# pgvector/pgvector

Measured on AMD Instinct MI355X. Metric: QPS @ recall@10 (IVFFlat, 1M x 1536d), higher is better.
Workload: dtype f32

## Files before the change

include/pgv_hip.h:

```cpp
#ifndef PGV_HIP_H
#define PGV_HIP_H

#include <stddef.h>
#include <stdint.h>

#ifdef __cplusplus
extern "C" {
#endif

#define PGV_ABI_VERSION 1

#define PGV_OK 0
#define PGV_ERR_ARG 1
#define PGV_ERR_DIMS 2
#define PGV_ERR_DEVICE 3
#define PGV_ERR_NOMEM 4
#define PGV_ERR_STATE 5
#define PGV_ERR_DATA 6

typedef enum pgv_dtype
{
	PGV_F32 = 0,
	PGV_F16 = 1
}			pgv_dtype;

typedef enum pgv_metric
{
	PGV_L2SQ = 0,
	PGV_NEG_IP = 1,
	PGV_L1 = 2
}			pgv_metric;

typedef enum pgv_ops
{
	PGV_OPS_L2 = 0,
	PGV_OPS_IP = 1,
	PGV_OPS_COSINE = 2
}			pgv_ops;

typedef struct pgv_ctx pgv_ctx;
typedef struct pgv_index pgv_index;
typedef struct pgv_hnsw pgv_hnsw;

typedef struct pgv_rng
{
	double		(*next_double) (void *state);
	uint32_t	(*next_u32) (void *state);
	void	   *state;
	uint64_t	seed;
}			pgv_rng;


const char *pgv_last_error(void);
int			pgv_abi_version(void);

int			pgv_device_count(void);
int			pgv_scan_chain_length(int dim, pgv_dtype dtype, int path);
int			pgv_device_memory(int device, uint64_t *free_bytes, uint64_t *total_bytes);
int			pgv_pinned_alloc(size_t bytes, void **out);
void		pgv_pinned_free(void *p);
int			pgv_pinned_register(void *p, size_t bytes);
void		pgv_pinned_unregister(void *p);

#define PGV_DEFAULT_STREAM ((void *) (intptr_t) -1)
int			pgv_ctx_create(int device, void *stream, pgv_ctx * *out);
void		pgv_ctx_destroy(pgv_ctx * ctx);
int			pgv_ctx_sync(pgv_ctx * ctx);
void	   *pgv_ctx_stream(pgv_ctx * ctx);
int			pgv_timer_start(pgv_ctx * ctx);
int			pgv_timer_stop(pgv_ctx * ctx, float *out_ms);

typedef struct pgv_stats
{
	double		scan_ms;
	int64_t		scan_launches;
	double		scan_pairs;
	double		scan_rows;
	double		aux_ms;
	int64_t		aux_launches;
	double		aux_pairs;
	double		assign_redo_rows;
	double		assign_rows;
	double		assign_recheck_rows;
	double		scan_unique_rows;
	double		scan_redo_queries;
	double		scan_widened_queries;
	double		scan_shadow_queries;
}			pgv_stats;
int			pgv_ctx_set_profiling(pgv_ctx * ctx, int on);
int			pgv_ctx_set_exact_scan(pgv_ctx * ctx, int on);
#define PGV_BOUND_STATISTICAL 0
#define PGV_BOUND_WORST_CASE 1
int			pgv_ctx_set_bound(pgv_ctx * ctx, int mode);
int			pgv_ctx_reset_stats(pgv_ctx * ctx);
int			pgv_ctx_get_stats(pgv_ctx * ctx, pgv_stats * out);


int			pgv_index_upload(pgv_ctx * ctx, pgv_metric metric, pgv_dtype dtype, int dim, int nlists,
							 const void *centers, const int64_t *list_offsets,
							 const void *vectors, const uint64_t *tids, pgv_index * *out);
void		pgv_index_free(pgv_index * index);
int			pgv_index_share(pgv_index * index, pgv_ctx * ctx, pgv_index * *out);
int			pgv_index_set_overlap(pgv_index * index, int lanes);
#define PGV_INDEX_HANDLE_BYTES 256
typedef struct pgv_index_handle
{
	unsigned char bytes[PGV_INDEX_HANDLE_BYTES];
}			pgv_index_handle;
int			pgv_index_export(pgv_index * index, pgv_index_handle * out);
int			pgv_index_import(pgv_ctx * ctx, const pgv_index_handle * handle, pgv_index * *out);
int			pgv_index_tids(pgv_index * index, const int64_t *slots, int64_t n, uint64_t *out);
int64_t		pgv_index_rows(const pgv_index * index);
int			pgv_index_lists(const pgv_index * index);

int			pgv_rank_lists(pgv_index * index, const void *queries, int nq, int maxprobes,
						   int32_t *out_lists, float *out_dist);

int			pgv_scan_lists(pgv_index * index, const void *query, const int32_t *lists, int nlists,
						   float *out_dist, int64_t *out_slot, int64_t capacity, int64_t *out_count);

int			pgv_search_batch(pgv_index * index, const void *queries, int nq, int probes, int k,
							 float *out_dist, int64_t *out_slot, uint64_t *out_tid);

int			pgv_index_shadow_cast(pgv_index * index, const void *queries, int nq, void *out_qcast, float *out_qscale,
								  float *out_qeps, float *out_cscale, float *out_ceps);

int			pgv_scan_batch(pgv_index * index, const void *queries, int nq, const int32_t *probe_lists,
						   int probes, int k, float *out_dist, int64_t *out_slot, uint64_t *out_tid);

typedef struct pgv_query pgv_query;
int			pgv_query_begin(pgv_index * index, pgv_query * *out);
void		pgv_query_end(pgv_query * q);
int			pgv_query_rank(pgv_query * q, const void *query, int max_probes);
int			pgv_query_scan(pgv_query * q, int first, int nprobes, int head, float *out_dist, int64_t *out_slot,
						   uint64_t *out_tid, int *out_count, int64_t *out_total);
int			pgv_query_more(pgv_query * q, int skip, int count, float *out_dist, int64_t *out_slot,
						   uint64_t *out_tid, int *out_count);
int			pgv_query_lists(pgv_query * q, int32_t *out_lists, int n);


int			pgv_assign(pgv_ctx * ctx, pgv_metric metric, pgv_dtype dtype, int dim,
					   const void *centers, int k, const void *rows, int64_t n,
					   int32_t *out_list, float *out_dist);

int			pgv_kmeans(pgv_ctx * ctx, pgv_ops ops, pgv_dtype dtype, int dim,
					   const void *samples, int n, int k, int max_iterations, const pgv_rng * rng,
					   void *out_centers, int32_t *out_closest, int *out_iters);

int			pgv_lloyd_partial(pgv_ctx * ctx, pgv_ops ops, pgv_dtype dtype, int dim,
							  const void *samples, int n, const void *centers, int k,
							  int32_t *io_closest, float *out_sums, int32_t *out_counts,
							  int64_t *out_changes);
int			pgv_lloyd_finish(pgv_ctx * ctx, pgv_ops ops, pgv_dtype dtype, int dim, int k,
							 const float *sums, const int32_t *counts, const pgv_rng * rng,
							 void *out_centers);

int			pgv_kmeanspp_init(pgv_ctx * ctx, pgv_ops ops, pgv_dtype dtype, int dim,
							  const void *samples, int n, int k, const pgv_rng * rng,
							  void *out_centers);


typedef struct pgv_comm pgv_comm;

#define PGV_COMM_ID_BYTES 128
int			pgv_comm_unique_id(void *out_id);
int			pgv_comm_create(pgv_ctx * ctx, int nranks, int rank, const void *unique_id, pgv_comm * *out);

typedef struct pgv_collectives
{
// ... 146 lines not shown
```

pgvector_amd/_lib.py:

```python
import ctypes as C
import os

try:
    import torch
except ImportError:
    torch = None

_HERE = os.path.dirname(os.path.abspath(__file__))
LIB_PATH = os.environ.get("PGV_HIP_LIB") or os.path.join(_HERE, "lib", "libpgv_hip.so")

PGV_OK, PGV_ERR_ARG, PGV_ERR_DIMS, PGV_ERR_DEVICE, PGV_ERR_NOMEM, PGV_ERR_STATE, PGV_ERR_DATA = range(7)
PGV_F32, PGV_F16 = 0, 1
PGV_L2SQ, PGV_NEG_IP, PGV_L1 = 0, 1, 2
PGV_OPS_L2, PGV_OPS_IP, PGV_OPS_COSINE = 0, 1, 2
PGV_BOUND_STATISTICAL, PGV_BOUND_WORST_CASE = 0, 1

SYMBOLS = [
    "pgv_last_error", "pgv_abi_version", "pgv_device_count", "pgv_scan_chain_length", "pgv_ctx_create", "pgv_ctx_destroy",
    "pgv_ctx_sync", "pgv_ctx_stream", "pgv_timer_start", "pgv_timer_stop", "pgv_ctx_set_profiling", "pgv_ctx_set_exact_scan", "pgv_index_share", "pgv_pinned_alloc", "pgv_pinned_free",
    "pgv_ctx_reset_stats", "pgv_ctx_get_stats", "pgv_index_upload", "pgv_index_free",
    "pgv_index_rows", "pgv_index_lists", "pgv_rank_lists", "pgv_scan_lists", "pgv_search_batch", "pgv_scan_batch",
    "pgv_assign", "pgv_kmeans", "pgv_lloyd_partial", "pgv_lloyd_finish", "pgv_kmeanspp_init",
    "pgv_distance_batch", "pgv_cosine_distance_batch", "pgv_bit_distance_batch", "pgv_hnsw_upload", "pgv_hnsw_free", "pgv_hnsw_score", "pgv_hnsw_set_graph", "pgv_hnsw_search",
    "pgv_hnsw_build_search", "pgv_hnsw_build_neighbors", "pgv_hnsw_link_begin", "pgv_hnsw_link_prepare",
    "pgv_hnsw_link_apply", "pgv_hnsw_link_end", "pgv_hnsw_build_search_keep", "pgv_hnsw_build_select_kept", "pgv_hnsw_score_pairs", "pgv_hnsw_score_groups", "pgv_hnsw_update_graph",
    "pgv_query_begin", "pgv_query_end", "pgv_query_rank", "pgv_query_scan", "pgv_query_more", "pgv_query_lists",
    "pgv_comm_unique_id", "pgv_comm_create", "pgv_comm_create_custom", "pgv_comm_destroy", "pgv_comm_size",
    "pgv_comm_rank", "pgv_kmeans_sharded", "pgv_search_batch_sharded",
    "pgv_device_memory", "pgv_pinned_register", "pgv_pinned_unregister", "pgv_index_export", "pgv_index_import",
    "pgv_index_tids", "pgv_hnsw_export", "pgv_hnsw_import", "pgv_hnsw_share", "pgv_hnsw_device", "pgv_exact_topk", "pgv_ctx_set_bound",
    "pgv_hnsw_upload_payload", "pgv_hnsw_get_payload", "pgv_builder_begin", "pgv_builder_add", "pgv_builder_set_centers", "pgv_builder_rows", "pgv_builder_finish", "pgv_builder_free", "pgv_index_drain",
    "pgv_index_set_overlap", "pgv_index_shadow_cast", "pgv_bit_topk", "pgv_binary_quantize", "pgv_rerank",
    "pgv_hnsw_upload_bits", "pgv_index_upload_bits", "pgv_index_nbits", "pgv_bit_assign", "pgv_bit_kmeans",
    "pgv_bit_lloyd_step", "pgv_sparse_distance_batch", "pgv_sparse_cosine_distance_batch", "pgv_sparse_topk",
]


class PgvError(RuntimeError):
    def __init__(self, code, message):
        super().__init__("libpgv_hip error %d: %s" % (code, message))
        self.code = code
        self.message = message


class PgvStats(C.Structure):
    _fields_ = [("scan_ms", C.c_double), ("scan_launches", C.c_int64),
                ("scan_pairs", C.c_double), ("scan_rows", C.c_double),
                ("aux_ms", C.c_double), ("aux_launches", C.c_int64), ("aux_pairs", C.c_double),
                ("assign_redo_rows", C.c_double), ("assign_rows", C.c_double), ("assign_recheck_rows", C.c_double), ("scan_unique_rows", C.c_double), ("scan_redo_queries", C.c_double), ("scan_widened_queries", C.c_double),
                ("scan_shadow_queries", C.c_double)]


ALL_REDUCE_F32 = C.CFUNCTYPE(C.c_int, C.c_void_p, C.c_void_p, C.c_size_t, C.c_void_p)
ALL_GATHER = C.CFUNCTYPE(C.c_int, C.c_void_p, C.c_void_p, C.c_void_p, C.c_size_t, C.c_void_p)


class PgvCollectives(C.Structure):
    _fields_ = [("all_reduce_sum_f32", ALL_REDUCE_F32), ("all_gather", ALL_GATHER), ("state", C.c_void_p)]


NEXT_DOUBLE = C.CFUNCTYPE(C.c_double, C.c_void_p)
NEXT_U32 = C.CFUNCTYPE(C.c_uint32, C.c_void_p)


class PgvRng(C.Structure):
    _fields_ = [("next_double", C.c_void_p), ("next_u32", C.c_void_p),
                ("state", C.c_void_p), ("seed", C.c_uint64)]


def _load():
    if not os.path.exists(LIB_PATH):
        raise ImportError(
            "libpgv_hip.so not built (%s): run `python -c 'import __graft_entry__ as g; g.build()'` "
            "or `make -C pgvector_amd/csrc` -- there is no CPU fallback" % LIB_PATH)
    lib = C.CDLL(LIB_PATH)
    P, I, I64 = C.c_void_p, C.c_int, C.c_int64
    lib.pgv_last_error.restype = C.c_char_p
    lib.pgv_last_error.argtypes = []
    lib.pgv_abi_version.restype = I
    lib.pgv_device_count.restype = I
    lib.pgv_scan_chain_length.argtypes = [I, I, I]
    lib.pgv_scan_chain_length.restype = I
    lib.pgv_ctx_create.argtypes = [I, P, C.POINTER(P)]
    lib.pgv_ctx_destroy.argtypes = [P]
    lib.pgv_ctx_destroy.restype = None
    lib.pgv_ctx_sync.argtypes = [P]
    lib.pgv_ctx_stream.argtypes = [P]
    lib.pgv_ctx_stream.restype = P
    lib.pgv_timer_start.argtypes = [P]
    lib.pgv_timer_stop.argtypes = [P, C.POINTER(C.c_float)]
    lib.pgv_ctx_set_profiling.argtypes = [P, I]
    lib.pgv_ctx_set_exact_scan.argtypes = [P, I]
    lib.pgv_ctx_reset_stats.argtypes = [P]
    lib.pgv_ctx_get_stats.argtypes = [P, C.POINTER(PgvStats)]
    lib.pgv_index_upload.argtypes = [P, I, I, I, I, P, P, P, P, C.POINTER(P)]
    lib.pgv_index_free.argtypes = [P]
    lib.pgv_index_share.argtypes = [P, P, C.POINTER(P)]
    lib.pgv_index_set_overlap.argtypes = [P, I]
    lib.pgv_index_shadow_cast.argtypes = [P, P, I, P, P, P, P, P]
    lib.pgv_index_free.restype = None
    lib.pgv_index_export.argtypes = [P, P]
    lib.pgv_index_import.argtypes = [P, P, C.POINTER(P)]
    lib.pgv_index_tids.argtypes = [P, P, I64, P]
    lib.pgv_hnsw_export.argtypes = [P, P]
    lib.pgv_hnsw_share.argtypes = [P, P, C.POINTER(P)]
    lib.pgv_hnsw_device.argtypes = [P]
    lib.pgv_hnsw_upload_payload.argtypes = [P, I, I, I, P, I64, P, I, C.POINTER(P)]
    lib.pgv_hnsw_get_payload.argtypes = [P, P, I, P]
    lib.pgv_hnsw_upload_bits.argtypes = [P, I, I, P, I64, P, I, C.POINTER(P)]
    lib.pgv_exact_topk.argtypes = [P, I, I, I, P, I, P, I64, I, P, P]
    lib.pgv_ctx_set_bound.argtypes = [P, I]
    lib.pgv_builder_begin.argtypes = [P, I, I, I, I, P, I64, C.POINTER(P)]
    lib.pgv_builder_add.argtypes = [P, P, P, I64]
    lib.pgv_builder_set_centers.argtypes = [P, P]
    lib.pgv_builder_rows.argtypes = [P]
    lib.pgv_builder_rows.restype = I64
    lib.pgv_builder_finish.argtypes = [P, C.POINTER(P), P, P]
    lib.pgv_builder_free.argtypes = [P]
    lib.pgv_builder_free.restype = None
    lib.pgv_index_drain.argtypes = [P, I64, P, P]
    lib.pgv_hnsw_import.argtypes = [P, P, C.POINTER(P)]
    lib.pgv_device_memory.argtypes = [I, C.POINTER(C.c_uint64), C.POINTER(C.c_uint64)]
    lib.pgv_pinned_register.argtypes = [P, C.c_size_t]
    lib.pgv_pinned_unregister.argtypes = [P]
    lib.pgv_pinned_unregister.restype = None
    lib.pgv_index_rows.argtypes = [P]
    lib.pgv_index_rows.restype = I64
    lib.pgv_index_lists.argtypes = [P]
    lib.pgv_rank_lists.argtypes = [P, P, I, I, P, P]
    lib.pgv_scan_lists.argtypes = [P, P, P, I, P, P, I64, C.POINTER(I64)]
    lib.pgv_search_batch.argtypes = [P, P, I, I, I, P, P, P]
    lib.pgv_scan_batch.argtypes = [P, P, I, P, I, I, P, P, P]
# ... 55 lines not shown
```

pgvector_amd/api.py:

```python
import ctypes as C
import weakref

import numpy as np

from . import _lib
from ._lib import (PGV_ERR_ARG, PGV_ERR_STATE, PGV_F16, PGV_F32, PGV_L1, PGV_L2SQ, PGV_NEG_IP, PGV_OPS_COSINE,
                   PGV_OPS_IP, PGV_OPS_L2, PgvError, PgvRng, PgvStats, check, lib)

_NP_OF = {PGV_F32: np.float32, PGV_F16: np.float16}


def _is_torch(x):
    return type(x).__module__.startswith("torch")


def ptr(x):
    if x is None:
        return None
    if _is_torch(x):
        assert x.is_contiguous(), "tensor must be contiguous"
        return C.c_void_p(x.data_ptr())
    assert isinstance(x, np.ndarray) and x.flags["C_CONTIGUOUS"], "need a C-contiguous array"
    return C.c_void_p(x.ctypes.data)

# ... 11 lines not shown

def as_dtype(x, dtype):
    if _is_torch(x):
        return x.contiguous()
    return np.ascontiguousarray(x, dtype=_NP_OF[dtype])


def make_rng(seed=0, next_double=None, next_u32=None, state=None):
    r = PgvRng()
    r.next_double = C.cast(next_double, C.c_void_p) if next_double is not None else None
    r.next_u32 = C.cast(next_u32, C.c_void_p) if next_u32 is not None else None
    r.state = state
    r.seed = seed
    return r


class Context:
    def __init__(self, device=0, stream=None):
        h = C.c_void_p()
        if stream is None:
            arg = None
        elif stream == 0:
            arg = C.c_void_p(-1)
        else:
            arg = C.c_void_p(stream)
        check(lib.pgv_ctx_create(device, arg, C.byref(h)))
        self.h = h
        self.device = device
        self._children = []

    def _adopt(self, child):
        self._children.append(weakref.ref(child))

    def close(self):
        if self.h:
            for ref in self._children:
                child = ref()
                if child is not None:
                    child.close()
            self._children = []
            lib.pgv_ctx_destroy(self.h)
            self.h = None

    def __del__(self):
        try:
            self.close()
        except Exception:
            pass

    def sync(self):
        check(lib.pgv_ctx_sync(self.h))

    def stream(self):
        return lib.pgv_ctx_stream(self.h)

    def timer_start(self):
        check(lib.pgv_timer_start(self.h))

    def timer_stop(self):
        ms = C.c_float()
        check(lib.pgv_timer_stop(self.h, C.byref(ms)))
        return ms.value

    def set_profiling(self, on):
        check(lib.pgv_ctx_set_profiling(self.h, 1 if on else 0))

    def set_exact_scan(self, on):
        check(lib.pgv_ctx_set_exact_scan(self.h, 1 if on else 0))

    def set_bound(self, worst_case):
        check(lib.pgv_ctx_set_bound(self.h, _lib.PGV_BOUND_WORST_CASE if worst_case else _lib.PGV_BOUND_STATISTICAL))

    def reset_stats(self):
        check(lib.pgv_ctx_reset_stats(self.h))

    def stats(self):
        s = PgvStats()
        check(lib.pgv_ctx_get_stats(self.h, C.byref(s)))
        return {"scan_ms": s.scan_ms, "scan_launches": s.scan_launches,
                "scan_pairs": s.scan_pairs, "scan_rows": s.scan_rows,
                "aux_ms": s.aux_ms, "aux_launches": s.aux_launches, "aux_pairs": s.aux_pairs,
                "assign_redo_rows": s.assign_redo_rows, "assign_rows": s.assign_rows,
                "assign_recheck_rows": s.assign_recheck_rows, "scan_unique_rows": s.scan_unique_rows, "scan_redo_queries": s.scan_redo_queries,
                "scan_widened_queries": s.scan_widened_queries, "scan_shadow_queries": s.scan_shadow_queries}


class IvfIndex:

    def __init__(self, ctx, metric, dtype, dim, centers, list_offsets, vectors, tids=None):
        self.ctx, self.metric, self.dtype, self.dim = ctx, metric, dtype, dim
        centers = as_dtype(centers, dtype)
        vectors = as_dtype(vectors, dtype)
        if not _is_torch(list_offsets):
            list_offsets = np.ascontiguousarray(list_offsets, dtype=np.int64)
        if tids is not None and not _is_torch(tids):
            tids = np.ascontiguousarray(tids, dtype=np.uint64)
        self.nlists = int(list_offsets.shape[0]) - 1
        h = C.c_void_p()
        check(lib.pgv_index_upload(ctx.h, metric, dtype, dim, self.nlists, ptr(centers),
                                   ptr(list_offsets), ptr(vectors), ptr(tids), C.byref(h)))
        self.h = h
        ctx._adopt(self)

    def set_overlap(self, lanes):
        check(lib.pgv_index_set_overlap(self.h, int(lanes)))

    def share(self, ctx):
        v = IvfIndex.__new__(IvfIndex)
        v.ctx, v.metric, v.dtype, v.dim, v.nlists = ctx, self.metric, self.dtype, self.dim, self.nlists
        h = C.c_void_p()
        check(lib.pgv_index_share(self.h, ctx.h, C.byref(h)))
        v.h = h
        ctx._adopt(v)
        return v

    def export(self):
        buf = C.create_string_buffer(256)
        check(lib.pgv_index_export(self.h, buf))
        return bytes(buf.raw)

    @classmethod
    def from_handle(cls, ctx, handle, metric=None, dtype=None, dim=None):
        v = cls.__new__(cls)
        h = C.c_void_p()
        buf = C.create_string_buffer(bytes(handle), 256)
        check(lib.pgv_index_import(ctx.h, buf, C.byref(h)))
        v.ctx, v.metric, v.dtype, v.dim, v.h = ctx, metric, dtype, dim, h
        v.nlists = lib.pgv_index_lists(h)
        ctx._adopt(v)
        return v

    def close(self):
        if self.h:
            lib.pgv_index_free(self.h)
            self.h = None

    def __del__(self):
        try:
            self.close()
        except Exception:
            pass

    @property
    def rows(self):
        return lib.pgv_index_rows(self.h)

    def tids(self, slots):
        slots = np.ascontiguousarray(slots, dtype=np.int64)
        out = np.empty(slots.shape, dtype=np.uint64)
        check(lib.pgv_index_tids(self.h, ptr(slots), int(slots.size), ptr(out)))
        return out

    def rank_lists(self, queries, maxprobes, want_dist=True):
        queries = as_dtype(queries, self.dtype)
        nq = int(queries.shape[0])
        lists = _empty_like_kind(queries, (nq, maxprobes), np.int32)
        dist = _empty_like_kind(queries, (nq, maxprobes), np.float32) if want_dist else None
        check(lib.pgv_rank_lists(self.h, ptr(queries), nq, maxprobes, ptr(lists), ptr(dist)))
        return lists, dist

    def scan_lists(self, query, lists):
        if query is not None:
            query = as_dtype(query, self.dtype)
        lists = np.ascontiguousarray(lists, dtype=np.int32)
        count = C.c_int64()
        rc = lib.pgv_scan_lists(self.h, ptr(query), ptr(lists), len(lists), None, None, 0, C.byref(count))
        if rc != _lib.PGV_OK and count.value == 0:
# ... 737 lines not shown
```

pgvector_amd/csrc/kernels_query.hip:

```cpp
#include "pgv_device.h"
#include "pgv_select.h"

#include <type_traits>

namespace pgv {

namespace {

constexpr int kQThreads = kSelThreads;
constexpr int kQWaves = kQThreads / kWave;
constexpr int kMaxBatchLists = 256;
constexpr int kHeadCap = 1024;

template <typename T, int METRIC, int NCH> struct WholeRows {
    Raw16 q[NCH];
    __device__ __forceinline__ void load_query(const char *qp, int lane) {
#pragma unroll
        for (int c = 0; c < NCH; c++) q[c] = load16(qp + ((size_t)c * kWave + lane) * sizeof(Raw16));
    }
    __device__ __forceinline__ float pair(const char *a, const char *b, int lane) const {
        Raw16 ra[NCH], rb[NCH];
#pragma unroll
        for (int c = 0; c < NCH; c++) ra[c] = load16(a + ((size_t)c * kWave + lane) * sizeof(Raw16));
#pragma unroll
// ... 222 lines not shown

template <typename T, int METRIC, int NCH>
__global__ __launch_bounds__(kQThreads) void mq_rank_kernel(const char *__restrict__ centers, int nlists, int nvec, int lg,
                                                            const char *__restrict__ queries, float *__restrict__ cdist,
                                                            int64_t cd_stride, int per) {
    const size_t row_bytes = (size_t)nvec * sizeof(Raw16);
    const char *qp = queries + (size_t)blockIdx.y * row_bytes;
    float *cd = cdist + (size_t)blockIdx.y * cd_stride;
    for (int64_t first = (int64_t)blockIdx.x * per; first < nlists; first += (int64_t)gridDim.x * per) {
        const int64_t end = first + per < nlists ? first + per : nlists;
        score_rows<T, METRIC, NCH>([&](int64_t j) { return centers + (size_t)j * row_bytes; }, first, end, qp, nvec, lg, cd);
    }
}

__global__ __launch_bounds__(kQThreads) void mq_lists_kernel(const float *__restrict__ cdist, int64_t cd_stride, int nlists,
                                                             int max_probes, int kp, int32_t *__restrict__ out_lists,
                                                             float *__restrict__ out_dist) {
    extern __shared__ __attribute__((aligned(16))) char smem[];
    unsigned long long *ent = reinterpret_cast<unsigned long long *>(smem);
    SelShared *s = reinterpret_cast<SelShared *>(smem + (size_t)kHeadCap * 8);
    const int q = blockIdx.x;
    block_topk_auto(cdist + (size_t)q * cd_stride, nlists, max_probes, kp, kHeadCap, ent, s);
    for (int i = threadIdx.x; i < max_probes; i += kQThreads) {
        out_lists[(size_t)q * max_probes + i] = (int32_t)(unsigned)(ent[i] & 0xffffffffu);
        if (out_dist) out_dist[(size_t)q * max_probes + i] = key_to_float((unsigned)(ent[i] >> 32));
    }
}

template <typename T, int METRIC, int NCH>
__global__ __launch_bounds__(kQThreads) void mq_scan_kernel(
    const char *__restrict__ vectors, const int64_t *__restrict__ list_off, const int32_t *__restrict__ probe_lists,
    int nprobes, int nvec, int lg, const char *__restrict__ queries, float *__restrict__ seg, int64_t seg_stride, int per) {
    __shared__ BatchMap map;
    const size_t row_bytes = (size_t)nvec * sizeof(Raw16);
    const int q = blockIdx.y;
    map.build(probe_lists + (size_t)q * nprobes, nprobes, list_off);
    const int64_t m = map.offs[nprobes];
    const char *qp = queries + (size_t)q * row_bytes;
    float *sg = seg + (size_t)q * seg_stride;
    for (int64_t first = (int64_t)blockIdx.x * per; first < m; first += (int64_t)gridDim.x * per) {
        const int64_t end = first + per < m ? first + per : m;
        score_rows<T, METRIC, NCH>([&](int64_t j) { return vectors + (size_t)map.slot_of(j, nprobes) * row_bytes; },
                                   first, end, qp, nvec, lg, sg);
    }
}

__global__ __launch_bounds__(kQThreads) void mq_head_kernel(
    const float *__restrict__ seg, int64_t seg_stride, const int64_t *__restrict__ list_off,
    const uint64_t *__restrict__ tids, const int32_t *__restrict__ probe_lists, int nprobes, int k, int kp,
    float *__restrict__ out_dist, int64_t *__restrict__ out_slot, uint64_t *__restrict__ out_tid,
    double *__restrict__ stats) {
    extern __shared__ __attribute__((aligned(16))) char smem[];
    __shared__ BatchMap map;
    const int q = blockIdx.x;
    map.build(probe_lists + (size_t)q * nprobes, nprobes, list_off);
    const int64_t m = map.offs[nprobes];
    unsigned long long *ent = reinterpret_cast<unsigned long long *>(smem);
    SelShared *s = reinterpret_cast<SelShared *>(smem + (size_t)kHeadCap * 8);
    block_topk_auto(seg + (size_t)q * seg_stride, m, k, kp, kHeadCap, ent, s);
    const int have = (int)(m < k ? m : k);
    for (int i = threadIdx.x; i < k; i += kQThreads) {
        const size_t o = (size_t)q * k + i;
        if (i < have) {
            const unsigned long long e = ent[i];
            const int64_t slot = map.slot_of((int64_t)(unsigned)(e & 0xffffffffu), nprobes);
            out_dist[o] = key_to_float((unsigned)(e >> 32));
            if (out_slot) out_slot[o] = slot;
            if (out_tid) out_tid[o] = tids ? tids[slot] : ~0ull;
        } else {
            out_dist[o] = INFINITY;
            if (out_slot) out_slot[o] = -1;
            if (out_tid) out_tid[o] = ~0ull;
        }
    }
    if (stats && threadIdx.x == 0) {
        atomicAdd(&stats[0], (double)m);
        atomicAdd(&stats[1], (double)m);
        atomicAdd(&stats[5], (double)m);
    }
}

constexpr int kRecheckCap = 256;

template <typename T, bool DOT = false>
__global__ __launch_bounds__(kQThreads) void batch_recheck_kernel(
    const char *__restrict__ vectors, const uint64_t *__restrict__ tids, int nvec, int lg,
    const char *__restrict__ queries, int kprime, int k, const float *__restrict__ approx_val,
    const int64_t *__restrict__ cand_pos, const int64_t *__restrict__ cand_slot,
    const int64_t *__restrict__ list_off, const int32_t *__restrict__ probe_lists,
    const int64_t *__restrict__ probe_off, int probes,
    const int64_t *__restrict__ seg_start, int64_t fixed_len,
    const unsigned *__restrict__ row_norm_max, ScanBound bound, const float *__restrict__ eps_add, int nq,
    float *__restrict__ out_dist, int64_t *__restrict__ out_slot, uint64_t *__restrict__ out_tid,
    int32_t *__restrict__ out_i32, int32_t *__restrict__ flags, float *__restrict__ pair_t, PlanEmit emit) {
    static_assert(!DOT || std::is_same<T, float>::value, "pair terms: fp32 rows");
    __shared__ float exact[kRecheckCap];
    __shared__ float dots[DOT ? kRecheckCap : 1];
    __shared__ __attribute__((aligned(16))) unsigned long long ent[kRecheckCap];
    const int q = blockIdx.x;
    const size_t row_bytes = (size_t)nvec * sizeof(Raw16);
    const int64_t m = seg_start ? seg_start[q + 1] - seg_start[q] : fixed_len;
    const int ncand = (int)(m < kprime ? m : (int64_t)kprime);
    const int kk = ncand < k ? ncand : k;
    const float *av = approx_val + (size_t)q * kprime;
    __shared__ float qn_part[kQWaves];
    {
        const char *qrow = queries + (size_t)q * row_bytes;
        float a = 0.f;
        for (int v = threadIdx.x; v < nvec; v += kQThreads) {
            const Raw16 x = load16(qrow + (size_t)v * sizeof(Raw16));
            a = accum_slice<T, 1>(a, x, x);
        }
        for (int m2 = 32; m2 > 0; m2 >>= 1) a += __shfl_xor(a, m2);
        if ((threadIdx.x & (kWave - 1)) == 0) qn_part[threadIdx.x >> 6] = a;
    }
    __syncthreads();
    float qn = 0.f;
    for (int w = 0; w < kQWaves; w++) qn += qn_part[w];
    const float rn = __uint_as_float(*row_norm_max);
    const float cross = 2.f * sqrtf(qn * rn);
    const float eps = 1.001f * (bound.g_sq * (qn + rn + cross) + bound.g_dot * cross + bound.g_norm * rn +
                                (eps_add ? eps_add[q] : 0.f));
    unsigned band = 0u;
    if (kk > 0) {
        const float edge = av[kk - 1] + 2.f * eps;
        band = float_to_key(edge + bound.g_ref * fabsf(edge + qn));
    }
    const int cnt = __syncthreads_count((int)threadIdx.x < ncand && float_to_key(av[threadIdx.x]) <= band);
    __shared__ int64_t slots[kRecheckCap];
    if ((int)threadIdx.x < cnt) {
        const int64_t p = cand_pos[(size_t)q * kprime + threadIdx.x];
        int64_t slot = p;
        if (cand_slot) {
            slot = cand_slot[(size_t)q * kprime + threadIdx.x];
        } else {
            const int64_t *off = probe_off + (size_t)q * probes;
            int lo = 0, hi = probes - 1;
            while (lo < hi) {
                const int mid = (lo + hi + 1) >> 1;
                if (off[mid] <= p)
                    lo = mid;
                else
                    hi = mid - 1;
            }
            slot = list_off[probe_lists[(size_t)q * probes + lo]] + (p - off[lo]);
        }
        slots[threadIdx.x] = slot;
    }
    __syncthreads();
    if constexpr (DOT)
        score_rows_dot([&](int64_t j) { return vectors + (size_t)slots[j] * row_bytes; }, 0, cnt,
                       queries + (size_t)q * row_bytes, nvec, lg, exact, dots);
    else
        score_rows<T, 0, 0>([&](int64_t j) { return vectors + (size_t)slots[j] * row_bytes; }, 0, cnt,
                            queries + (size_t)q * row_bytes, nvec, lg, exact);
    __syncthreads();
    if ((int)threadIdx.x < kRecheckCap)
        ent[threadIdx.x] = (int)threadIdx.x < cnt
                               ? ((unsigned long long)float_to_key(exact[threadIdx.x]) << 32) |
                                     (unsigned)cand_pos[(size_t)q * kprime + threadIdx.x]
                               : ~0ull;
    __syncthreads();
    const unsigned long long mine = ent[threadIdx.x];
    const int64_t my_slot = (int)threadIdx.x < cnt ? slots[threadIdx.x] : -1;
    int rank = 0;
    {
        const ulonglong2 *e2 = reinterpret_cast<const ulonglong2 *>(ent);
        const int n2 = (cnt + 1) / 2;
#pragma unroll 8
        for (int j = 0; j < n2; j++) {
            const ulonglong2 o = e2[j];
            rank += o.x < mine ? 1 : 0;
            rank += o.y < mine ? 1 : 0;
        }
    }
    if ((int)threadIdx.x < cnt && rank < k) {
        const size_t o = (size_t)q * k + rank;
        out_dist[o] = key_to_float((unsigned)(mine >> 32));
        if (out_slot) out_slot[o] = my_slot;
        if (out_i32) out_i32[o] = (int32_t)my_slot;
        if (out_tid) out_tid[o] = tids ? tids[my_slot] : ~0ull;
        if constexpr (DOT) pair_t[o] = -2.f * dots[threadIdx.x];
    }
    if ((int)threadIdx.x >= kk && (int)threadIdx.x < k) {
        const size_t o = (size_t)q * k + threadIdx.x;
        out_dist[o] = INFINITY;
        if (out_slot) out_slot[o] = -1;
        if (out_i32) out_i32[o] = -1;
        if (out_tid) out_tid[o] = ~0ull;
        if constexpr (DOT) pair_t[o] = 0.f;
    }
    if constexpr (DOT) {
        if (emit.cnt) {
            __syncthreads();
            if ((int)threadIdx.x < cnt && rank < k) {
                atomicAdd(&emit.cnt[my_slot], 1);
                slots[rank] = emit.list_off[my_slot + 1] - emit.list_off[my_slot];
            }
            if ((int)threadIdx.x >= kk && (int)threadIdx.x < k) slots[threadIdx.x] = 0;
            __syncthreads();
            if ((int)threadIdx.x < k) {
                int64_t run = 0;
                for (int i = 0; i < (int)threadIdx.x; i++) run += slots[i];
                emit.probe_off[(size_t)q * k + threadIdx.x] = run;
                if ((int)threadIdx.x == k - 1) emit.seg_len[q] = run + slots[threadIdx.x];
            }
        }
    }
    if (threadIdx.x == 0) {
        const int32_t flag = (m > ncand && cnt == ncand) ? 1 : 0;
        flags[q] = flag;
        if (flag) flags[nq + 1 + atomicAdd(&flags[nq], 1)] = q;
    }
}

constexpr int kWide = kRecheckCap;

template <typename T>
__global__ __launch_bounds__(kQThreads) void batch_fix_kernel(
    const char *__restrict__ vectors, const int64_t *__restrict__ list_off, const uint64_t *__restrict__ tids, int nvec,
    int lg, const char *__restrict__ queries, const int32_t *__restrict__ probe_lists,
    const int64_t *__restrict__ probe_off, int probes, const int64_t *__restrict__ seg_start, int64_t fixed_len,
    const int32_t *__restrict__ flags, int nq, float *__restrict__ seg_vals, int k, int kp, int cap,
    const unsigned *__restrict__ row_norm_max, ScanBound bound, const float *__restrict__ eps_add, int widen,
    float *__restrict__ out_dist, int64_t *__restrict__ out_slot, uint64_t *__restrict__ out_tid,
    int32_t *__restrict__ out_i32, double *__restrict__ stats, float *__restrict__ pair_t, PlanEmit emit) {
    extern __shared__ __attribute__((aligned(16))) char smem[];
    unsigned long long *ent = reinterpret_cast<unsigned long long *>(smem);
    SelShared *sel = reinterpret_cast<SelShared *>(smem + (size_t)cap * 8);
    __shared__ float exact[kWide];
    __shared__ int64_t slots[kWide];
    __shared__ float qn_part[kQWaves];
    const int nflag = flags[nq];
    const size_t row_bytes = (size_t)nvec * sizeof(Raw16);
    for (int f = blockIdx.x; f < nflag; f += gridDim.x) {
        const int q = flags[nq + 1 + f];
        const int64_t base = probe_lists ? seg_start[q] : (int64_t)q * fixed_len;
        const int64_t m = probe_lists ? seg_start[q + 1] - base : fixed_len;
        const int64_t *off = probe_off + (size_t)q * probes;
        const int32_t *pl = probe_lists + (size_t)q * probes;
        auto slot_of = [&](int64_t j) -> int64_t {
            if (!probe_lists) return j;
            int lo = 0, hi = probes - 1;
            while (lo < hi) {
                const int mid = (lo + hi + 1) >> 1;
                if (off[mid] <= j)
                    lo = mid;
                else
                    hi = mid - 1;
            }
            return list_off[pl[lo]] + (j - off[lo]);
        };
        float *v = seg_vals + base;
        const char *qrow = queries + (size_t)q * row_bytes;
        auto pair_terms = [&]() {
            if constexpr (std::is_same<T, float>::value) {
                if (pair_t) {
                    __threadfence();
                    __syncthreads();
                    fill_pair_terms(vectors, row_bytes, qrow, nvec * 4, out_i32 ? out_i32 + (size_t)q * k : nullptr,
                                    out_slot ? out_slot + (size_t)q * k : nullptr, k, pair_t + (size_t)q * k);
                    if (emit.cnt) {
                        if ((int)threadIdx.x < k) {
                            const int l = __hip_atomic_load(out_i32 + (size_t)q * k + threadIdx.x, __ATOMIC_RELAXED,
                                                            __HIP_MEMORY_SCOPE_AGENT);
                            if (l >= 0) atomicAdd(&emit.cnt[l], 1);
                            slots[threadIdx.x] = l >= 0 ? emit.list_off[l + 1] - emit.list_off[l] : 0;
                        }
                        __syncthreads();
                        if ((int)threadIdx.x < k) {
                            int64_t run = 0;
                            for (int i = 0; i < (int)threadIdx.x; i++) run += slots[i];
                            emit.probe_off[(size_t)q * k + threadIdx.x] = run;
                            if ((int)threadIdx.x == k - 1) emit.seg_len[q] = run + slots[threadIdx.x];
                        }
                    }
                }
            }
        };
        if constexpr (std::is_same<T, float>::value) {
            if (pair_t && emit.cnt) {
                if ((int)threadIdx.x < k) {
                    const int l = out_i32[(size_t)q * k + threadIdx.x];
                    if (l >= 0) atomicSub(&emit.cnt[l], 1);
                }
                __syncthreads();
            }
        }
        bool settled = false;
        if (widen && k <= kWide / 2) {
            const int nw = (int)(m < kWide ? m : (int64_t)kWide);
            block_topk([v](int64_t i) { return v[i]; }, m, nw, kWide, cap, ent, sel);
            {
                float a = 0.f;
                for (int x = threadIdx.x; x < nvec; x += kQThreads) {
                    const Raw16 e = load16(qrow + (size_t)x * sizeof(Raw16));
                    a = accum_slice<T, 1>(a, e, e);
                }
                for (int m2 = 32; m2 > 0; m2 >>= 1) a += __shfl_xor(a, m2);
                if ((threadIdx.x & (kWave - 1)) == 0) qn_part[threadIdx.x >> 6] = a;
            }
            __syncthreads();
            float qn = 0.f;
            for (int w = 0; w < kQWaves; w++) qn += qn_part[w];
            const float rn = __uint_as_float(*row_norm_max);
            const float cross = 2.f * sqrtf(qn * rn);
            const float eps = 1.001f * (bound.g_sq * (qn + rn + cross) + bound.g_dot * cross + bound.g_norm * rn +
                                        (eps_add ? eps_add[q] : 0.f));
            const int kk = nw < k ? nw : k;
            unsigned band = 0u;
            if (kk > 0) {
                const float edge = key_to_float((unsigned)(ent[kk - 1] >> 32)) + 2.f * eps;
                band = float_to_key(edge + bound.g_ref * fabsf(edge + qn));
            }
            const int cnt = __syncthreads_count((int)threadIdx.x < nw && (unsigned)(ent[threadIdx.x] >> 32) <= band);
            settled = !(m > nw && cnt == nw);
            if (settled) {
                const unsigned my_pos = (int)threadIdx.x < cnt ? (unsigned)(ent[threadIdx.x] & 0xffffffffu) : 0u;
                if ((int)threadIdx.x < cnt) slots[threadIdx.x] = slot_of((int64_t)my_pos);
                __syncthreads();
                score_rows<T, 0, 0>([&](int64_t j) { return vectors + (size_t)slots[j] * row_bytes; }, 0, cnt, qrow, nvec, lg,
                                    exact);
                __syncthreads();
                if ((int)threadIdx.x < kWide)
                    ent[threadIdx.x] = (int)threadIdx.x < cnt
                                           ? ((unsigned long long)float_to_key(exact[threadIdx.x]) << 32) | my_pos
                                           : ~0ull;
                __syncthreads();
                const unsigned long long mine = ent[threadIdx.x];
                int rank = 0;
                for (int j = 0; j < cnt; j++) rank += ent[j] < mine ? 1 : 0;
                const int have = (int)(m < k ? m : (int64_t)k);
                if ((int)threadIdx.x < cnt && rank < k) {
                    const size_t o = (size_t)q * k + rank;
                    const int64_t slot = slots[threadIdx.x];
                    out_dist[o] = key_to_float((unsigned)(mine >> 32));
                    if (out_slot) out_slot[o] = slot;
                    if (out_i32) out_i32[o] = (int32_t)slot;
                    if (out_tid) out_tid[o] = tids ? tids[slot] : ~0ull;
                }
                if ((int)threadIdx.x >= have && (int)threadIdx.x < k) {
                    const size_t o = (size_t)q * k + threadIdx.x;
                    out_dist[o] = INFINITY;
                    if (out_slot) out_slot[o] = -1;
                    if (out_i32) out_i32[o] = -1;
                    if (out_tid) out_tid[o] = ~0ull;
                }
                if (stats && threadIdx.x == 0) atomicAdd(&stats[7], 1.0);
                pair_terms();
            }
            __syncthreads();
        }
        if (settled) continue;
        if (stats && threadIdx.x == 0) atomicAdd(&stats[6], 1.0);
        score_rows<T, 0, 0>([&](int64_t j) { return vectors + (size_t)slot_of(j) * row_bytes; }, 0, m, qrow, nvec, lg, v);
        __threadfence();
        __syncthreads();
        block_topk([v](int64_t i) { return __hip_atomic_load(v + i, __ATOMIC_RELAXED, __HIP_MEMORY_SCOPE_AGENT); }, m, k, kp,
                   cap, ent, sel);
        for (int i = threadIdx.x; i < k; i += kQThreads) {
            const unsigned long long e = ent[i];
            const bool have = e != ~0ull && (int64_t)i < (m < k ? m : (int64_t)k);
            const int64_t slot = have ? slot_of((int64_t)(unsigned)(e & 0xffffffffu)) : -1;
            out_dist[(size_t)q * k + i] = have ? key_to_float((unsigned)(e >> 32)) : INFINITY;
            if (out_slot) out_slot[(size_t)q * k + i] = slot;
            if (out_i32) out_i32[(size_t)q * k + i] = (int32_t)slot;
            if (out_tid) out_tid[(size_t)q * k + i] = (have && tids) ? tids[slot] : ~0ull;
        }
        pair_terms();
        __syncthreads();
    }
}

constexpr size_t kQueryLds = (size_t)kHeadCap * 8 + sizeof(SelShared);

void run_geometry(pgv_ctx *ctx, const RowGeom &g, int64_t nrows, int *per, int *grid) {
    const bool whole = g.lpr_log2 == 6 && g.nvec % kWave == 0;
    const int step = kQWaves * (whole ? 2 : (kWave >> g.lpr_log2));
    int64_t runs = (nrows + step - 1) / step;
    const int64_t cap = (int64_t)ctx->num_cus * 8;
    *per = step;
    *grid = (int)(runs < 1 ? 1 : (runs > cap ? cap : runs));
}

int pow2_at_least(int k) {
    int kp = 2;
    while (kp < k) kp <<= 1;
    return kp;
}

template <typename T, int METRIC, typename F> int dispatch_nch(const RowGeom &g, F f) {
    if (g.lpr_log2 == 6 && g.nvec % kWave == 0) {
        switch (g.nvec / kWave) {
            case 1: return f(std::integral_constant<int, 1>());
            case 2: return f(std::integral_constant<int, 2>());
            case 3: return f(std::integral_constant<int, 3>());
            case 4: return f(std::integral_constant<int, 4>());
            case 6: return f(std::integral_constant<int, 6>());
        }
    }
    return f(std::integral_constant<int, 0>());
}

}

int query_max_batch_lists() { return kMaxBatchLists; }
int query_head_cap() { return kHeadCap; }
size_t query_head_bytes(int head) { return sizeof(QueryHead) + (size_t)head * (4 + 8 + 8) + 64; }

int launch_query_stage(pgv_ctx *ctx, const void *src_pinned, void *dst_dev, int nvec) {
    hipLaunchKernelGGL(query_stage_kernel, dim3(1), dim3(1024), 0, ctx->stream, static_cast<const Raw16 *>(src_pinned),
                       static_cast<Raw16 *>(dst_dev), nvec);
    PGV_HIP(hipGetLastError());
    return PGV_OK;
}

int launch_query_iota(pgv_ctx *ctx, int32_t *out, int n) {
    hipLaunchKernelGGL(query_iota_kernel, dim3((n + 255) / 256), dim3(256), 0, ctx->stream, out, n);
    PGV_HIP(hipGetLastError());
    return PGV_OK;
}

int launch_one_query_rows(pgv_ctx *ctx, const RowsView &v, const void *q_dev, float *out) {
    if (v.n <= 0) return PGV_OK;
    if (v.bits()) PGV_FAIL(PGV_ERR_ARG, "one query over rows: fp32 / fp16 rows only");
    const RowGeom &g = v.geom;
    const void *rows = v.rows;
    const int n = (int)v.n;
    int per, grid;
    run_geometry(ctx, g, n, &per, &grid);
    return dispatch_metric(v.metric, v.dtype(), [&](auto *tp, auto mc) {
        using T = std::remove_pointer_t<decltype(tp)>;
        constexpr int M = decltype(mc)::value;
        return dispatch_nch<T, M>(g, [&](auto nc) {
            constexpr int NCH = decltype(nc)::value;
            hipLaunchKernelGGL((query_rank_kernel<T, M, NCH>), dim3(grid), dim3(kQThreads), 0, ctx->stream,
                               static_cast<const char *>(rows), n, g.nvec, g.lpr_log2, static_cast<const char *>(q_dev),
                               out, per);
            PGV_HIP(hipGetLastError());
            return PGV_OK;
        });
    });
}

int launch_query_rank(pgv_ctx *ctx, const pgv_index *ix, const void *q_dev, float *cdist, int max_probes,
                      int32_t *out_lists) {
    const RowGeom &g = ix->geom;
    int per, grid;
    run_geometry(ctx, g, ix->nlists, &per, &grid);
    const int kp = pow2_at_least(max_probes);
    PGV_TRY(dispatch_metric(ix->metric, ix->dtype, [&](auto *tp, auto mc) {
        using T = std::remove_pointer_t<decltype(tp)>;
        constexpr int M = decltype(mc)::value;
        return dispatch_nch<T, M>(g, [&](auto nc) {
            constexpr int NCH = decltype(nc)::value;
            hipLaunchKernelGGL((query_rank_kernel<T, M, NCH>), dim3(grid), dim3(kQThreads), 0, ctx->stream,
// ... 13 lines not shown
                      int64_t rows_bound, float *seg) {
    const RowGeom &g = ix->geom;
    int per, grid;
    run_geometry(ctx, g, rows_bound, &per, &grid);
    return dispatch_metric(ix->metric, ix->dtype, [&](auto *tp, auto mc) {
        using T = std::remove_pointer_t<decltype(tp)>;
        constexpr int M = decltype(mc)::value;
        return dispatch_nch<T, M>(g, [&](auto nc) {
            constexpr int NCH = decltype(nc)::value;
            hipLaunchKernelGGL((query_scan_kernel<T, M, NCH>), dim3(grid), dim3(kQThreads), 0, ctx->stream,
                               static_cast<const char *>(ix->vectors), ix->list_offsets, probe_lists, nprobes, g.nvec,
                               g.lpr_log2, static_cast<const char *>(q_dev), seg, per);
            PGV_HIP(hipGetLastError());
            return PGV_OK;
        });
    });
}

int launch_query_head(pgv_ctx *ctx, const pgv_index *ix, const float *seg, const int32_t *probe_lists, int nprobes,
                      int skip, int count, void *head_rec, unsigned seq) {
    const int kp = pow2_at_least(skip + count);
    QueryHead *hdr = static_cast<QueryHead *>(head_rec);
    char *base = static_cast<char *>(head_rec) + 64;
    int64_t *h_slot = reinterpret_cast<int64_t *>(base);
    uint64_t *h_tid = reinterpret_cast<uint64_t *>(base + (size_t)count * 8);
    float *h_dist = reinterpret_cast<float *>(base + (size_t)count * 16);
    hipLaunchKernelGGL(query_head_kernel, dim3(1), dim3(kQThreads), kQueryLds, ctx->stream, seg, ix->list_offsets,
                       ix->tids, probe_lists, nprobes, skip, count, kp, hdr, h_dist, h_slot, h_tid, seq);
    PGV_HIP(hipGetLastError());
    return PGV_OK;
}

int launch_multi_rank(pgv_ctx *ctx, const pgv_index *ix, const void *q_dev, int nq, float *cdist, int64_t cd_stride,
                      int max_probes, int32_t *out_lists, float *out_dist) {
    const RowGeom &g = ix->geom;
    int per, grid;
    run_geometry(ctx, g, ix->nlists, &per, &grid);
    const int kp = pow2_at_least(max_probes);
    PGV_TRY(dispatch_metric(ix->metric, ix->dtype, [&](auto *tp, auto mc) {
        using T = std::remove_pointer_t<decltype(tp)>;
        constexpr int M = decltype(mc)::value;
        return dispatch_nch<T, M>(g, [&](auto nc) {
            constexpr int NCH = decltype(nc)::value;
            hipLaunchKernelGGL((mq_rank_kernel<T, M, NCH>), dim3(grid, nq), dim3(kQThreads), 0, ctx->stream,
                               static_cast<const char *>(ix->centers), ix->nlists, g.nvec, g.lpr_log2,
                               static_cast<const char *>(q_dev), cdist, cd_stride, per);
            PGV_HIP(hipGetLastError());
            return PGV_OK;
        });
    }));
    hipLaunchKernelGGL(mq_lists_kernel, dim3(nq), dim3(kQThreads), kQueryLds, ctx->stream, cdist, cd_stride, ix->nlists,
                       max_probes, kp, out_lists, out_dist);
    PGV_HIP(hipGetLastError());
    return PGV_OK;
}

int launch_multi_scan(pgv_ctx *ctx, const pgv_index *ix, const void *q_dev, int nq, const int32_t *probe_lists, int nprobes,
                      int64_t rows_bound, float *seg, int64_t seg_stride, int k, float *out_dist, int64_t *out_slot,
                      uint64_t *out_tid) {
    const RowGeom &g = ix->geom;
    int per, grid;
    run_geometry(ctx, g, rows_bound, &per, &grid);
    const int cap = (ctx->num_cus * 8 + nq - 1) / nq;
    if (grid > cap) grid = cap < 1 ? 1 : cap;
    PGV_TRY(dispatch_metric(ix->metric, ix->dtype, [&](auto *tp, auto mc) {
        using T = std::remove_pointer_t<decltype(tp)>;
        constexpr int M = decltype(mc)::value;
        return dispatch_nch<T, M>(g, [&](auto nc) {
            constexpr int NCH = decltype(nc)::value;
            hipLaunchKernelGGL((mq_scan_kernel<T, M, NCH>), dim3(grid, nq), dim3(kQThreads), 0, ctx->stream,
                               static_cast<const char *>(ix->vectors), ix->list_offsets, probe_lists, nprobes, g.nvec,
                               g.lpr_log2, static_cast<const char *>(q_dev), seg, seg_stride, per);
            PGV_HIP(hipGetLastError());
            return PGV_OK;
        });
    }));
    double *stats = (ctx->profiling && ctx->stats_dev.p) ? ctx->stats_dev.as<double>() : nullptr;
    hipLaunchKernelGGL(mq_head_kernel, dim3(nq), dim3(kQThreads), kQueryLds, ctx->stream, seg, seg_stride, ix->list_offsets,
                       ix->tids, probe_lists, nprobes, k, pow2_at_least(k), out_dist, out_slot, out_tid, stats);
    PGV_HIP(hipGetLastError());
    return PGV_OK;
}

namespace {
struct ApproxScratch {
    float *cand_val = nullptr;
    int64_t *cand_pos = nullptr;
    int32_t *flags = nullptr;
    int carve(DBuf &buf, int nq, int kprime) {
        const size_t nk = (size_t)nq * kprime;
        const size_t a1 = (sizeof(float) * nk + 15) & ~(size_t)15, a2 = a1 + sizeof(int64_t) * nk;
        PGV_TRY(buf.ensure(a2 + sizeof(int32_t) * (2 * (size_t)nq + 1)));
        cand_val = buf.as<float>();
        cand_pos = reinterpret_cast<int64_t *>(buf.as<char>() + a1);
        flags = reinterpret_cast<int32_t *>(buf.as<char>() + a2);
        return PGV_OK;
    }
};
}

int launch_exact_tail(pgv_ctx *ctx, const ExactTail &t, DBuf &scratch) {
    if (t.nq <= 0) return PGV_OK;
    const ExactRows &xr = t.rows;
    const bool dense = t.dense();
    if (dense ? (t.fixed_len <= 0 || t.probe_off || t.seg_start || t.probes != 0)
              : (t.fixed_len != 0 || !t.probe_off || !t.seg_start || t.probes < 1))
        PGV_FAIL(PGV_ERR_ARG, "exact tail: a list plan or one dense run");
    if (t.kprime > kRecheckCap || t.k > t.kprime)
        PGV_FAIL(PGV_ERR_ARG, "exact tail: k' = %d outside k..%d", t.kprime, kRecheckCap);
    if (t.pair_t && xr.dtype != PGV_F32) PGV_FAIL(PGV_ERR_ARG, "exact tail: pair terms are for fp32 rows");
    static_assert(kWide >= kRecheckCap, "k <= k' <= kWide: batch_fix_kernel's emit");
    if (t.emit.cnt && !(dense && t.pair_t && t.out_i32 && t.emit.probe_off && t.emit.seg_len && t.emit.list_off))
        PGV_FAIL(PGV_ERR_ARG, "exact tail: the plan is counted where the pair terms are written");
    ApproxScratch sc;
    PGV_TRY(sc.carve(scratch, t.nq, t.kprime));
    const int64_t *cand_slot = dense ? sc.cand_pos : nullptr;
    const int64_t *seg_start = dense ? nullptr : t.seg_start;
    const int64_t fixed_len = dense ? t.fixed_len : 0;
    PGV_TRY(launch_topk_segments(ctx, t.approx, seg_start, t.nq, fixed_len, t.kprime, sc.cand_val, sc.cand_pos,
                                 sc.flags + t.nq, t.emit.cnt, t.emit.cnt ? 2 * (int)fixed_len : 0,
                                 dense ? 0 : t.seg_bound));
#define PGV_RECHECK(T, DOT)                                                                                          \
    hipLaunchKernelGGL((batch_recheck_kernel<T, DOT>), dim3(t.nq), dim3(kQThreads), 0, ctx->stream,                   \
                       static_cast<const char *>(xr.vectors), xr.tids, xr.geom.nvec, xr.geom.lpr_log2,                \
                       static_cast<const char *>(t.queries), t.kprime, t.k, sc.cand_val, sc.cand_pos, cand_slot,      \
                       xr.list_offsets, t.probe_lists, t.probe_off, t.probes, seg_start, fixed_len, xr.norm_max,      \
                       t.bound, t.eps_add, t.nq, t.out_dist, t.out_slot, t.out_tid, t.out_i32, sc.flags, t.pair_t,    \
                       t.emit)
    if (t.pair_t)
        PGV_RECHECK(float, true);
    else if (xr.dtype == PGV_F32)
        PGV_RECHECK(float, false);
    else
        PGV_RECHECK(__half, false);
#undef PGV_RECHECK
    PGV_HIP(hipGetLastError());
    double *stats = (ctx->profiling && ctx->stats_dev.p) ? ctx->stats_dev.as<double>() : nullptr;
    int kp = 2;
    while (kp < t.k) kp <<= 1;
    const int cap = kp > kFastCap ? kp : kFastCap;
    const size_t lds = (size_t)cap * 8 + sizeof(SelShared);
    const int grid = t.nq < ctx->num_cus ? t.nq : ctx->num_cus;
#define PGV_FIX(T)                                                                                                    \
    hipLaunchKernelGGL(batch_fix_kernel<T>, dim3(grid), dim3(kQThreads), lds, ctx->stream,                            \
                       static_cast<const char *>(xr.vectors), xr.list_offsets, xr.tids, xr.geom.nvec,                 \
                       xr.geom.lpr_log2, static_cast<const char *>(t.queries), t.probe_lists, t.probe_off, t.probes,  \
                       seg_start, fixed_len, sc.flags, t.nq, t.approx, t.k, kp, cap, xr.norm_max, t.bound, t.eps_add, \
                       ctx->no_widen ? 0 : 1, t.out_dist, t.out_slot, t.out_tid, t.out_i32, stats, t.pair_t, t.emit)
    if (xr.dtype == PGV_F32)
        PGV_FIX(float);
    else
        PGV_FIX(__half);
#undef PGV_FIX
    PGV_HIP(hipGetLastError());
    return PGV_OK;
}

}
```

pgvector_amd/csrc/kernels_select.hip:

```cpp
#include "pgv_device.h"
#include "pgv_select.h"

namespace pgv {

namespace {


__global__ void plan_count_kernel(const int32_t *__restrict__ probe_lists,
                                  const int64_t *__restrict__ list_off, int nq, int probes,
                                  int *__restrict__ cnt, int64_t *__restrict__ probe_off,
                                  int64_t *__restrict__ seg_len) {
    const int q = blockIdx.x * blockDim.x + threadIdx.x;
    if (q >= nq) return;
    int64_t run = 0;
    for (int p = 0; p < probes; p++) {
        const int l = probe_lists[(size_t)q * probes + p];
        probe_off[(size_t)q * probes + p] = run;
        run += list_off[l + 1] - list_off[l];
        atomicAdd(&cnt[l], 1);
    }
    seg_len[q] = run;
}

template <typename F>
__device__ void block_exclusive_scan(int n, F value, int64_t *out, int64_t *scratch ) {
    const int lane = threadIdx.x & 63, wave = threadIdx.x >> 6, nwaves = blockDim.x >> 6;
    int64_t carry = 0;
    for (int base = 0; base < n; base += blockDim.x) {
        const int i = base + threadIdx.x;
        const int64_t v = i < n ? value(i) : 0;
        int64_t incl = v;
#pragma unroll
        for (int d = 1; d < 64; d <<= 1) {
            const int64_t t = __shfl_up(incl, d);
            if (lane >= d) incl += t;
        }
        if (lane == 63) scratch[wave] = incl;
        __syncthreads();
        int64_t before = 0, total = 0;
        for (int w = 0; w < nwaves; w++) {
            const int64_t t = scratch[w];
            if (w < wave) before += t;
            total += t;
        }
        if (i < n) out[i] = carry + before + incl - v;
        carry += total;
        __syncthreads();
    }
    if (threadIdx.x == 0) out[n] = carry;
    __syncthreads();
}

__global__ __launch_bounds__(1024) void plan_scan_kernel(
    const int *__restrict__ cnt, const int64_t *__restrict__ list_off,
    const int64_t *__restrict__ seg_len, int nq, int nlists, int qt, int rows_per_task,
    int64_t *__restrict__ seg_start, int64_t *__restrict__ pair_start,
    int64_t *__restrict__ task_start, int64_t *__restrict__ totals ,
    double *__restrict__ acc) {
    __shared__ int64_t scratch[1024 / 64 + 1];
    __shared__ double red[2][1024 / 64];
    block_exclusive_scan(nq, [&](int i) { return seg_len[i]; }, seg_start, scratch);
    block_exclusive_scan(nlists, [&](int i) { return (int64_t)cnt[i]; }, pair_start, scratch);
    double rows = 0.0, uniq = 0.0;
    block_exclusive_scan(
        nlists,
        [&](int i) {
            const int64_t len = list_off[i + 1] - list_off[i];
            const int64_t ng = (cnt[i] + qt - 1) / qt;
            const int64_t nc = (len + rows_per_task - 1) / rows_per_task;
            rows += (double)ng * (double)len;
            uniq += ng > 0 ? (double)len : 0.0;
            return ng * nc;
        },
        task_start, scratch);
    if (threadIdx.x == 0) {
        totals[0] = seg_start[nq];
        totals[1] = task_start[nlists];
        *reinterpret_cast<int *>(totals + 2) = (int)task_start[nlists];
    }
    if (acc) {
        for (int o = 32; o > 0; o >>= 1) {
            rows += __shfl_xor(rows, o);
            uniq += __shfl_xor(uniq, o);
        }
        if ((threadIdx.x & 63) == 0) {
            red[0][threadIdx.x >> 6] = rows;
            red[1][threadIdx.x >> 6] = uniq;
        }
        __syncthreads();
        if (threadIdx.x == 0) {
            double r = 0.0, u = 0.0;
            for (int w = 0; w < (int)(blockDim.x >> 6); w++) {
                r += red[0][w];
                u += red[1][w];
            }
            acc[0] += (double)seg_start[nq];
            acc[1] += r;
            acc[5] += u;
        }
    }
}

__device__ __forceinline__ void plan_pairs_body(int64_t i, const int32_t *__restrict__ probe_lists,
                                                const int64_t *__restrict__ list_off,
                                                const int64_t *__restrict__ probe_off,
                                                const int64_t *__restrict__ seg_start,
                                                const int64_t *__restrict__ pair_start, int *__restrict__ fill,
                                                int nq, int probes, const float *__restrict__ pair_t,
                                                ScanPair *__restrict__ pairs) {
    if (i >= (int64_t)nq * probes) return;
    const int q = (int)(i / probes);
    const int l = probe_lists[i];
    const int64_t pos = pair_start[l] + atomicAdd(&fill[l], 1);
    ScanPair pr;
    pr.out_rel = seg_start[q] + probe_off[i] - list_off[l];
    pr.query = q;
    pr.pad = pair_t ? (int32_t)__float_as_uint(pair_t[i]) : 0;
    pairs[pos] = pr;
}

__global__ void plan_pairs_kernel(const int32_t *__restrict__ probe_lists,
                                  const int64_t *__restrict__ list_off,
                                  const int64_t *__restrict__ probe_off,
                                  const int64_t *__restrict__ seg_start,
                                  const int64_t *__restrict__ pair_start, int *__restrict__ fill,
                                  int nq, int probes, const float *__restrict__ pair_t,
                                  ScanPair *__restrict__ pairs) {
    plan_pairs_body((int64_t)blockIdx.x * blockDim.x + threadIdx.x, probe_lists, list_off, probe_off, seg_start, pair_start,
                    fill, nq, probes, pair_t, pairs);
}

__device__ __forceinline__ void plan_tasks_body(int64_t first, int64_t stride, const int *__restrict__ cnt,
                                                const int64_t *__restrict__ list_off,
                                                const int64_t *__restrict__ pair_start,
                                                const int64_t *__restrict__ task_start, int nlists, int qt,
                                                int rows_per_task, ScanTask *__restrict__ tasks) {
    const int64_t ntasks = task_start[nlists];
    for (int64_t t = first; t < ntasks; t += stride) {
        int lo = 0, hi = nlists - 1;
        while (lo < hi) {
            const int mid = (lo + hi + 1) >> 1;
            if (task_start[mid] <= t)
                lo = mid;
            else
                hi = mid - 1;
        }
        const int l = lo;
        const int64_t len = list_off[l + 1] - list_off[l];
        const int ng = (cnt[l] + qt - 1) / qt;
        const int64_t rel = t - task_start[l];
        const int c = (int)(rel / ng), g = (int)(rel % ng);
        ScanTask task;
        task.row0 = list_off[l] + (int64_t)c * rows_per_task;
        const int64_t left = len - (int64_t)c * rows_per_task;
        task.nrows = (int)(left < rows_per_task ? left : rows_per_task);
        task.pair0 = (int)(pair_start[l] + (int64_t)g * qt);
        const int pl = cnt[l] - g * qt;
        task.npairs = pl < qt ? pl : qt;
        task.pad = ng > 1 ? 1 : 0;
        tasks[t] = task;
    }
}

__global__ void plan_tasks_kernel(const int *__restrict__ cnt, const int64_t *__restrict__ list_off,
                                  const int64_t *__restrict__ pair_start,
                                  const int64_t *__restrict__ task_start, int nlists, int qt,
                                  int rows_per_task, ScanTask *__restrict__ tasks) {
    plan_tasks_body((int64_t)blockIdx.x * blockDim.x + threadIdx.x, (int64_t)gridDim.x * blockDim.x, cnt, list_off,
                    pair_start, task_start, nlists, qt, rows_per_task, tasks);
}

__global__ void plan_pairs_tasks_kernel(const int32_t *__restrict__ probe_lists, const int64_t *__restrict__ list_off,
                                        const int64_t *__restrict__ probe_off, const int64_t *__restrict__ seg_start,
                                        const int64_t *__restrict__ pair_start, const int64_t *__restrict__ task_start,
                                        const int *__restrict__ cnt, int *__restrict__ fill, int nq, int probes, int nlists,
                                        int qt, int rows_per_task, const float *__restrict__ pair_t, int pair_blocks,
                                        ScanPair *__restrict__ pairs, ScanTask *__restrict__ tasks) {
    if ((int)blockIdx.x < pair_blocks)
        plan_pairs_body((int64_t)blockIdx.x * blockDim.x + threadIdx.x, probe_lists, list_off, probe_off, seg_start,
                        pair_start, fill, nq, probes, pair_t, pairs);
    else
        plan_tasks_body((int64_t)(blockIdx.x - pair_blocks) * blockDim.x + threadIdx.x,
                        (int64_t)(gridDim.x - pair_blocks) * blockDim.x, cnt, list_off, pair_start, task_start, nlists, qt,
                        rows_per_task, tasks);
}

__device__ __forceinline__ bool dist_before(float a, float b) { return float_to_key(a) < float_to_key(b); }

enum TopkClass { kTopkSmall = 0, kTopkMedium = 1, kTopkLong = 2 };
constexpr int kLongVec = 16;
constexpr int kLongTail = 16;
constexpr int kLongMax = (kLongVec + kLongTail) * 4 * kSelThreads;

template <int CLS>
__device__ __forceinline__ bool topk_class_forms(const float *va, int ma, int skip, int k, int kp, int cap,
// ... 5 lines not shown
        if (ma <= 16 * kSelThreads) return block_topk_small<4>(va, ma, skip, k, kp, cap, ent, s);
    } else {
        if (ma <= 16 * kSelThreads) return block_topk_small<4>(va, ma, skip, k, kp, cap, ent, s);
        if (ma <= kSmallVec * 4 * kSelThreads) return block_topk_small<kSmallVec>(va, ma, skip, k, kp, cap, ent, s);
        if (ma <= kLongVec * 4 * kSelThreads) return block_topk_small<kLongVec>(va, ma, skip, k, kp, cap, ent, s);
        if (ma <= kLongMax) return block_topk_small<kLongVec, kLongTail>(va, ma, skip, k, kp, cap, ent, s);
    }
    return false;
}

template <int CLS>
__global__ __launch_bounds__(kSelThreads) void topk_kernel(
    const float *__restrict__ vals, const int64_t *__restrict__ seg_start, int64_t fixed_len,
    int k, int kp, int cap, float *__restrict__ out_val, int64_t *__restrict__ out_pos,
    int32_t *__restrict__ zero_word, int32_t *__restrict__ zero_range, int zero_n) {
    extern __shared__ __attribute__((aligned(16))) char smem[];
    unsigned long long *ent = reinterpret_cast<unsigned long long *>(smem);
    SelShared *s = reinterpret_cast<SelShared *>(smem + (size_t)cap * 8);

    const int seg = blockIdx.x;
    if (zero_word && seg == 0 && threadIdx.x == 0) *zero_word = 0;
    if (zero_range)
        for (int i = seg * kSelThreads + (int)threadIdx.x; i < zero_n; i += (int)gridDim.x * kSelThreads) zero_range[i] = 0;
    const int64_t base = seg_start ? seg_start[seg] : (int64_t)seg * fixed_len;
    const int64_t m = seg_start ? seg_start[seg + 1] - base : fixed_len;
    const float *v = vals + base;
    bool done = false;
    const int skip = (int)((reinterpret_cast<uintptr_t>(v) >> 2) & 3);
    const int64_t ma = m + skip;
    if (m > k && ma <= kLongMax && k <= kSelThreads / 2)
        done = topk_class_forms<CLS>(v - skip, (int)ma, skip, k, kp, cap, ent, s);
    if (!done) block_topk([v](int64_t i) { return v[i]; }, m, k, kp, cap, ent, s);

    for (int i = threadIdx.x; i < k; i += kSelThreads) {
        const unsigned long long e = ent[i];
        const bool have = e != ~0ull && (int64_t)i < (m < k ? m : (int64_t)k);
        out_val[(size_t)seg * k + i] = have ? key_to_float((unsigned)(e >> 32)) : INFINITY;
        out_pos[(size_t)seg * k + i] = have ? (int64_t)(unsigned)(e & 0xffffffffu) : -1;
    }
}

__global__ void positions_to_slots_kernel(const int32_t *__restrict__ probe_lists,
                                          const int64_t *__restrict__ probe_off,
                                          const int64_t *__restrict__ list_off,
                                          const uint64_t *__restrict__ tids, int nq, int probes,
                                          int k, const int64_t *__restrict__ pos,
                                          int64_t *__restrict__ out_slot,
                                          uint64_t *__restrict__ out_tid) {
    const int64_t i = (int64_t)blockIdx.x * blockDim.x + threadIdx.x;
    if (i >= (int64_t)nq * k) return;
    const int q = (int)(i / k);
    const int64_t p = pos[i];
    int64_t slot = -1;
    if (p >= 0) {
        const int64_t *off = probe_off + (size_t)q * probes;
        int lo = 0, hi = probes - 1;
        while (lo < hi) {
            const int mid = (lo + hi + 1) >> 1;
            if (off[mid] <= p)
                lo = mid;
            else
                hi = mid - 1;
        }
        const int l = probe_lists[(size_t)q * probes + lo];
        slot = list_off[l] + (p - off[lo]);
    }
    if (out_slot) out_slot[i] = slot;
    if (out_tid) out_tid[i] = (slot >= 0 && tids) ? tids[slot] : ~0ull;
}

__global__ void iota_slots_kernel(const int32_t *__restrict__ lists,
                                  const int64_t *__restrict__ probe_off,
                                  const int64_t *__restrict__ list_off,
                                  int64_t *__restrict__ out_slot) {
    const int p = blockIdx.x;
    const int l = lists[p];
    const int64_t beg = list_off[l], len = list_off[l + 1] - beg;
    for (int64_t i = threadIdx.x; i < len; i += blockDim.x) out_slot[probe_off[p] + i] = beg + i;
}

__global__ __launch_bounds__(256) void plan_stats_kernel(const int *__restrict__ cnt,
                                                         const int64_t *__restrict__ list_off,
                                                         const int64_t *__restrict__ totals, int nlists,
                                                         int qt, double *__restrict__ acc) {
    __shared__ double red[256], red_u[256];
    double rows = 0.0, uniq = 0.0;
    for (int l = threadIdx.x; l < nlists; l += 256) {
        const double len = (double)(list_off[l + 1] - list_off[l]);
        rows += (double)((cnt[l] + qt - 1) / qt) * len;
        uniq += cnt[l] > 0 ? len : 0.0;
    }
    red[threadIdx.x] = rows;
    red_u[threadIdx.x] = uniq;
    __syncthreads();
    for (int s = 128; s > 0; s >>= 1) {
        if (threadIdx.x < s) {
            red[threadIdx.x] += red[threadIdx.x + s];
            red_u[threadIdx.x] += red_u[threadIdx.x + s];
        }
        __syncthreads();
    }
    if (threadIdx.x == 0) {
        acc[0] += (double)totals[0];
        acc[1] += red[0];
        acc[5] += red_u[0];
    }
}

__global__ void merge_heads_kernel(const float *__restrict__ dist_all, const uint64_t *__restrict__ tid_all, int nranks,
                                   int nq, int k, float *__restrict__ out_dist, uint64_t *__restrict__ out_tid) {
    const int q = blockIdx.x * blockDim.x + threadIdx.x;
    if (q >= nq) return;
    int at[16];
    for (int r = 0; r < nranks; r++) at[r] = 0;
    for (int i = 0; i < k; i++) {
        int best = -1;
        float bd = INFINITY;
        for (int r = 0; r < nranks; r++) {
            if (at[r] >= k) continue;
            const float d = dist_all[((size_t)r * nq + q) * k + at[r]];
            if (best < 0 || dist_before(d, bd)) {
                best = r;
                bd = d;
            }
        }
        out_dist[(size_t)q * k + i] = bd;
        out_tid[(size_t)q * k + i] = tid_all[((size_t)best * nq + q) * k + at[best]];
        at[best]++;
    }
}

__global__ void cast_pos_kernel(const int64_t *__restrict__ pos, int64_t n,
                                int32_t *__restrict__ out) {
    const int64_t i = (int64_t)blockIdx.x * blockDim.x + threadIdx.x;
    if (i < n) out[i] = (int32_t)pos[i];
}

}

int launch_merge_heads(pgv_ctx *ctx, const float *dist_all, const uint64_t *tid_all, int nranks, int nq, int k,
                       float *out_dist, uint64_t *out_tid) {
    if (nq <= 0) return PGV_OK;
    if (nranks > 16) PGV_FAIL(PGV_ERR_ARG, "merge: more than 16 ranks");
    hipLaunchKernelGGL(merge_heads_kernel, dim3((nq + 127) / 128), dim3(128), 0, ctx->stream, dist_all, tid_all, nranks,
                       nq, k, out_dist, out_tid);
    PGV_HIP(hipGetLastError());
    return PGV_OK;
}

int launch_cast_pos_to_i32(pgv_ctx *ctx, const int64_t *pos, int64_t n, int32_t *out) {
    if (n <= 0) return PGV_OK;
    hipLaunchKernelGGL(cast_pos_kernel, dim3((unsigned)((n + 255) / 256)), dim3(256), 0,
                       ctx->stream, pos, n, out);
    PGV_HIP(hipGetLastError());
    return PGV_OK;
}

int plan_batch_reserve(pgv_ctx *ctx, int nlists, int nq, int probes, PlanBuffers *pb) {
    const size_t npairs = (size_t)nq * probes;
    PGV_TRY(ctx->plan_a.ensure(sizeof(int) * 2 * (size_t)nlists));
    const size_t nb = npairs + (size_t)nq + (size_t)nq + 1 + 2 * ((size_t)nlists + 1) + 3;
    PGV_TRY(ctx->plan_b.ensure(sizeof(int64_t) * nb));
    pb->cnt = ctx->plan_a.as<int>();
    pb->fill = pb->cnt + nlists;
    pb->probe_off = ctx->plan_b.as<int64_t>();
    pb->seg_len = pb->probe_off + npairs;
    pb->seg_start = pb->seg_len + nq;
    pb->pair_start = pb->seg_start + nq + 1;
    pb->task_start = pb->pair_start + nlists + 1;
    pb->totals = pb->task_start + nlists + 1;
    return PGV_OK;
}

int launch_plan_batch(pgv_ctx *ctx, const pgv_index *ix, const int32_t *probe_lists, int nq,
                      int probes, int qt, int rows_per_task, bool read_totals, PlanResult *res, const float *pair_t,
                      bool counted) {
    const int nlists = ix->nlists;
    const size_t npairs = (size_t)nq * probes;

    int64_t max_chunks = 0, sum_chunks = 0;
    for (int l = 0; l < nlists; l++) {
        const int64_t nc = (ix->h_offsets[l + 1] - ix->h_offsets[l] + rows_per_task - 1) / rows_per_task;
        sum_chunks += nc;
        if (nc > max_chunks) max_chunks = nc;
    }
    res->ntasks_bound = max_chunks * (int64_t)(npairs / qt) + sum_chunks;
    res->out_bound = (int64_t)nq * ix->len_prefix[probes];
    if (res->ntasks_bound > 0x7fffffff) PGV_FAIL(PGV_ERR_ARG, "plan: too many tasks");

    PlanBuffers pb;
    PGV_TRY(plan_batch_reserve(ctx, nlists, nq, probes, &pb));
    PGV_TRY(ctx->pairs.ensure(sizeof(ScanPair) * npairs));
    PGV_TRY(ctx->tasks.ensure(sizeof(ScanTask) * (size_t)(res->ntasks_bound > 0 ? res->ntasks_bound : 1) + 16));
    int *cnt = pb.cnt, *fill = pb.fill;
    int64_t *probe_off = pb.probe_off, *seg_len = pb.seg_len, *seg_start = pb.seg_start, *pair_start = pb.pair_start;
    int64_t *task_start = pb.task_start, *totals = pb.totals;
    ScanTask *tasks = ctx->tasks.as<ScanTask>();
    const int64_t want = (res->ntasks_bound + 255) / 256;
    const int64_t cap = (int64_t)ctx->num_cus * 8;
    const unsigned task_blocks = (unsigned)(want < 1 ? 1 : (want > cap ? cap : want));
    const unsigned pair_blocks = (unsigned)((npairs + 255) / 256);
    res->ntasks = res->ntasks_bound;
    res->total_out = res->out_bound;

    if (counted) {
        double *acc = nullptr;
        if (read_totals) {
            PGV_TRY(ctx->stats_dev.ensure(8 * sizeof(double)));
            acc = ctx->stats_dev.as<double>();
        }
        hipLaunchKernelGGL(plan_scan_kernel, dim3(1), dim3(1024), 0, ctx->stream, cnt, ix->list_offsets, seg_len, nq, nlists,
                           qt, rows_per_task, seg_start, pair_start, task_start, totals, acc);
        hipLaunchKernelGGL(plan_pairs_tasks_kernel, dim3(pair_blocks + task_blocks), dim3(256), 0, ctx->stream, probe_lists,
                           ix->list_offsets, probe_off, seg_start, pair_start, task_start, cnt, fill, nq, probes, nlists, qt,
                           rows_per_task, pair_t, (int)pair_blocks, ctx->pairs.as<ScanPair>(), tasks);
        PGV_HIP(hipGetLastError());
    } else {
        PGV_HIP(hipMemsetAsync(cnt, 0, sizeof(int) * 2 * (size_t)nlists, ctx->stream));
        hipLaunchKernelGGL(plan_count_kernel, dim3((nq + 255) / 256), dim3(256), 0, ctx->stream,
                           probe_lists, ix->list_offsets, nq, probes, cnt, probe_off, seg_len);
        hipLaunchKernelGGL(plan_scan_kernel, dim3(1), dim3(1024), 0, ctx->stream, cnt,
                           ix->list_offsets, seg_len, nq, nlists, qt, rows_per_task, seg_start,
                           pair_start, task_start, totals, static_cast<double *>(nullptr));
        hipLaunchKernelGGL(plan_pairs_kernel, dim3(pair_blocks), dim3(256), 0,
                           ctx->stream, probe_lists, ix->list_offsets, probe_off, seg_start,
                           pair_start, fill, nq, probes, pair_t, ctx->pairs.as<ScanPair>());
        hipLaunchKernelGGL(plan_tasks_kernel, dim3(task_blocks), dim3(256), 0,
                           ctx->stream, cnt, ix->list_offsets, pair_start, task_start, nlists, qt, rows_per_task, tasks);
        PGV_HIP(hipGetLastError());
        if (read_totals) {
            PGV_TRY(ctx->stats_dev.ensure(8 * sizeof(double)));
            hipLaunchKernelGGL(plan_stats_kernel, dim3(1), dim3(256), 0, ctx->stream, cnt,
                               ix->list_offsets, totals, nlists, qt, ctx->stats_dev.as<double>());
            PGV_HIP(hipGetLastError());
        }
    }
    res->tasks = tasks;
    res->pairs = ctx->pairs.as<ScanPair>();
    res->ntasks_dev = reinterpret_cast<int *>(totals + 2);
    res->seg_start = seg_start;
    res->probe_off = probe_off;
    res->pair_start = pair_start;
    return PGV_OK;
}

int launch_topk_segments(pgv_ctx *ctx, const float *vals, const int64_t *seg_start, int nseg,
                         int64_t fixed_len, int k, float *out_val, int64_t *out_pos, int32_t *zero_word,
                         int32_t *zero_range, int zero_n, int64_t len_bound) {
    if (nseg <= 0 || k <= 0) return PGV_OK;
    if (k > 4096) PGV_FAIL(PGV_ERR_ARG, "top-k: k = %d exceeds the supported 4096", k);
    int kp = 1;
    while (kp < k) kp <<= 1;
    if (kp < 2) kp = 2;
    const int cap = kp > kFastCap ? kp : kFastCap;
    const size_t lds = (size_t)cap * 8 + sizeof(SelShared);
    int64_t ma_bound = 0;
    if (!seg_start)
        ma_bound = fixed_len + (fixed_len % 4 == 0 ? (int64_t)((reinterpret_cast<uintptr_t>(vals) >> 2) & 3) : 3);
    else if (len_bound > 0)
        ma_bound = len_bound + 3;
    auto kernel = topk_kernel<kTopkLong>;
    if (ma_bound > 0 && ma_bound <= 4 * kSelThreads)
        kernel = topk_kernel<kTopkSmall>;
    else if (ma_bound > 0 && ma_bound <= 16 * kSelThreads)
        kernel = topk_kernel<kTopkMedium>;
    hipLaunchKernelGGL(kernel, dim3(nseg), dim3(kSelThreads), lds, ctx->stream, vals, seg_start, fixed_len, k, kp, cap,
                       out_val, out_pos, zero_word, zero_range, zero_n);
    PGV_HIP(hipGetLastError());
    return PGV_OK;
}

int launch_positions_to_slots(pgv_ctx *ctx, const pgv_index *ix, const int32_t *probe_lists,
                              const int64_t *probe_off, int nq, int probes, int k,
                              const int64_t *pos, int64_t *out_slot, uint64_t *out_tid) {
    const int64_t total = (int64_t)nq * k;
    if (total <= 0) return PGV_OK;
    hipLaunchKernelGGL(positions_to_slots_kernel, dim3((unsigned)((total + 255) / 256)), dim3(256),
                       0, ctx->stream, probe_lists, probe_off, ix->list_offsets, ix->tids, nq,
                       probes, k, pos, out_slot, out_tid);
    PGV_HIP(hipGetLastError());
    return PGV_OK;
}

int launch_iota_slots(pgv_ctx *ctx, const pgv_index *ix, const int32_t *lists_dev, int nlists,
                      const int64_t *probe_off, int64_t *out_slot) {
    if (nlists <= 0) return PGV_OK;
    hipLaunchKernelGGL(iota_slots_kernel, dim3(nlists), dim3(256), 0, ctx->stream, lists_dev,
                       probe_off, ix->list_offsets, out_slot);
    PGV_HIP(hipGetLastError());
    return PGV_OK;
}

}
```

pgvector_amd/csrc/kernels_shadow.hip:

```cpp
#include "pgv_device.h"

#include <cfloat>

namespace pgv {

namespace {

__device__ __forceinline__ int list_of_row(const int64_t *__restrict__ list_off, int nlists, int64_t r) {
    int lo = 0, hi = nlists - 1;
    while (lo < hi) {
        const int mid = (lo + hi + 1) >> 1;
        if (list_off[mid] <= r)
            lo = mid;
        else
            hi = mid - 1;
    }
    return lo;
}

__device__ __forceinline__ int scale_for(float m) {
    if (!(m > 0.f) || !isfinite(m)) return 0;
    int e;
    (void)frexpf(m, &e);
    return e - 14;
}

__global__ __launch_bounds__(256) void shadow_absmax_kernel(const float *__restrict__ rows, const float *__restrict__ centers,
                                                            const int64_t *__restrict__ list_off, int nlists, int64_t n,
                                                            int ld, unsigned *__restrict__ max_bits) {
    const int64_t r = (int64_t)blockIdx.x * 4 + (threadIdx.x >> 6);
    if (r >= n) return;
    const int lane = threadIdx.x & (kWave - 1);
    const float *x = rows + (size_t)r * ld;
    const float *c = centers ? centers + (size_t)list_of_row(list_off, nlists, r) * ld : nullptr;
    float m = 0.f;
    for (int i = lane; i < ld; i += kWave) {
        const float d = fabsf(c ? x[i] - c[i] : x[i]);
        m = (d > m || d != d) ? d : m;
    }
    for (int o = 32; o > 0; o >>= 1) {
        const float v = __shfl_xor(m, o);
        m = (v > m || v != v) ? v : m;
    }
    if (lane == 0 && __float_as_uint(m) > __hip_atomic_load(max_bits, __ATOMIC_RELAXED, __HIP_MEMORY_SCOPE_AGENT))
        atomicMax(max_bits, __float_as_uint(m));
}

__global__ __launch_bounds__(256) void shadow_build_kernel(const float *__restrict__ rows, const float *__restrict__ centers,
                                                           const int64_t *__restrict__ list_off, int nlists, int64_t n,
                                                           int ld, int ld16, const unsigned *__restrict__ max_bits,
                                                           __half *__restrict__ shadow,
                                                           unsigned long long *__restrict__ ep_bits) {
    const int64_t r = (int64_t)blockIdx.x * 4 + (threadIdx.x >> 6);
    if (r >= n) return;
    const int lane = threadIdx.x & (kWave - 1);
    const int s = scale_for(__uint_as_float(*max_bits));
    const float *x = rows + (size_t)r * ld;
    const float *c = centers ? centers + (size_t)list_of_row(list_off, nlists, r) * ld : nullptr;
    __half *h = shadow + (size_t)r * ld16;
    const double up = ldexp(1.0, s);
    double e2 = 0.0, p2 = 0.0;
    for (int i = lane; i < ld16; i += kWave) {
        __half v = __float2half(0.f);
        if (i < ld) {
            const float ci = c ? c[i] : 0.f;
            v = __float2half(ldexpf(x[i] - ci, -s));
            const double back = (double)__half2float(v) * up;
            const double d = ((double)x[i] - (double)ci) - back;
            e2 = fma(d, d, e2);
            p2 = fma(back, back, p2);
        }
        h[i] = v;
    }
    for (int o = 32; o > 0; o >>= 1) {
        e2 += __shfl_xor(e2, o);
        p2 += __shfl_xor(p2, o);
    }
    if (lane == 0) {
        const unsigned long long eb = (unsigned long long)__double_as_longlong(e2 != e2 ? INFINITY : e2),
                                 pb = (unsigned long long)__double_as_longlong(p2 != p2 ? INFINITY : p2);
        if (eb > __hip_atomic_load(&ep_bits[0], __ATOMIC_RELAXED, __HIP_MEMORY_SCOPE_AGENT)) atomicMax(&ep_bits[0], eb);
        if (pb > __hip_atomic_load(&ep_bits[1], __ATOMIC_RELAXED, __HIP_MEMORY_SCOPE_AGENT)) atomicMax(&ep_bits[1], pb);
    }
}

constexpr int kCastChunks = 4;

struct CastChunk {
    float4 a, b;
};

__device__ __forceinline__ float absmax_keep_nan(float m, float v) {
    const float a = fabsf(v);
    return (a > m || a != a) ? a : m;
}

__device__ __forceinline__ CastChunk cast_chunk_load(const float *__restrict__ x, int c, int ld) {
    CastChunk r;
    const float4 zero = make_float4(0.f, 0.f, 0.f, 0.f);
    r.a = 8 * c < ld ? *reinterpret_cast<const float4 *>(x + 8 * c) : zero;
    r.b = 8 * c + 4 < ld ? *reinterpret_cast<const float4 *>(x + 8 * c + 4) : zero;
    return r;
}

__device__ __forceinline__ float cast_chunk_max(const CastChunk &r, float m) {
    m = absmax_keep_nan(m, r.a.x);
    m = absmax_keep_nan(m, r.a.y);
    m = absmax_keep_nan(m, r.a.z);
    m = absmax_keep_nan(m, r.a.w);
    m = absmax_keep_nan(m, r.b.x);
    m = absmax_keep_nan(m, r.b.y);
    m = absmax_keep_nan(m, r.b.z);
    m = absmax_keep_nan(m, r.b.w);
    return m;
}

__device__ __forceinline__ void cast_chunk_store(const CastChunk &r, int c, int ld, int sq, double up, __half *__restrict__ h,
                                                 double (&qq)[4], double (&dd)[4], double (&hh)[4]) {
    const float xs[8] = {r.a.x, r.a.y, r.a.z, r.a.w, r.b.x, r.b.y, r.b.z, r.b.w};
    union {
        __half v[8];
        uint4 w;
    } out;
#pragma unroll
    for (int e = 0; e < 8; e++) {
        __half v = __float2half(0.f);
        if (8 * c + e < ld) {
            v = __float2half(ldexpf(xs[e], -sq));
            const double back = (double)__half2float(v) * up, xi = (double)xs[e];
            qq[e & 3] = fma(xi, xi, qq[e & 3]);
            dd[e & 3] = fma(xi - back, xi - back, dd[e & 3]);
            hh[e & 3] = fma(back, back, hh[e & 3]);
        }
        out.v[e] = v;
    }
    *reinterpret_cast<uint4 *>(h + 8 * c) = out.w;
}

__global__ __launch_bounds__(256) void shadow_query_kernel(const float *__restrict__ queries, int nq, int ld, int ld16,
                                                           ShadowTerms st, RankShadowTerms rt,
                                                           const float *__restrict__ center_norm_max,
                                                           const float *__restrict__ row_norm_max,
                                                           __half *__restrict__ qcast, float *__restrict__ qscale,
                                                           float *__restrict__ qeps, float *__restrict__ cscale,
                                                           float *__restrict__ ceps) {
    const int q = (int)(blockIdx.x * 4 + (threadIdx.x >> 6));
    if (q >= nq) return;
    const int lane = threadIdx.x & (kWave - 1);
    const float *x = queries + (size_t)q * ld;
    __half *h = qcast + (size_t)q * ld16;
    const int nchunks = ld16 / 8;
    const bool in_regs = nchunks <= kWave * kCastChunks;
    CastChunk reg[kCastChunks];
    float m = 0.f;
    if (in_regs) {
#pragma unroll
        for (int j = 0; j < kCastChunks; j++) {
            const int c = lane + j * kWave;
            reg[j] = cast_chunk_load(x, c < nchunks ? c : nchunks, ld);
        }
#pragma unroll
        for (int j = 0; j < kCastChunks; j++) m = cast_chunk_max(reg[j], m);
    } else {
        for (int c = lane; c < nchunks; c += kWave) m = cast_chunk_max(cast_chunk_load(x, c, ld), m);
    }
    for (int o = 32; o > 0; o >>= 1) {
        const float v = __shfl_xor(m, o);
        m = (v > m || v != v) ? v : m;
    }
    const int sq = scale_for(m);
    const double up = ldexp(1.0, sq);
    double qq4[4] = {0.0, 0.0, 0.0, 0.0}, dd4[4] = {0.0, 0.0, 0.0, 0.0}, hh4[4] = {0.0, 0.0, 0.0, 0.0};
    if (in_regs) {
#pragma unroll
        for (int j = 0; j < kCastChunks; j++) {
            const int c = lane + j * kWave;
            if (c < nchunks) cast_chunk_store(reg[j], c, ld, sq, up, h, qq4, dd4, hh4);
        }
    } else {
        for (int c = lane; c < nchunks; c += kWave) cast_chunk_store(cast_chunk_load(x, c, ld), c, ld, sq, up, h, qq4, dd4, hh4);
    }
    double qq = (qq4[0] + qq4[1]) + (qq4[2] + qq4[3]);
    double dd = (dd4[0] + dd4[1]) + (dd4[2] + dd4[3]);
    double hh = (hh4[0] + hh4[1]) + (hh4[2] + hh4[3]);
    for (int o = 32; o > 0; o >>= 1) {
        qq += __shfl_xor(qq, o);
        dd += __shfl_xor(dd, o);
        hh += __shfl_xor(hh, o);
    }
    const double u = 5.9604644775390625e-8;
    if (lane == 0 && ceps) {
        const int e = 1 + rt.s + sq;
        const double qn = sqrt(qq), dq = sqrt(dd), qh = sqrt(hh);
        const double cn = (double)*center_norm_max * (1.0 + rt.g_cn);
        double eps = 2.0 * (qn * rt.E + dq * rt.P)
                     + rt.g_dot * 2.0 * qh * rt.P
                     + 4.0 * u * (cn + 2.0 * qh * rt.P * (1.0 + rt.g_dot));
        eps = eps * (1.0 + 1.0 / 1048576.0) + 4.0 * (double)FLT_MIN;
        if (e < -125 || e > 125 || !(eps < 1e30)) eps = INFINITY;
        cscale[q] = ldexpf(1.f, e < -125 ? 0 : (e > 125 ? 0 : e));
        ceps[q] = (float)eps;
    }
    if (lane == 0 && qeps) {
        const int e = 1 + st.s + sq;
        const double qn = sqrt(qq), dq = sqrt(dd), qh = sqrt(hh);
        const double cmax = sqrt((double)*center_norm_max * (1.0 + st.g_cn)), rn = (double)*row_norm_max * (1.0 + st.g_cn);
        const double tmax = 2.0 * qn * cmax;
        double eps = 2.0 * (qn * st.E + dq * st.P)
                     + st.g_dot * 2.0 * qh * st.P
                     + st.g_pair * tmax
                     + 4.0 * u * (rn + tmax * (1.0 + st.g_pair) + 2.0 * qh * st.P * (1.0 + st.g_dot));
        eps = eps * (1.0 + 1.0 / 1048576.0) + 4.0 * (double)FLT_MIN;
        if (e < -125 || e > 125 || !(eps < 1e30)) eps = INFINITY;
        qscale[q] = ldexpf(1.f, e < -125 ? 0 : (e > 125 ? 0 : e));
        qeps[q] = (float)eps;
    }
}

__global__ __launch_bounds__(256) void shadow_pair_kernel(const float *__restrict__ queries, const float *__restrict__ centers,
                                                          const int64_t *__restrict__ pair_start, int nlists, int64_t npairs,
                                                          int ld, ScanPair *__restrict__ pairs) {
    const int64_t pos = (int64_t)blockIdx.x * 4 + (threadIdx.x >> 6);
    if (pos >= npairs) return;
    const int lane = threadIdx.x & (kWave - 1);
    int lo = 0, hi = nlists - 1;
    while (lo < hi) {
        const int mid = (lo + hi + 1) >> 1;
        if (pair_start[mid] <= pos)
            lo = mid;
        else
            hi = mid - 1;
    }
    const int q = pairs[pos].query;
    const float *x = queries + (size_t)q * ld;
    const float *c = centers + (size_t)lo * ld;
    float a = 0.f;
    for (int i = lane; i < ld; i += kWave) a = fmaf(x[i], c[i], a);
    for (int o = 32; o > 0; o >>= 1) a += __shfl_xor(a, o);
    if (lane == 0) pairs[pos].pad = (int32_t)__float_as_uint(-2.f * a);
}

}

int launch_shadow_build(pgv_ctx *ctx, const RowGeom &g32, const RowGeom &g16, const void *rows, const void *centers,
                        const int64_t *list_off, int nlists, int64_t n, void *shadow, void *words) {
    if (n <= 0) return PGV_OK;
    PGV_HIP(hipMemsetAsync(words, 0, 24, ctx->stream));
    unsigned *max_bits = static_cast<unsigned *>(words);
    unsigned long long *ep = reinterpret_cast<unsigned long long *>(static_cast<char *>(words) + 8);
    const dim3 grid((unsigned)((n + 3) / 4));
    hipLaunchKernelGGL(shadow_absmax_kernel, grid, dim3(256), 0, ctx->stream, static_cast<const float *>(rows),
                       static_cast<const float *>(centers), list_off, nlists, n, g32.ld, max_bits);
    hipLaunchKernelGGL(shadow_build_kernel, grid, dim3(256), 0, ctx->stream, static_cast<const float *>(rows),
                       static_cast<const float *>(centers), list_off, nlists, n, g32.ld, g16.ld, max_bits, static_cast<__half *>(shadow), ep);
    PGV_HIP(hipGetLastError());
    return PGV_OK;
}

int shadow_scale_of(float max_abs) {
    if (!(max_abs > 0.f) || !std::isfinite(max_abs)) return 0;
    int e;
    (void)std::frexp(max_abs, &e);
    return e - 14;
}

int launch_shadow_query(pgv_ctx *ctx, const RowGeom &g32, const RowGeom &g16, const void *queries, int nq,
                        const ShadowTerms &st, const RankShadowTerms &rt, const float *center_norm_max,
                        const float *row_norm_max, void *qcast, float *qscale, float *qeps, float *cscale, float *ceps) {
    if (nq <= 0) return PGV_OK;
    hipLaunchKernelGGL(shadow_query_kernel, dim3((unsigned)((nq + 3) / 4)), dim3(256), 0, ctx->stream,
                       static_cast<const float *>(queries), nq, g32.ld, g16.ld, st, rt, center_norm_max, row_norm_max,
                       static_cast<__half *>(qcast), qscale, qeps, cscale, ceps);
    PGV_HIP(hipGetLastError());
    return PGV_OK;
}

int launch_shadow_pairs(pgv_ctx *ctx, const RowGeom &g32, const void *queries, const void *centers,
                        const int64_t *pair_start, int nlists, int64_t npairs, ScanPair *pairs) {
    if (npairs <= 0) return PGV_OK;
    hipLaunchKernelGGL(shadow_pair_kernel, dim3((unsigned)((npairs + 3) / 4)), dim3(256), 0, ctx->stream,
                       static_cast<const float *>(queries), static_cast<const float *>(centers), pair_start, nlists, npairs,
                       g32.ld, pairs);
    PGV_HIP(hipGetLastError());
    return PGV_OK;
}

}
```

pgvector_amd/csrc/pgv_abi.hip:

```cpp
#include "pgv_abi_common.h"




namespace pgv {

static thread_local char g_err[512] = "";

void set_error(const char *fmt, ...) {
    va_list ap;
    va_start(ap, fmt);
    vsnprintf(g_err, sizeof(g_err), fmt, ap);
    va_end(ap);
}

int DBuf::ensure(size_t bytes) {
    bytes += 64;
    if (bytes <= cap && p) return PGV_OK;
    if (p) {
        (void)hipFree(p);
        p = nullptr;
        cap = 0;
    }
    size_t want = bytes < 256 ? 256 : bytes;
// ... 123 lines not shown
    hipDeviceProp_t prop;
    PGV_HIP(hipGetDeviceProperties(&prop, device));
    if (strncmp(prop.gcnArchName, "gfx950", 6) != 0)
        PGV_FAIL(PGV_ERR_DEVICE, "device %d is %s; libpgv_hip is built for gfx950 only", device,
                 prop.gcnArchName);
    pgv_ctx *ctx = new (std::nothrow) pgv_ctx();
    if (!ctx) PGV_FAIL(PGV_ERR_NOMEM, "out of host memory");
    ctx->device = device;
    {
        const char *e = getenv("PGV_NO_WIDEN");
        ctx->no_widen = e && atoi(e) != 0;
    }
    ctx->num_cus = prop.multiProcessorCount > 0 ? prop.multiProcessorCount : 256;
    if (stream == PGV_DEFAULT_STREAM) {
        ctx->stream = nullptr;
    } else if (stream) {
        ctx->stream = static_cast<hipStream_t>(stream);
    } else {
        hipError_t e = hipStreamCreateWithFlags(&ctx->stream, hipStreamNonBlocking);
        if (e != hipSuccess) {
            delete ctx;
            PGV_FAIL(PGV_ERR_DEVICE, "hipStreamCreate failed: %s", hipGetErrorString(e));
        }
        ctx->own_stream = true;
    }
    if (hipEventCreate(&ctx->ev0) != hipSuccess || hipEventCreate(&ctx->ev1) != hipSuccess) {
        pgv_ctx_destroy(ctx);
        PGV_FAIL(PGV_ERR_DEVICE, "hipEventCreate failed");
    }
    *out = ctx;
    return PGV_OK;
}

void pgv_ctx_destroy(pgv_ctx *ctx) {
    if (!ctx) return;
    (void)hipSetDevice(ctx->device);
    (void)hipStreamSynchronize(ctx->stream);
    DBuf *d[] = {&ctx->q_stage, &ctx->rows_stage, &ctx->centers_stage, &ctx->out_stage,
                 &ctx->out_stage2, &ctx->idx_stage, &ctx->tasks, &ctx->pairs, &ctx->counters,
                 &ctx->plan_a, &ctx->plan_b, &ctx->plan_c, &ctx->plan_d, &ctx->dist_mat,
                 &ctx->sel_a, &ctx->sel_b, &ctx->km_a, &ctx->km_b, &ctx->km_c, &ctx->km_d,
                 &ctx->km_e, &ctx->km_f, &ctx->km_g, &ctx->stats_dev, &ctx->mf_a, &ctx->mf_b, &ctx->mf_c,
                 &ctx->zeros, &ctx->ms_a, &ctx->ms_b, &ctx->dense_plan, &ctx->xt_norms, &ctx->mf_d, &ctx->sh_q};
    for (DBuf *b : d) b->release();
    ctx->h_a.release();
    ctx->h_b.release();
    ctx->h_c.release();
    for (hipEvent_t e : ctx->ev_pool) (void)hipEventDestroy(e);
    if (ctx->h_a_busy) (void)hipEventDestroy(ctx->h_a_busy);
    if (ctx->ev0) (void)hipEventDestroy(ctx->ev0);
    if (ctx->ev1) (void)hipEventDestroy(ctx->ev1);
    if (ctx->own_stream && ctx->stream) (void)hipStreamDestroy(ctx->stream);
    delete ctx;
}

int pgv_ctx_sync(pgv_ctx *ctx) {
    if (!ctx) PGV_FAIL(PGV_ERR_ARG, "ctx is NULL");
    PGV_HIP(hipStreamSynchronize(ctx->stream));
    for (pgv_ctx *c : ctx->children) PGV_HIP(hipStreamSynchronize(c->stream));
    return PGV_OK;
}

void *pgv_ctx_stream(pgv_ctx *ctx) { return ctx ? (void *)ctx->stream : nullptr; }

int pgv_timer_start(pgv_ctx *ctx) {
    if (!ctx) PGV_FAIL(PGV_ERR_ARG, "ctx is NULL");
    PGV_HIP(hipEventRecord(ctx->ev0, ctx->stream));
    return PGV_OK;
}

int pgv_timer_stop(pgv_ctx *ctx, float *out_ms) {
    if (!ctx || !out_ms) PGV_FAIL(PGV_ERR_ARG, "ctx/out_ms is NULL");
    PGV_HIP(hipEventRecord(ctx->ev1, ctx->stream));
    PGV_HIP(hipEventSynchronize(ctx->ev1));
    PGV_HIP(hipEventElapsedTime(out_ms, ctx->ev0, ctx->ev1));
    return PGV_OK;
}

int pgv_ctx_set_profiling(pgv_ctx *ctx, int on) {
    if (!ctx) PGV_FAIL(PGV_ERR_ARG, "ctx is NULL");
    PGV_TRY(resolve_events(ctx));
    ctx->profiling = on != 0;
    if (ctx->profiling && !ctx->stats_dev.p) {
        PGV_TRY(ctx->stats_dev.ensure(8 * sizeof(double)));
        PGV_HIP(hipMemsetAsync(ctx->stats_dev.p, 0, 8 * sizeof(double), ctx->stream));
    }
    for (pgv_ctx *c : ctx->children) PGV_TRY(pgv_ctx_set_profiling(c, on));
    return PGV_OK;
}

int pgv_ctx_set_exact_scan(pgv_ctx *ctx, int on) {
    if (!ctx) PGV_FAIL(PGV_ERR_ARG, "pgv_ctx_set_exact_scan: ctx is NULL");
    ctx->no_mfma_scan = on != 0;
    for (pgv_ctx *c : ctx->children) c->no_mfma_scan = ctx->no_mfma_scan;
    return PGV_OK;
}

int pgv_ctx_set_bound(pgv_ctx *ctx, int mode) {
    if (!ctx) PGV_FAIL(PGV_ERR_ARG, "pgv_ctx_set_bound: ctx is NULL");
    if (mode != PGV_BOUND_STATISTICAL && mode != PGV_BOUND_WORST_CASE)
        PGV_FAIL(PGV_ERR_ARG, "pgv_ctx_set_bound: unknown mode %d", mode);
    ctx->bound_mode = mode;
    ctx->assign_bound_mode = mode;
    for (pgv_ctx *c : ctx->children) c->bound_mode = c->assign_bound_mode = mode;
    return PGV_OK;
}

int pgv_ctx_reset_stats(pgv_ctx *ctx) {
    if (!ctx) PGV_FAIL(PGV_ERR_ARG, "ctx is NULL");
    PGV_TRY(resolve_events(ctx));
    ctx->scan_ms = 0;
    ctx->scan_launches = 0;
    ctx->scan_pairs = 0;
    ctx->scan_rows = 0;
    if (ctx->stats_dev.p) PGV_HIP(hipMemsetAsync(ctx->stats_dev.p, 0, 8 * sizeof(double), ctx->stream));
    ctx->aux_ms = 0;
    ctx->aux_launches = 0;
    ctx->aux_pairs = 0;
    ctx->scan_shadow_queries = 0;
    for (pgv_ctx *c : ctx->children) PGV_TRY(pgv_ctx_reset_stats(c));
    return PGV_OK;
}

int pgv_ctx_get_stats(pgv_ctx *ctx, pgv_stats *out) {
    if (!ctx || !out) PGV_FAIL(PGV_ERR_ARG, "ctx/out is NULL");
    PGV_TRY(resolve_events(ctx));
    double dev_acc[8] = {0.0, 0.0, 0.0, 0.0, 0.0, 0.0, 0.0, 0.0};
    if (ctx->stats_dev.p) {
        PGV_HIP(hipMemcpyAsync(dev_acc, ctx->stats_dev.p, sizeof(dev_acc), hipMemcpyDeviceToHost, ctx->stream));
        PGV_HIP(hipStreamSynchronize(ctx->stream));
    }
    out->scan_ms = ctx->scan_ms;
    out->scan_launches = ctx->scan_launches;
    out->scan_pairs = ctx->scan_pairs + dev_acc[0];
    out->scan_rows = ctx->scan_rows + dev_acc[1];
    out->aux_ms = ctx->aux_ms;
    out->aux_launches = ctx->aux_launches;
    out->aux_pairs = ctx->aux_pairs;
    out->assign_redo_rows = dev_acc[2];
    out->assign_rows = dev_acc[3];
    out->assign_recheck_rows = dev_acc[4];
    out->scan_unique_rows = dev_acc[5];
    out->scan_redo_queries = dev_acc[6];
    out->scan_widened_queries = dev_acc[7];
    out->scan_shadow_queries = ctx->scan_shadow_queries;
    for (pgv_ctx *c : ctx->children) {
        pgv_stats cs;
        PGV_TRY(pgv_ctx_get_stats(c, &cs));
        out->scan_ms += cs.scan_ms;
        out->scan_launches += cs.scan_launches;
        out->scan_pairs += cs.scan_pairs;
        out->scan_rows += cs.scan_rows;
        out->aux_ms += cs.aux_ms;
        out->aux_launches += cs.aux_launches;
        out->aux_pairs += cs.aux_pairs;
        out->assign_redo_rows += cs.assign_redo_rows;
        out->assign_rows += cs.assign_rows;
        out->assign_recheck_rows += cs.assign_recheck_rows;
        out->scan_unique_rows += cs.scan_unique_rows;
        out->scan_redo_queries += cs.scan_redo_queries;
        out->scan_widened_queries += cs.scan_widened_queries;
        out->scan_shadow_queries += cs.scan_shadow_queries;
    }
    return PGV_OK;
}

}
```

pgvector_amd/csrc/pgv_abi_common.h:

```cpp
#pragma once

#include "pgv_internal.h"
#include "pgv_gate.h"
#include <dlfcn.h>
#include <linux/futex.h>
#include <sys/syscall.h>
#include <unistd.h>
#include <algorithm>
#include <cmath>
#include <cstdarg>
#include <new>

using namespace pgv;

namespace {

int check_common(pgv_dtype dtype, int dim) {
    if (dtype != PGV_F32 && dtype != PGV_F16) PGV_FAIL(PGV_ERR_ARG, "unknown dtype %d", (int)dtype);
    if (dim < 1 || dim > 16000) PGV_FAIL(PGV_ERR_DIMS, "dimensions %d outside 1..16000", dim);
    return PGV_OK;
}

int check_metric(pgv_metric m) {
    if (m != PGV_L2SQ && m != PGV_NEG_IP && m != PGV_L1) PGV_FAIL(PGV_ERR_ARG, "unknown metric %d", (int)m);
// ... 253 lines not shown
        PGV_TRY(launch_scan(ctx, v, queries_dev, w, qt, out_dev));
    PGV_TRY(timer.end());
    return PGV_OK;
}

struct Xoro {
    uint64_t s0, s1;
    static uint64_t rotl(uint64_t x, int k) { return (x << k) | (x >> (64 - k)); }
    static uint64_t splitmix(uint64_t &st) {
        uint64_t v = (st += 0x9E3779B97f4A7C15ull);
        v = (v ^ (v >> 30)) * 0xBF58476D1CE4E5B9ull;
        v = (v ^ (v >> 27)) * 0x94D049BB133111EBull;
        return v ^ (v >> 31);
    }
    explicit Xoro(uint64_t seed) {
        s0 = splitmix(seed);
        s1 = splitmix(seed);
        if (!s0 && !s1) s0 = 1;
    }
    uint64_t next() {
        uint64_t a = s0, x = s1 ^ a, out = rotl(a * 5, 7) * 9;
        s0 = rotl(a, 24) ^ x ^ (x << 16);
        s1 = rotl(x, 37);
        return out;
    }
};

struct Rng {
    const pgv_rng *user;
    Xoro own;
    explicit Rng(const pgv_rng *r) : user(r), own(r ? r->seed : 0) {}
    double next_double() {
        if (user && user->next_double) return user->next_double(user->state);
        return std::ldexp((double)(own.next() >> 12), -52);
    }
    uint32_t next_u32() {
        if (user && user->next_u32) return user->next_u32(user->state);
        return (uint32_t)(own.next() >> 32);
    }
};

struct KmppState {
    float *weight, *raw;
    double *block_sums, *draws_dev;
    int nblocks;
    int32_t *picked;
};

}

namespace {

static const size_t kExportGranule = (size_t)2 << 20;
static inline hipError_t malloc_exportable(void **p, size_t bytes) {
    const size_t rounded = (bytes + kExportGranule - 1) / kExportGranule * kExportGranule;
    return hipMalloc(p, rounded ? rounded : kExportGranule);
}

static int approx_candidates(int k) {
    if (k <= 8) return 32;
    if (4 * k > 256) return k + 64;
    int kp = 64;
    while (kp < 4 * k) kp <<= 1;
    return kp;
}

static bool spherical(pgv_ops ops) { return ops == PGV_OPS_IP || ops == PGV_OPS_COSINE; }

static RowsView kmeans_rows(pgv_ops ops, pgv_dtype dtype, const RowGeom &g, const void *s_dev, int n) {
    return {s_dev, n, g, row_kind(dtype), spherical(ops) ? PGV_NEG_IP : PGV_L2SQ};
}

static int check_ops(pgv_ops ops) {
    if (ops != PGV_OPS_L2 && ops != PGV_OPS_IP && ops != PGV_OPS_COSINE)
        PGV_FAIL(PGV_ERR_ARG, "unknown opclass family %d", (int)ops);
    return PGV_OK;
}

}

extern "C" {
int rank_lists_dev(pgv_index *ix, const void *q_dev, int nq, int maxprobes, int32_t *out_lists_dev, float *out_dist_dev);
int scan_batch_dev(pgv_index *ix, const void *q_dev, int nq, const int32_t *probe_lists, int probes, int k, float *out_dist,
                   int64_t *out_slot, uint64_t *out_tid);
int check_batch_args(pgv_index *ix, const void *queries, int nq, int probes, int k, float *out_dist, uint64_t *out_tid,
                     const char *who);
int kmpp_begin(pgv_ctx *ctx, int n_local, int k, int64_t n_total, Rng &rng, KmppState *state, int64_t *first);
int kmpp_round_weights(pgv_ctx *ctx, const RowsView &sv, const void *center_i, const KmppState &state);
int lloyd_partial_dev(pgv_ctx *ctx, pgv_ops ops, pgv_dtype dtype, const RowGeom &g, const void *samples_dev, int n,
                      const void *centers_dev, int k, int32_t *closest_io, float *sums, int32_t *counts,
                      unsigned long long *changes);
int lloyd_finish_dev(pgv_ctx *ctx, pgv_ops ops, pgv_dtype dtype, const RowGeom &g, int dim, int k, const float *sums_dev,
                     const int32_t *counts_dev, const int32_t *counts_host, Rng &rng, void *centers_dev);
int check_centers_dev(pgv_ctx *ctx, pgv_ops ops, pgv_dtype dtype, const RowGeom &g, int dim, int k, const void *centers_dev);
}
```

pgvector_amd/csrc/pgv_abi_ivf.hip:

```cpp
#include "pgv_abi_common.h"

extern "C" {


namespace {
struct IndexLayout {
    size_t centers, vectors, offsets, tids, row_norms, center_norms, bytes;
    bool has_tids, has_norms;
};
IndexLayout index_layout(int nlists, int64_t n, size_t row_bytes, bool has_tids, bool l2) {
    auto up = [](size_t v) { return (v + 255) & ~(size_t)255; };
    IndexLayout L{};
    size_t at = 0;
    L.centers = at; at = up(at + (size_t)nlists * row_bytes);
    L.vectors = at; at = up(at + (size_t)(n > 0 ? n : 1) * row_bytes);
    L.offsets = at; at = up(at + sizeof(int64_t) * ((size_t)nlists + 1));
    L.has_tids = has_tids;
    L.tids = at; if (has_tids) at = up(at + sizeof(uint64_t) * (size_t)n);
    L.has_norms = l2;
    L.row_norms = at; if (l2 && n > 0) at = up(at + sizeof(float) * ((size_t)n + 1));
    L.center_norms = at; if (l2) at = up(at + sizeof(float) * ((size_t)nlists + 1));
    L.bytes = at;
    return L;
}
void index_carve(pgv_index *ix, const IndexLayout &L) {
    char *b = static_cast<char *>(ix->arena);
    ix->centers = b + L.centers;
    ix->vectors = b + L.vectors;
    ix->list_offsets = reinterpret_cast<int64_t *>(b + L.offsets);
    ix->tids = L.has_tids ? reinterpret_cast<uint64_t *>(b + L.tids) : nullptr;
    ix->row_norms = L.has_norms && ix->nrows > 0 ? reinterpret_cast<float *>(b + L.row_norms) : nullptr;
    ix->center_norms = L.has_norms ? reinterpret_cast<float *>(b + L.center_norms) : nullptr;
}
void index_host_tables(pgv_index *ix) {
    const int nlists = ix->nlists;
    std::vector<int64_t> lens((size_t)nlists);
    int64_t maxlen = 0;
    for (int l = 0; l < nlists; l++) {
        lens[l] = ix->h_offsets[l + 1] - ix->h_offsets[l];
        if (lens[l] > maxlen) maxlen = lens[l];
    }
    ix->max_list_len = maxlen;
    std::sort(lens.begin(), lens.end(), [](int64_t a, int64_t b) { return a > b; });
    ix->len_prefix.assign((size_t)nlists + 1, 0);
    for (int l = 0; l < nlists; l++) ix->len_prefix[l + 1] = ix->len_prefix[l] + lens[l];
}
}

extern "C++" {
namespace {

int shadow_env() {
    const char *e = getenv("PGV_SCAN_SHADOW");
    return e ? atoi(e) : -1;
}

int rank_shadow_env() {
    const char *e = getenv("PGV_RANK_SHADOW");
    return e ? atoi(e) : 1;
}

int shadow_create(pgv_ctx *ctx, pgv_index *ix) {
    const int env = shadow_env();
    if (env == 0 || ix->metric != PGV_L2SQ || ix->dtype != PGV_F32 || ix->nrows <= 0 || !ix->row_norms || !ix->center_norms)
        return PGV_OK;
    if (env < 0 && !rows_stream_past_caches(ivf_rows(ix))) return PGV_OK;
    const RowGeom g16 = row_geom(ix->dim, PGV_F16);
    const size_t bytes = ((size_t)ix->nrows * g16.ld * sizeof(uint16_t) + 255) & ~(size_t)255;
    const size_t cbytes = ((size_t)ix->nlists * g16.ld * sizeof(uint16_t) + 255) & ~(size_t)255;
    void *sh = nullptr;
    if (hipMalloc(&sh, bytes + 256 + cbytes) != hipSuccess) {
        (void)hipGetLastError();
        return PGV_OK;
    }
    void *words = static_cast<char *>(sh) + bytes;
    void *csh = static_cast<char *>(sh) + bytes + 256;
    int rc = launch_shadow_build(ctx, ix->geom, g16, ix->vectors, ix->centers, ix->list_offsets, ix->nlists, ix->nrows, sh,
                                 words);
    if (rc == PGV_OK)
        rc = launch_shadow_build(ctx, ix->geom, g16, ix->centers, nullptr, nullptr, 0, ix->nlists, csh,
                                 static_cast<char *>(words) + 32);
    unsigned char h[56];
    if (rc == PGV_OK && (hipStreamSynchronize(ctx->stream) != hipSuccess ||
                         hipMemcpy(h, words, sizeof(h), hipMemcpyDeviceToHost) != hipSuccess)) {
        set_error("shadow build failed: %s", hipGetErrorString(hipGetLastError()));
        rc = PGV_ERR_DEVICE;
    }
    if (rc != PGV_OK) {
        (void)hipFree(sh);
        return rc;
    }
    float max_abs;
    double e2, p2;
    memcpy(&max_abs, h, 4);
    memcpy(&e2, h + 8, 8);
    memcpy(&p2, h + 16, 8);
    const double P = std::sqrt(p2), E = std::sqrt(e2);
    if (!std::isfinite(E) || !std::isfinite(P) || !std::isfinite(max_abs)) {
        (void)hipFree(sh);
        return PGV_OK;
    }
    ix->shadow = sh;
    ix->shadow_geom = g16;
    ix->shadow_s = shadow_scale_of(max_abs);
    ix->shadow_E = (E + 1e-12 * (P + E)) * (1.0 + 1e-9);
    ix->shadow_P = P * (1.0 + 1e-9);
    float cmax_abs;
    double ce2, cp2;
    memcpy(&cmax_abs, h + 32, 4);
    memcpy(&ce2, h + 40, 8);
    memcpy(&cp2, h + 48, 8);
    const double Pc = std::sqrt(cp2), Ec = std::sqrt(ce2);
    if (std::isfinite(Ec) && std::isfinite(Pc) && std::isfinite(cmax_abs)) {
        ix->cshadow = csh;
        ix->cshadow_s = shadow_scale_of(cmax_abs);
        ix->cshadow_E = (Ec + 1e-12 * (Pc + Ec)) * (1.0 + 1e-9);
        ix->cshadow_P = Pc * (1.0 + 1e-9);
    }
    return PGV_OK;
}

struct ShadowBatch {
    void *qcast = nullptr;
    float *qscale = nullptr, *qeps = nullptr;
    float *cscale = nullptr, *ceps = nullptr;
    float *pair_t = nullptr;
    bool scan_follows = false;
    bool cast_for_scan = false;
    bool pairs_done = false;
};

int shadow_batch_cast(pgv_index *ix, const void *q_dev, int nq, int probes, bool for_rank, bool for_scan, ShadowBatch *sb) {
    pgv_ctx *ctx = ix->ctx;
    const RowGeom &g16 = ix->shadow_geom;
    const size_t qb = ((size_t)nq * g16.ld * sizeof(uint16_t) + 255) & ~(size_t)255;
    PGV_TRY(ctx->sh_q.ensure(qb + sizeof(float) * (size_t)nq * (4 + (size_t)probes)));
    sb->qcast = ctx->sh_q.p;
    sb->qscale = reinterpret_cast<float *>(ctx->sh_q.as<char>() + qb);
    sb->qeps = sb->qscale + nq;
    sb->cscale = sb->qeps + nq;
    sb->ceps = sb->cscale + nq;
    sb->pair_t = sb->ceps + nq;
    constexpr double u = 5.9604644775390625e-8;
    ShadowTerms st{};
    st.s = ix->shadow_s;
    st.E = ix->shadow_E;
    st.P = ix->shadow_P;
    st.g_dot = gamma_n(shadow_chain_length(g16) + 4.0, u);
    st.g_pair = gamma_n((double)pair_chain_length(ix->geom), u);
    st.g_cn = shadow_band(ix->geom.ld, 0.f, u).g_norm;
    RankShadowTerms rt{};
    rt.s = ix->cshadow_s;
    rt.E = ix->cshadow_E;
    rt.P = ix->cshadow_P;
    rt.g_dot = st.g_dot;
    rt.g_cn = st.g_cn;
    PGV_TRY(launch_shadow_query(ctx, ix->geom, g16, q_dev, nq, st, rt, ix->center_norms + ix->nlists,
                                ix->row_norms + ix->nrows, sb->qcast, for_scan ? sb->qscale : nullptr,
                                for_scan ? sb->qeps : nullptr, for_rank ? sb->cscale : nullptr,
                                for_rank ? sb->ceps : nullptr));
    sb->cast_for_scan = for_scan;
    return PGV_OK;
}

struct IndexElem {
    pgv_metric metric;
    pgv_dtype dtype;
    int dim, nbits;
    static IndexElem bits(int nbits) { return {PGV_L1, PGV_F32, nbits, nbits}; }
    size_t tight_bytes() const { return nbits > 0 ? (size_t)(nbits + 7) / 8 : (size_t)dim * elem_size(dtype); }
};

template <typename Fill>
int index_create(pgv_ctx *ctx, const IndexElem &el, int nlists, const std::vector<int64_t> &off, bool has_tids, Fill fill,
                 pgv_index **out) {
    const pgv_metric metric = el.metric;
    const int nbits = el.nbits;
    const int64_t n = off[nlists];
    pgv_index *ix = new (std::nothrow) pgv_index();
    if (!ix) PGV_FAIL(PGV_ERR_NOMEM, "out of host memory");
    ix->ctx = ctx;
    ix->refs = new (std::nothrow) int(1);
    if (!ix->refs) {
        delete ix;
        PGV_FAIL(PGV_ERR_NOMEM, "out of host memory");
    }
    ix->metric = metric;
    ix->dtype = el.dtype;
    ix->dim = el.dim;
    ix->nlists = nlists;
    ix->nrows = n;
    ix->nbits = nbits;
    ix->geom = nbits > 0 ? bit_row_geom(nbits) : row_geom(el.dim, el.dtype);
    ix->h_offsets = off;
    index_host_tables(ix);

    auto fail = [&](int rc) {
        pgv_index_free(ix);
        return rc;
    };
    IndexLayout lay = index_layout(nlists, n, ivf_rows(ix).row_bytes(), has_tids && n > 0, metric == PGV_L2SQ && nbits == 0);
    if (malloc_exportable(&ix->arena, lay.bytes) != hipSuccess) {
        (void)hipGetLastError();
        set_error("hipMalloc(%zu) for the index mirror failed", lay.bytes);
        return fail(PGV_ERR_NOMEM);
    }
    ix->arena_bytes = lay.bytes;
    index_carve(ix, lay);
    int rc;
    if ((rc = fill(ix)) != PGV_OK) return fail(rc);
// ... 538 lines not shown
    }
    if (ix->arena) {
        if (ix->imported)
            (void)hipIpcCloseMemHandle(ix->arena);
        else
            (void)hipFree(ix->arena);
    }
    if (ix->shadow) (void)hipFree(ix->shadow);
    delete ix->refs;
    delete ix;
}

int pgv_index_tids(pgv_index *ix, const int64_t *slots, int64_t n, uint64_t *out) {
    if (!ix || !out || (n > 0 && !slots)) PGV_FAIL(PGV_ERR_ARG, "pgv_index_tids: index/slots/out is NULL");
    if (!ix->tids) PGV_FAIL(PGV_ERR_STATE, "pgv_index_tids: the index was uploaded without tids");
    if (is_device_ptr(slots) || is_device_ptr(out)) PGV_FAIL(PGV_ERR_ARG, "pgv_index_tids: host arrays only");
    PGV_HIP(hipSetDevice(ix->ctx->device));
    int64_t i = 0;
    while (i < n) {
        if (slots[i] < 0 || slots[i] >= ix->nrows) PGV_FAIL(PGV_ERR_ARG, "pgv_index_tids: slot %lld out of range", (long long)slots[i]);
        int64_t j = i + 1;
        while (j < n && slots[j] == slots[j - 1] + 1) j++;
        if (slots[j - 1] >= ix->nrows) PGV_FAIL(PGV_ERR_ARG, "pgv_index_tids: slot %lld out of range", (long long)slots[j - 1]);
        PGV_HIP(hipMemcpyAsync(out + i, ix->tids + slots[i], sizeof(uint64_t) * (size_t)(j - i), hipMemcpyDeviceToHost,
                               ix->ctx->stream));
        i = j;
    }
    PGV_HIP(hipStreamSynchronize(ix->ctx->stream));
    return PGV_OK;
}

int64_t pgv_index_rows(const pgv_index *ix) { return ix ? ix->nrows : -1; }
int pgv_index_lists(const pgv_index *ix) { return ix ? ix->nlists : -1; }

static int rank_lists_impl(pgv_index *ix, const void *q_dev, int nq, int maxprobes,
                           int32_t *out_lists_dev, float *out_dist_dev, ShadowBatch *sb) {
    pgv_ctx *ctx = ix->ctx;
    PGV_TRY(ctx->dist_mat.ensure(sizeof(float) * (size_t)nq * ix->nlists));
    float *mat = ctx->dist_mat.as<float>();
    PGV_TRY(ctx->sel_a.ensure(sizeof(int64_t) * (size_t)nq * maxprobes));
    float *dist = out_dist_dev;
    if (!dist) {
        PGV_TRY(ctx->sel_b.ensure(sizeof(float) * (size_t)nq * maxprobes));
        dist = ctx->sel_b.as<float>();
    }
    int64_t *pos = ctx->sel_a.as<int64_t>();
    if (ix->nbits > 0) {
        ScanTimer timer{ctx};
        PGV_TRY(timer.begin((double)ix->nlists * nq, (double)ix->nlists * ((nq + 31) / 32), true));
        PGV_TRY(launch_hamming_tiles(ctx, ivf_centers(ix), q_dev, bit_query_bytes(ix->nbits), nq, mat));
        PGV_TRY(timer.end());
        PGV_TRY(launch_topk_segments(ctx, mat, nullptr, nq, ix->nlists, maxprobes, dist, pos));
        return launch_cast_pos_to_i32(ctx, pos, (int64_t)nq * maxprobes, out_lists_dev);
    }
    if (nq <= 24 && maxprobes <= query_head_cap()) {
        const int64_t cd_stride = ((int64_t)ix->nlists + 7) / 4 * 4;
        PGV_TRY(ctx->dist_mat.ensure(sizeof(float) * (size_t)nq * cd_stride));
        return launch_multi_rank(ctx, ix, q_dev, nq, ctx->dist_mat.as<float>(), cd_stride, maxprobes, out_lists_dev,
                                 out_dist_dev);
    }
    int cand = maxprobes + 16 < ix->nlists ? maxprobes + 16 : ix->nlists;
    const int rank_env = rank_shadow_env();
    const bool rank_sh = ix->metric == PGV_L2SQ && ix->cshadow && ix->dtype == PGV_F32 && rank_env != 0 && shadow_env() != 0;
    if (rank_sh && maxprobes + 54 <= 256) cand = maxprobes + 54 < ix->nlists ? maxprobes + 54 : ix->nlists;
    const bool mfma = nq >= 128 && ix->nlists >= 64 && !ctx->no_mfma_scan &&
                      (ix->metric == PGV_NEG_IP || (ix->metric == PGV_L2SQ && ix->center_norms && cand <= 256));
    if (mfma && ix->metric == PGV_L2SQ) {
        ShadowBatch own;
        if (!sb) sb = &own;
        const bool scan_follows = sb->scan_follows;
        if (rank_sh) {
            PGV_TRY(shadow_batch_cast(ix, q_dev, nq, maxprobes, true, scan_follows, sb));
            PGV_TRY(dense_scan(ctx, ivf_shadow_centers(ix), sb->qcast, nq, ix->nlists, mat, true, ix->center_norms, nullptr,
                               sb->cscale));
        } else {
            PGV_TRY(dense_scan(ctx, ivf_centers(ix), q_dev, nq, ix->nlists, mat, true, ix->center_norms, nullptr));
        }
        ExactTail tail;
        tail.pair_t = (rank_sh && rank_env == 1 && scan_follows) ? sb->pair_t : nullptr;
        PlanBuffers pbuf;
        if (tail.pair_t) {
            PGV_TRY(plan_batch_reserve(ctx, ix->nlists, nq, maxprobes, &pbuf));
            tail.emit = {pbuf.cnt, pbuf.probe_off, pbuf.seg_len, ix->list_offsets};
        }
        tail.rows = {ix->centers, nullptr, nullptr, ix->geom, ix->dtype,
                     reinterpret_cast<const unsigned *>(ix->center_norms + ix->nlists)};
        tail.queries = q_dev;
        tail.nq = nq;
        tail.kprime = cand;
        tail.k = maxprobes;
        tail.approx = mat;
        tail.fixed_len = ix->nlists;
        tail.bound = scan_bound_chain(ctx, ix->geom.ld, scan_chain_length(ix->geom, ix->dtype, false));
        if (rank_sh) tail.bound = shadow_band(ix->geom.ld, tail.bound.g_ref);
        tail.eps_add = rank_sh ? sb->ceps : nullptr;
        tail.out_dist = dist;
        tail.out_i32 = out_lists_dev;
        PGV_TRY(launch_exact_tail(ctx, tail, ctx->ms_b));
        sb->pairs_done = tail.pair_t != nullptr;
        return PGV_OK;
    } else {
        PGV_TRY(dense_scan(ctx, ivf_centers(ix), q_dev, nq, ix->nlists, mat, mfma, nullptr, nullptr));
        PGV_TRY(launch_topk_segments(ctx, mat, nullptr, nq, ix->nlists, maxprobes, dist, pos));
    }
    PGV_TRY(launch_cast_pos_to_i32(ctx, pos, (int64_t)nq * maxprobes, out_lists_dev));
    return PGV_OK;
}

int rank_lists_dev(pgv_index *ix, const void *q_dev, int nq, int maxprobes, int32_t *out_lists_dev, float *out_dist_dev) {
    return rank_lists_impl(ix, q_dev, nq, maxprobes, out_lists_dev, out_dist_dev, nullptr);
}

int pgv_rank_lists(pgv_index *ix, const void *queries, int nq, int maxprobes, int32_t *out_lists,
                   float *out_dist) {
    if (!ix || !out_lists) PGV_FAIL(PGV_ERR_ARG, "pgv_rank_lists: index/out_lists is NULL");
    if (nq < 0) PGV_FAIL(PGV_ERR_ARG, "nq < 0");
    if (maxprobes < 1 || maxprobes > ix->nlists)
        PGV_FAIL(PGV_ERR_ARG, "maxprobes %d outside 1..lists (%d)", maxprobes, ix->nlists);
    if (nq == 0) return PGV_OK;
    if (!queries) PGV_FAIL(PGV_ERR_ARG, "queries is NULL");
    pgv_ctx *ctx = ix->ctx;
    PGV_HIP(hipSetDevice(ctx->device));
    const void *q_dev;
    PGV_TRY(stage_queries(ix, queries, nq, &q_dev));
    OutArg ol, od;
    PGV_TRY(ol.init(out_lists, sizeof(int32_t) * (size_t)nq * maxprobes, ctx->out_stage));
    PGV_TRY(od.init(out_dist, sizeof(float) * (size_t)nq * maxprobes, ctx->out_stage2));
    PGV_TRY(rank_lists_dev(ix, q_dev, nq, maxprobes, ol.as<int32_t>(), od.as<float>()));
    bool need = false;
    PGV_TRY(ol.finish(ctx, &need));
    PGV_TRY(od.finish(ctx, &need));
    return sync_if(ctx, need);
}

static int scan_turn_begin(pgv_ctx *ctx) {
    if (ctx->scan_gate) PGV_HIP(hipStreamWaitEvent(ctx->stream, ctx->scan_gate, 0));
    return PGV_OK;
}
static int scan_turn_end(pgv_ctx *ctx) {
    if (ctx->scan_gate) PGV_HIP(hipEventRecord(ctx->scan_gate, ctx->stream));
    return PGV_OK;
}

struct ScanPath {
    bool bits = false;
    bool per_query = false;
    bool use_mfma = false;
    bool use_tile = false;
    bool wide = false;
    int qt = 0, rows_per_task = 0;
    bool approx = false;
    bool shadow = false;
};
static ScanPath scan_path(const pgv_index *ix, int nq, int probes, int k) {
    ScanPath p;
    const double share = (double)nq * probes / (double)ix->nlists;
    if (ix->nbits > 0) {
        p.bits = true;
        p.qt = hamming_list_group_size(share);
        p.rows_per_task = hamming_list_rows_per_task();
        return p;
    }
    p.per_query = (share <= 0.4 || nq <= 4) && nq <= 1024 && probes <= query_max_batch_lists() && k <= query_head_cap();
    if (p.per_query) return p;
    p.use_mfma = share > 3.0 && k <= 192 && !ix->ctx->no_mfma_scan &&
                 (ix->metric == PGV_NEG_IP || (ix->metric == PGV_L2SQ && ix->row_norms));
    p.use_tile = !p.use_mfma && tile_scan_supported(ix->geom) && share > 8.0;
    static const int wide_env = [] {
        const char *e = getenv("PGV_SCAN_WIDE");
        return e ? atoi(e) : -1;
    }();
    p.wide = p.use_mfma && (wide_env < 0 ? share > 12.0 : wide_env != 0);
    p.qt = p.use_mfma ? (p.wide ? mfma_scan_queries_per_task_wide() : mfma_scan_queries_per_task())
                      : (p.use_tile ? tile_scan_queries_per_task()
                                    : scan_group_size(ix->geom, ix->dtype, (int)std::ceil(share)));
    constexpr int rpt_tiles = 20;
    p.rows_per_task = p.use_mfma ? mfma_scan_rows_per_task()
                                 : (p.use_tile ? rpt_tiles * tile_scan_tile_rows(ix->geom)
                                               : (p.qt >= 16 ? 256 : (p.qt >= 4 ? 128 : 64)));
    p.approx = p.use_mfma && ix->metric == PGV_L2SQ;
    p.shadow = p.approx && ix->shadow && shadow_env() != 0;
    return p;
}

static int list_scan_step(pgv_index *ix, const ScanPath &path, const ScanWork &work, const void *queries, const float *qscale,
                          double counted, float *out) {
    pgv_ctx *ctx = ix->ctx;
    const RowsView v = path.shadow ? ivf_shadow_rows(ix) : ivf_rows(ix);
    PGV_TRY(scan_turn_begin(ctx));
    ScanTimer timer{ctx};
    PGV_TRY(timer.begin(counted, counted));
    if (path.bits)
        PGV_TRY(launch_hamming_lists(ctx, v, queries, bit_query_bytes(ix->nbits), work, path.qt, out));
    else if (path.use_mfma)
        PGV_TRY(launch_mfma_scan(ctx, v, queries, work, ix->row_norms, nullptr, out, rows_stream_past_caches(v), path.qt,
                                 path.shadow ? qscale : nullptr));
    else if (path.use_tile)
        PGV_TRY(launch_tile_scan(ctx, v, queries, work, out));
    else
        PGV_TRY(launch_scan(ctx, v, queries, work, path.qt, out));
    PGV_TRY(timer.end());
    return scan_turn_end(ctx);
}

static int scan_batch_impl(pgv_index *ix, const void *q_dev, int nq, const int32_t *probe_lists, int probes,
                           int k, float *out_dist, int64_t *out_slot, uint64_t *out_tid, ShadowBatch *sb) {
    pgv_ctx *ctx = ix->ctx;
    const ScanPath path = scan_path(ix, nq, probes, k);
    if (path.per_query) {
        const int64_t bound = ix->len_prefix[probes];
        const int64_t seg_stride = (bound + 7) / 4 * 4;
        PGV_TRY(ctx->plan_d.ensure(sizeof(float) * (size_t)nq * seg_stride));
        OutArg od, os, ot;
        PGV_TRY(od.init(out_dist, sizeof(float) * (size_t)nq * k, ctx->out_stage));
        PGV_TRY(os.init(out_slot, sizeof(int64_t) * (size_t)nq * k, ctx->out_stage2));
        PGV_TRY(ot.init(out_tid, sizeof(uint64_t) * (size_t)nq * k, ctx->sel_b));
        PGV_TRY(scan_turn_begin(ctx));
        ScanTimer timer{ctx};
        PGV_TRY(timer.begin(0.0, 0.0));
        PGV_TRY(launch_multi_scan(ctx, ix, q_dev, nq, probe_lists, probes, bound, ctx->plan_d.as<float>(), seg_stride, k,
                                  od.as<float>(), os.as<int64_t>(), ot.as<uint64_t>()));
        PGV_TRY(timer.end());
        PGV_TRY(scan_turn_end(ctx));
        bool need = false;
        PGV_TRY(od.finish(ctx, &need));
        PGV_TRY(os.finish(ctx, &need));
        PGV_TRY(ot.finish(ctx, &need));
        return sync_if(ctx, need);
    }
    ShadowBatch own;
    if (!sb) sb = &own;
    if (path.shadow && !sb->cast_for_scan) PGV_TRY(shadow_batch_cast(ix, q_dev, nq, probes, false, true, sb));
    const float *pair_t = (path.shadow && sb->pairs_done) ? sb->pair_t : nullptr;
    PlanResult plan;
    PGV_TRY(launch_plan_batch(ctx, ix, probe_lists, nq, probes, path.qt, path.rows_per_task, ctx->profiling, &plan, pair_t,
                              pair_t != nullptr));
    if (path.shadow) {
        if (!pair_t)
            PGV_TRY(launch_shadow_pairs(ctx, ix->geom, q_dev, ix->centers, plan.pair_start, ix->nlists, (int64_t)nq * probes,
                                        plan.pairs));
        ctx->scan_shadow_queries += nq;
    }

    PGV_TRY(ctx->plan_d.ensure(sizeof(float) * (size_t)(plan.out_bound > 0 ? plan.out_bound : 1)));
    float *seg_vals = ctx->plan_d.as<float>();
    if (plan.ntasks_bound > 0)
        PGV_TRY(list_scan_step(ix, path, plan.work(), path.shadow ? sb->qcast : q_dev, sb->qscale, 0.0, seg_vals));

    OutArg od, os, ot;
    PGV_TRY(od.init(out_dist, sizeof(float) * (size_t)nq * k, ctx->out_stage));
    PGV_TRY(os.init(out_slot, sizeof(int64_t) * (size_t)nq * k, ctx->out_stage2));
    PGV_TRY(ot.init(out_tid, sizeof(uint64_t) * (size_t)nq * k, ctx->sel_b));
    PGV_TRY(ctx->sel_a.ensure(sizeof(int64_t) * (size_t)nq * k));
    int64_t *pos = ctx->sel_a.as<int64_t>();
    if (path.approx) {
        ExactTail tail;
        tail.rows = {ix->vectors, ix->tids, ix->list_offsets, ix->geom, ix->dtype,
                     reinterpret_cast<const unsigned *>(ix->row_norms + ix->nrows)};
        tail.queries = q_dev;
        tail.nq = nq;
        tail.kprime = approx_candidates(k);
        tail.k = k;
        tail.approx = seg_vals;
        tail.probe_lists = probe_lists;
        tail.probe_off = plan.probe_off;
        tail.probes = probes;
        tail.seg_start = plan.seg_start;
        tail.seg_bound = ix->len_prefix[probes];
        tail.bound = scan_bound_chain(ctx, ix->geom.ld, scan_chain_length(ix->geom, ix->dtype, path.wide));
        if (path.shadow) tail.bound = shadow_band(ix->geom.ld, tail.bound.g_ref);
        tail.eps_add = path.shadow ? sb->qeps : nullptr;
        tail.out_dist = od.as<float>();
        tail.out_slot = os.as<int64_t>();
        tail.out_tid = ot.as<uint64_t>();
        PGV_TRY(launch_exact_tail(ctx, tail, ctx->ms_a));
    } else {
        PGV_TRY(launch_topk_segments(ctx, seg_vals, plan.seg_start, nq, 0, k, od.as<float>(), pos, nullptr, nullptr, 0,
                                     ix->len_prefix[probes]));
        PGV_TRY(launch_positions_to_slots(ctx, ix, probe_lists, plan.probe_off, nq, probes, k, pos,
                                          os.as<int64_t>(), ot.as<uint64_t>()));
    }
    bool need = false;
    PGV_TRY(od.finish(ctx, &need));
    PGV_TRY(os.finish(ctx, &need));
    PGV_TRY(ot.finish(ctx, &need));
    return sync_if(ctx, need);
}

int scan_batch_dev(pgv_index *ix, const void *q_dev, int nq, const int32_t *probe_lists, int probes, int k, float *out_dist,
                   int64_t *out_slot, uint64_t *out_tid) {
    return scan_batch_impl(ix, q_dev, nq, probe_lists, probes, k, out_dist, out_slot, out_tid, nullptr);
}

int pgv_scan_lists(pgv_index *ix, const void *query, const int32_t *lists, int nlists,
                   float *out_dist, int64_t *out_slot, int64_t capacity, int64_t *out_count) {
    if (!ix || !out_count) PGV_FAIL(PGV_ERR_ARG, "pgv_scan_lists: index/out_count is NULL");
    if (nlists < 0 || (nlists > 0 && !lists)) PGV_FAIL(PGV_ERR_ARG, "bad list array");
    pgv_ctx *ctx = ix->ctx;
    PGV_HIP(hipSetDevice(ctx->device));

    std::vector<int32_t> hl((size_t)nlists);
    if (nlists) {
        if (is_device_ptr(lists))
            PGV_HIP(hipMemcpy(hl.data(), lists, sizeof(int32_t) * (size_t)nlists, hipMemcpyDeviceToHost));
        else
            memcpy(hl.data(), lists, sizeof(int32_t) * (size_t)nlists);
    }
    int64_t m = 0;
    for (int p = 0; p < nlists; p++) {
        if (hl[p] < 0 || hl[p] >= ix->nlists) PGV_FAIL(PGV_ERR_ARG, "list id %d out of range", hl[p]);
        m += ix->h_offsets[hl[p] + 1] - ix->h_offsets[hl[p]];
    }
    *out_count = m;
    if (m > capacity) PGV_FAIL(PGV_ERR_ARG, "output capacity %lld < %lld tuples", (long long)capacity, (long long)m);
    if (m == 0) return PGV_OK;
    if (!out_dist || !out_slot) PGV_FAIL(PGV_ERR_ARG, "out_dist/out_slot is NULL");

    OutArg od, os;
    PGV_TRY(od.init(out_dist, sizeof(float) * (size_t)m, ctx->out_stage));
    PGV_TRY(os.init(out_slot, sizeof(int64_t) * (size_t)m, ctx->out_stage2));

    ScanPath path;
    path.bits = ix->nbits > 0;
    path.qt = path.bits ? hamming_list_group_size(1.0) : 1;
    path.rows_per_task = path.bits ? hamming_list_rows_per_task() : rows_per_task_for(ctx, m, 1);
    const int ch = path.rows_per_task;
    int64_t ntasks = 0;
    for (int p = 0; p < nlists; p++) {
        int64_t len = ix->h_offsets[hl[p] + 1] - ix->h_offsets[hl[p]];
        ntasks += (len + ch - 1) / ch;
    }
    const size_t tb = sizeof(ScanTask) * (size_t)ntasks, pb = sizeof(ScanPair) * (size_t)nlists,
                 ob = sizeof(int64_t) * (size_t)nlists, lb = sizeof(int32_t) * (size_t)nlists;
    PGV_TRY(staging_acquire(ctx));
    PGV_TRY(ctx->h_a.ensure(tb + pb + ob + lb + 16));
    char *hb = ctx->h_a.as<char>();
    ScanTask *ht = reinterpret_cast<ScanTask *>(hb);
    ScanPair *hp = reinterpret_cast<ScanPair *>(hb + tb);
    int64_t *hoff = reinterpret_cast<int64_t *>(hb + tb + pb);
    int32_t *hlist = reinterpret_cast<int32_t *>(hb + tb + pb + ob);
    int *hn = reinterpret_cast<int *>(hb + tb + pb + ob + lb);
    int64_t t = 0, run = 0;
    for (int p = 0; p < nlists; p++) {
        const int64_t beg = ix->h_offsets[hl[p]], len = ix->h_offsets[hl[p] + 1] - beg;
        hp[p].out_rel = run - beg;
        hp[p].query = 0;
        hp[p].pad = 0;
        hoff[p] = run;
        hlist[p] = hl[p];
        for (int64_t c = 0; c * ch < len; c++) {
            ht[t].row0 = beg + c * ch;
            int64_t left = len - c * ch;
            ht[t].nrows = (int)(left < ch ? left : ch);
            ht[t].pair0 = p;
            ht[t].npairs = 1;
            ht[t].pad = 0;
            t++;
        }
        run += len;
    }
    *hn = (int)ntasks;
    const size_t total = tb + pb + ob + lb + 16;
    PGV_TRY(ctx->tasks.ensure(total));
    PGV_HIP(hipMemcpyAsync(ctx->tasks.p, hb, total, hipMemcpyHostToDevice, ctx->stream));
    char *db = ctx->tasks.as<char>();

    PGV_TRY(launch_iota_slots(ctx, ix, reinterpret_cast<int32_t *>(db + tb + pb + ob), nlists,
                              reinterpret_cast<int64_t *>(db + tb + pb), os.as<int64_t>()));
    if (query == nullptr) {
        PGV_HIP(hipMemsetAsync(od.dev, 0, sizeof(float) * (size_t)m, ctx->stream));
    } else {
        const void *q_dev;
        PGV_TRY(stage_queries(ix, query, 1, &q_dev));
        const ScanWork work{reinterpret_cast<ScanTask *>(db), reinterpret_cast<int *>(db + tb + pb + ob + lb), (int)ntasks,
                            reinterpret_cast<ScanPair *>(db + tb)};
        PGV_TRY(list_scan_step(ix, path, work, q_dev, nullptr, (double)m, od.as<float>()));
    }
    bool need = true;
    PGV_TRY(od.finish(ctx, &need));
    PGV_TRY(os.finish(ctx, &need));
    return sync_if(ctx, need);
}

int check_batch_args(pgv_index *ix, const void *queries, int nq, int probes, int k, float *out_dist,
                            uint64_t *out_tid, const char *who) {
    if (!ix) PGV_FAIL(PGV_ERR_ARG, "%s: index is NULL", who);
    if (nq < 0 || k < 1) PGV_FAIL(PGV_ERR_ARG, "bad nq/k");
    if (probes < 1 || probes > ix->nlists)
        PGV_FAIL(PGV_ERR_ARG, "probes %d outside 1..lists (%d)", probes, ix->nlists);
    if (out_tid && !ix->tids) PGV_FAIL(PGV_ERR_STATE, "index was uploaded without tids");
    if (nq > 0 && (!queries || !out_dist)) PGV_FAIL(PGV_ERR_ARG, "queries/out_dist is NULL");
    return PGV_OK;
}

int pgv_search_batch(pgv_index *ix, const void *queries, int nq, int probes, int k, float *out_dist,
                     int64_t *out_slot, uint64_t *out_tid) {
    PGV_TRY(check_batch_args(ix, queries, nq, probes, k, out_dist, out_tid, "pgv_search_batch"));
    if (nq == 0) return PGV_OK;
    if (!ix->lanes.empty()) {
        pgv_index *lane = ix->lanes[ix->lane_next++ % ix->lanes.size()];
        PGV_HIP(hipSetDevice(ix->ctx->device));
        PGV_HIP(hipEventRecord(ix->lane_event, ix->ctx->stream));
        PGV_HIP(hipStreamWaitEvent(lane->ctx->stream, ix->lane_event, 0));
        return pgv_search_batch(lane, queries, nq, probes, k, out_dist, out_slot, out_tid);
    }
    pgv_ctx *ctx = ix->ctx;
    PGV_HIP(hipSetDevice(ctx->device));
    const void *q_dev;
    PGV_TRY(stage_queries(ix, queries, nq, &q_dev));
    PGV_TRY(ctx->idx_stage.ensure(sizeof(int32_t) * (size_t)nq * probes));
    int32_t *probe_lists = ctx->idx_stage.as<int32_t>();
    ShadowBatch sb;
    sb.scan_follows = scan_path(ix, nq, probes, k).shadow;
    PGV_TRY(rank_lists_impl(ix, q_dev, nq, probes, probe_lists, nullptr, &sb));
    return scan_batch_impl(ix, q_dev, nq, probe_lists, probes, k, out_dist, out_slot, out_tid, &sb);
}

int pgv_scan_batch(pgv_index *ix, const void *queries, int nq, const int32_t *probe_lists, int probes, int k,
                   float *out_dist, int64_t *out_slot, uint64_t *out_tid) {
    PGV_TRY(check_batch_args(ix, queries, nq, probes, k, out_dist, out_tid, "pgv_scan_batch"));
    if (nq == 0) return PGV_OK;
    if (!probe_lists) PGV_FAIL(PGV_ERR_ARG, "probe_lists is NULL");
    pgv_ctx *ctx = ix->ctx;
    PGV_HIP(hipSetDevice(ctx->device));
    if (!is_device_ptr(probe_lists)) {
        for (size_t i = 0; i < (size_t)nq * probes; i++)
            if (probe_lists[i] < 0 || probe_lists[i] >= ix->nlists)
                PGV_FAIL(PGV_ERR_ARG, "probe list id %d out of range 0..%d", probe_lists[i], ix->nlists - 1);
    }
    const void *q_dev, *pl_dev;
    PGV_TRY(stage_queries(ix, queries, nq, &q_dev));
    PGV_TRY(stage_flat(ctx, probe_lists, sizeof(int32_t) * (size_t)nq * probes, ctx->idx_stage, &pl_dev));
    return scan_batch_dev(ix, q_dev, nq, static_cast<const int32_t *>(pl_dev), probes, k, out_dist, out_slot,
                          out_tid);
}

int pgv_index_shadow_cast(pgv_index *ix, const void *queries, int nq, void *out_qcast, float *out_qscale, float *out_qeps,
                          float *out_cscale, float *out_ceps) {
    if (!ix || !queries || nq < 1) PGV_FAIL(PGV_ERR_ARG, "pgv_index_shadow_cast: index/queries is NULL or nq < 1");
    PGV_NO_BIT_INDEX(ix, "pgv_index_shadow_cast");
    if (!ix->shadow || !ix->cshadow) PGV_FAIL(PGV_ERR_STATE, "pgv_index_shadow_cast: the index has no fp16 shadow");
    pgv_ctx *ctx = ix->ctx;
    PGV_HIP(hipSetDevice(ctx->device));
    const void *q_dev;
    PGV_TRY(stage_rows(ctx, queries, nq, ix->dim, ix->dtype, ix->geom, ctx->q_stage, &q_dev));
    ShadowBatch sb;
    PGV_TRY(shadow_batch_cast(ix, q_dev, nq, 1, true, true, &sb));
    const struct {
        void *dst;
        const void *src;
        size_t bytes;
    } parts[] = {{out_qcast, sb.qcast, (size_t)nq * ix->shadow_geom.ld * sizeof(uint16_t)},
                 {out_qscale, sb.qscale, sizeof(float) * (size_t)nq},
                 {out_qeps, sb.qeps, sizeof(float) * (size_t)nq},
                 {out_cscale, sb.cscale, sizeof(float) * (size_t)nq},
                 {out_ceps, sb.ceps, sizeof(float) * (size_t)nq}};
    for (const auto &p : parts)
        if (p.dst) PGV_HIP(hipMemcpyAsync(p.dst, p.src, p.bytes, hipMemcpyDefault, ctx->stream));
    PGV_HIP(hipStreamSynchronize(ctx->stream));
    return PGV_OK;
}

namespace {

struct QueryHeadHost {
    long long total;
    int count;
    unsigned seq;
};

static int g_scan_gate_width = -1;
static PgvGate g_scan_gate;
static void scan_gate_enter() {
    if (g_scan_gate_width < 0) {
        const char *e = getenv("PGV_MAX_INFLIGHT_SCANS");
        __atomic_store_n(&g_scan_gate_width, e ? atoi(e) : 16, __ATOMIC_RELAXED);
    }
    g_scan_gate.enter(g_scan_gate_width);
}
static void scan_gate_leave() { g_scan_gate.leave(g_scan_gate_width); }
struct ScanGate {
    ScanGate() { scan_gate_enter(); }
    ~ScanGate() { scan_gate_leave(); }
};

int wait_head(pgv_ctx *ctx, pgv_query *q, unsigned seq) {
    volatile QueryHeadHost *h = static_cast<volatile QueryHeadHost *>(q->head_pinned);
    for (int spin = 0; spin < 200000; spin++) {
        if (__atomic_load_n(&h->seq, __ATOMIC_ACQUIRE) == seq) return PGV_OK;
        __builtin_ia32_pause();
    }
    PGV_HIP(hipStreamSynchronize(ctx->stream));
    if (__atomic_load_n(&h->seq, __ATOMIC_ACQUIRE) != seq) PGV_FAIL(PGV_ERR_DEVICE, "query kernel did not report");
    return PGV_OK;
}

void copy_head(pgv_query *q, int stride, int n, float *out_dist, int64_t *out_slot, uint64_t *out_tid) {
    const char *base = static_cast<const char *>(q->head_pinned) + 64;
    if (out_slot) memcpy(out_slot, base, sizeof(int64_t) * (size_t)n);
    if (out_tid) memcpy(out_tid, base + (size_t)stride * 8, sizeof(uint64_t) * (size_t)n);
    if (out_dist) memcpy(out_dist, base + (size_t)stride * 16, sizeof(float) * (size_t)n);
}

}

static bool query_direct_enabled() {
    static const bool on = [] {
        const char *e = getenv("PGV_QUERY_DIRECT");
        return !(e && e[0] == '0');
    }();
    return on;
}

int pgv_query_begin(pgv_index *ix, pgv_query **out) {
    if (!ix || !out) PGV_FAIL(PGV_ERR_ARG, "pgv_query_begin: index/out is NULL");
    *out = nullptr;
    PGV_NO_BIT_INDEX(ix, "pgv_query_begin");
// ... 148 lines not shown
```

pgvector_amd/csrc/pgv_internal.h:

```cpp
#pragma once

#include <hip/hip_runtime.h>

#include <cstdint>
#include <cstdio>
#include <cstdlib>
#include <cstring>
#include <cmath>
#include <vector>

#include "../../include/pgv_hip.h"

namespace pgv {

void set_error(const char *fmt, ...) __attribute__((format(printf, 1, 2)));

#define PGV_FAIL(code, ...)            \
    do {                               \
        ::pgv::set_error(__VA_ARGS__); \
        return (code);                 \
    } while (0)

#define PGV_HIP(call)                                                                  \
    do {                                                                               \
// ... 6 lines not shown
    } while (0)

#define PGV_TRY(call)          \
    do {                       \
        int rc__ = (call);     \
        if (rc__ != PGV_OK)    \
            return rc__;       \
    } while (0)

struct DBuf {
    void *p = nullptr;
    size_t cap = 0;
    int ensure(size_t bytes);
    void release();
    template <typename T> T *as() const { return static_cast<T *>(p); }
};

struct HBuf {
    void *p = nullptr;
    size_t cap = 0;
    int ensure(size_t bytes);
    void release();
    template <typename T> T *as() const { return static_cast<T *>(p); }
};

bool is_device_ptr(const void *p);

constexpr int kVecBytes = 16;

constexpr int kHnswMaxBits = 64000;
constexpr int kIvfMaxBits = 64000;

inline int elem_size(pgv_dtype t) { return t == PGV_F32 ? 4 : 2; }
inline int padded_dim(int dim, pgv_dtype t) {
    int per = kVecBytes / elem_size(t);
    return (dim + per - 1) / per * per;
}

struct RowGeom {
    int ld;
    int nvec;
    int lpr_log2;
    int nchunks;
};
RowGeom row_geom(int dim, pgv_dtype t);
RowGeom bit_row_geom(int nbits);

enum class RowKind { F32, F16, Bits };
struct RowsView {
    const void *rows;
    int64_t n;
    RowGeom geom;
    RowKind kind;
    pgv_metric metric;
    bool bits() const { return kind == RowKind::Bits; }
    pgv_dtype dtype() const { return kind == RowKind::F16 ? PGV_F16 : PGV_F32; }
    size_t row_bytes() const { return bits() ? (size_t)geom.ld : (size_t)geom.ld * elem_size(dtype()); }
};
inline RowKind row_kind(pgv_dtype t) { return t == PGV_F16 ? RowKind::F16 : RowKind::F32; }

struct HnswGraph {
    void *mem = nullptr;
    size_t bytes = 0;
    const int32_t *levels = nullptr;
    const int64_t *nbr_start = nullptr;
    int32_t *nbr = nullptr;
    int64_t nbr_total = 0;
    int m = 0;
    int32_t entry = -1;
};

struct ScanTask {
    int64_t row0;
    int32_t nrows;
    int32_t pair0;
    int32_t npairs;
    int32_t pad;
};
struct ScanPair {
    int64_t out_rel;
    int32_t query;
    int32_t pad;
};
struct ScanWork {
    const ScanTask *tasks;
    const int *ntasks_dev;
    int ntasks_bound;
    const ScanPair *pairs;
};

}

struct pgv_ctx {
    int device = 0;
    hipStream_t stream = nullptr;
    bool own_stream = false;
    int num_cus = 256;
    hipEvent_t ev0 = nullptr, ev1 = nullptr;
    pgv::DBuf q_stage, rows_stage, centers_stage, out_stage, out_stage2, idx_stage;
    pgv::DBuf tasks, pairs, counters, plan_a, plan_b, plan_c, plan_d, dist_mat, sel_a, sel_b;
    pgv::DBuf km_a, km_b, km_c, km_d, km_e, km_f, km_g;
    pgv::DBuf ms_b;
    pgv::DBuf dense_plan;
    int64_t dense_plan_rows = -1, dense_plan_stride = -1;
    int dense_plan_nq = -1, dense_plan_kind = -1;
    bool counters_clean = false;
    pgv::DBuf ms_a;
    pgv::DBuf sh_q;
    pgv::DBuf mf_d;
    pgv::DBuf mf_a, mf_b, mf_c, zeros;
    pgv::DBuf stats_dev;
    pgv::HBuf h_a, h_b, h_c;
    hipEvent_t h_a_busy = nullptr;
    bool h_a_pending = false;
    bool profiling = false;
    bool no_mfma_scan = false;
    bool no_widen = false;
    int bound_mode = 1;
    int assign_bound_mode = 1;
    pgv::DBuf xt_norms;
    std::vector<hipEvent_t> ev_pool;
    size_t ev_used = 0;
    double scan_ms = 0.0;
    int64_t scan_launches = 0;
    double scan_pairs = 0.0;
    double scan_rows = 0.0;
    std::vector<char> ev_is_aux;
    double aux_ms = 0.0;
    int64_t aux_launches = 0;
    double aux_pairs = 0.0;
    double scan_shadow_queries = 0.0;
    std::vector<pgv_ctx *> children;
    hipEvent_t scan_gate = nullptr;
};

struct pgv_index {
    pgv_ctx *ctx = nullptr;
    pgv_metric metric = PGV_L2SQ;
    pgv_dtype dtype = PGV_F32;
    int dim = 0;
    int nbits = 0;
    int nlists = 0;
    int64_t nrows = 0;
    pgv::RowGeom geom{};
    void *centers = nullptr;
    void *vectors = nullptr;
    int64_t *list_offsets = nullptr;
    uint64_t *tids = nullptr;
    float *row_norms = nullptr;
    float *center_norms = nullptr;
    int *refs = nullptr;
    void *arena = nullptr;
    size_t arena_bytes = 0;
    bool imported = false;
    void *shadow = nullptr;
    pgv::RowGeom shadow_geom{};
    int shadow_s = 0;
    double shadow_E = 0.0;
    double shadow_P = 0.0;
    void *cshadow = nullptr;
    int cshadow_s = 0;
    double cshadow_E = 0.0;
    double cshadow_P = 0.0;
    std::vector<int64_t> h_offsets;
    std::vector<int64_t> len_prefix;
    int64_t max_list_len = 0;
    std::vector<pgv_index *> lanes;
    unsigned lane_next = 0;
    hipEvent_t lane_event = nullptr;
    hipEvent_t lane_scan_done = nullptr;
};

struct pgv_query {
    pgv_index *ix = nullptr;
    pgv::DBuf state;
    pgv::DBuf seg;
    pgv::DBuf q_dev;
    void *q_pinned = nullptr;
    const void *q_row = nullptr;
    void *q_direct = nullptr;
    void *head_pinned = nullptr;
    size_t head_bytes = 0;
    int32_t *lists = nullptr;
    float *cdist = nullptr;
    int max_probes = 0;
    bool is_null = false;
    bool rank_pending = false;
    int cur_first = 0, cur_n = 0;
    unsigned seq = 0;
};

struct HnswElements {
    pgv_metric metric = PGV_L2SQ;
    pgv_dtype dtype = PGV_F32;
    int dim = 0;
    int nbits = 0;
    int64_t n = 0;
    pgv::RowGeom geom{};
    void *elements = nullptr;
    char *payload = nullptr;
    int payload_bytes = 0;
};

struct pgv_hnsw : HnswElements {
    pgv_ctx *ctx = nullptr;
    pgv::HnswGraph graph;
    pgv::DBuf bitmaps;
    bool imported = false;
    pgv_hnsw *view_of = nullptr;
    hipEvent_t graph_ev = nullptr;
    bool graph_ev_set = false;
    struct HnswLinkState *link = nullptr;
};

namespace pgv {
inline RowsView hnsw_rows(const pgv_hnsw *h) {
    return {h->elements, h->n, h->geom, h->nbits > 0 ? RowKind::Bits : row_kind(h->dtype), h->metric};
}
inline RowsView ivf_rows(const pgv_index *ix) {
    return {ix->vectors, ix->nrows, ix->geom, ix->nbits > 0 ? RowKind::Bits : row_kind(ix->dtype), ix->metric};
}
inline RowsView ivf_centers(const pgv_index *ix) {
    RowsView v = ivf_rows(ix);
    v.rows = ix->centers;
    v.n = ix->nlists;
    return v;
}
inline RowsView ivf_shadow_rows(const pgv_index *ix) { return {ix->shadow, ix->nrows, ix->shadow_geom, RowKind::F16, ix->metric}; }
inline RowsView ivf_shadow_centers(const pgv_index *ix) {
    return {ix->cshadow, ix->nlists, ix->shadow_geom, RowKind::F16, ix->metric};
}
}

struct HnswLinkState {
    float *nb_dist = nullptr;
    uint8_t *nb_flag = nullptr;
    int *list_count = nullptr;
    int *list_rec = nullptr;
    size_t nlists = 0;
    int64_t *stats_dev = nullptr, *stats_host = nullptr;
    pgv::DBuf rec, links, ids, pa, pb, tri, mm, loc, sel;
    int nrec = 0, nq = 0, lcap = 0;
    int64_t npairs = 0;
    bool prepared = false;
    int32_t *rec_owner = nullptr, *rec_lc = nullptr, *rec_nstart = nullptr, *rec_from = nullptr, *rec_wait = nullptr,
            *rec_list = nullptr;
    int64_t *rec_off = nullptr, *rec_pos = nullptr, *ids_start = nullptr, *pair_start = nullptr, *mm_start = nullptr,
            *totals = nullptr;
    int *rec_fill = nullptr, *blocked = nullptr, *nrec_dev = nullptr;
    int32_t *d_link_elem = nullptr;
    float *d_link_dist = nullptr;
    int32_t *d_sel_ids = nullptr, *d_sel_cnt = nullptr, *d_elems = nullptr;
    float *d_sel_dist = nullptr;
    uint8_t *d_sel_closer = nullptr, *d_linked = nullptr;
    struct Kept {
        pgv::DBuf ids, dist, cnt, elems;
        int nq = 0, ef = 0, lcap = 0;
    } kept[2];
};

namespace pgv {

struct ScanBound {
    float g_sq, g_dot, g_norm, g_ref;
};
struct ShadowTerms {
    int s;
    double E, P;
    double g_dot, g_pair, g_cn;
};
struct RankShadowTerms {
    int s;
    double E, P;
    double g_dot, g_cn;
};
inline float gamma_n(double n, double v) { return (float)(n * v / (1.0 - n * v)); }
inline int pair_chain_length(const RowGeom &g32) {
    const int by_pair_kernel = (g32.ld + 63) / 64 + 6;
    const int per_lane = (g32.nvec + (1 << g32.lpr_log2) - 1) >> g32.lpr_log2;
    const int by_recheck = 4 * ((per_lane + 1) / 2) + 1 + g32.lpr_log2;
    return by_pair_kernel > by_recheck ? by_pair_kernel : by_recheck;
}
inline ScanBound scan_bound(const pgv_ctx *ctx, int dim) {
    if (ctx->bound_mode == 0) return {8.f * std::sqrt((float)dim + 4.f) * 5.9604645e-8f, 0.f, 0.f, 0.f};
    constexpr double v = 5.9604645e-8;
    return {0.f, gamma_n(dim / 4.0 + 4.0, v), gamma_n(dim / 64.0 + 10.0, v), 2.f * gamma_n(dim + 2.0, v)};
}
inline ScanBound scan_bound_chain(const pgv_ctx *ctx, int dim, int chain) {
    ScanBound b = scan_bound(ctx, dim);
    if (ctx->bound_mode != 0) b.g_dot = gamma_n(chain + 4.0, 5.9604645e-8);
    return b;
}
inline ScanBound shadow_band(int ld, float g_ref, double u = 5.9604645e-8) {
    return {0.f, 0.f, gamma_n(ld / 64.0 + 10.0, u), g_ref};
}
struct ExpansionBound {
    float gamma;
    float gamma_exact;
};
inline ExpansionBound argmin_bound(const pgv_ctx *ctx, int dim) {
    constexpr float u = 5.9604645e-8f;
    if (ctx->assign_bound_mode == 0) return {8.f * std::sqrt((float)dim + 4.f) * u, 0.f};
    const float n1 = (float)(dim + 1) * u, n2 = (float)(dim + 2) * u;
    return {n1 / (1.f - n1), n2 / (1.f - n2)};
}

int launch_scan(pgv_ctx *ctx, const RowsView &v, const void *queries, const ScanWork &w, int qt, float *out);
int scan_group_size(const RowGeom &g, pgv_dtype dtype, int wanted);
int launch_score_gather(pgv_ctx *ctx, const RowsView &v, const void *queries, const int32_t *slot, const int32_t *query_of,
                        int64_t npairs, float *out);
int launch_score_groups(pgv_ctx *ctx, const RowsView &v, const int32_t *ids, const int64_t *ids_at, int64_t ids_stride,
                        const int32_t *n_arr, const int32_t *from_arr, const int64_t *pair_at, int ngroups, float *out);
int launch_expand_groups(pgv_ctx *ctx, const int32_t *ids, const int64_t *ids_at, int64_t ids_stride, const int32_t *n_arr,
                         const int32_t *from_arr, const int64_t *pair_at, int ngroups, int32_t *a, int32_t *b);

int launch_cosine(pgv_ctx *ctx, pgv_dtype dtype, const RowGeom &g, const void *rows, const void *query, int64_t n,
                  double *out);
int launch_bit_distance(pgv_ctx *ctx, int mode, const RowGeom &g, const void *rows, const void *query, int64_t n,
                        double *out);

int bit_topk_slice_bytes();
inline int bit_query_bytes(int nbits) {
    const int slice = bit_topk_slice_bytes();
    return ((nbits + 7) / 8 + slice - 1) / slice * slice;
}
int launch_hamming_tiles(pgv_ctx *ctx, const RowsView &v, const void *queries, int qbytes, int nq, float *out);
int hamming_list_group_size(double queries_per_list);
int hamming_list_rows_per_task();
int launch_hamming_lists(pgv_ctx *ctx, const RowsView &v, const void *queries, int qbytes, const ScanWork &w, int qt,
                         float *out);
int launch_bit_closest(pgv_ctx *ctx, const float *mat, int k, const float *best_val, const int64_t *best_pos, int n,
                       bool sticky, int32_t *closest_io, float *out_dist, int32_t *counts, unsigned long long *changes);
int launch_bit_sums(pgv_ctx *ctx, const void *samples, int ld, int nbits, int n, const int32_t *closest, int32_t *sums);
int launch_bit_centers(pgv_ctx *ctx, const int32_t *sums, const int32_t *counts, int k, int nbits, int ld,
                       const int32_t *refill_row, const uint8_t *refill, void *centers);
int launch_binary_quantize(pgv_ctx *ctx, pgv_dtype dtype, int dim, const void *rows, int64_t n, void *out_bits);
int launch_rerank_pairs(pgv_ctx *ctx, const int64_t *cand, int64_t total, int kc, int32_t *slot, int32_t *query_of);
int launch_rerank_mask(pgv_ctx *ctx, const int64_t *cand, int64_t total, float *vals);
int launch_rerank_map(pgv_ctx *ctx, const int64_t *cand, int nq, int kc, int k, const int64_t *pos, int64_t *out_idx);

struct SparseCsr {
    const int64_t *ptr;
    const int32_t *idx;
    const float *val;
    int64_t n;
};
struct SparseTile {
    int64_t elem0;
    int32_t q0, nq, nnz, pad;
};
int sparse_tile_nnz();
int sparse_tile_queries();
int sparse_reg_row_nnz();
void sparse_plan_tiles(const int64_t *q_ptr, int nq, std::vector<SparseTile> *tiles, int *max_q_nnz);
int launch_sparse_tiles(pgv_ctx *ctx, int mode, const SparseTile *tiles_dev, int ntiles, int max_tile_nnz, int max_tile_nq,
                        int max_q_nnz, const SparseCsr &q, const SparseCsr &r, void *out, int64_t out_stride);

int hnsw_search_grid(pgv_ctx *ctx, int nq, int64_t n, int *words_out);
struct HnswSearchArgs {
    const void *queries = nullptr;
    const int32_t *qids = nullptr;
    const int32_t *qlevels = nullptr;
    int nq = 0, ef = 0, k = 0;
    int64_t *out_elem = nullptr;
    float *out_dist = nullptr;
    int64_t *out_scored = nullptr;
    int32_t *lw_ids = nullptr;
    float *lw_dist = nullptr;
    int32_t *lw_cnt = nullptr;
    int lcap = 0;
};
int launch_hnsw_search(pgv_ctx *ctx, const RowsView &v, const HnswGraph &graph, const HnswSearchArgs &a, uint32_t *bitmaps,
                       int words, int grid, int *counter);
int launch_hnsw_patch(pgv_ctx *ctx, const HnswGraph &graph, int64_t n, const int32_t *ids, const int64_t *packed_off,
                      const int32_t *packed, int nupd);

bool tile_scan_supported(const RowGeom &g);
int tile_scan_queries_per_task();
int tile_scan_tile_rows(const RowGeom &g);
int launch_tile_scan(pgv_ctx *ctx, const RowsView &v, const void *queries, const ScanWork &w, float *out);

int launch_argmin(pgv_ctx *ctx, pgv_metric metric, pgv_dtype dtype, const RowGeom &g,
                  const void *rows, int64_t n, const void *centers, int k, int32_t *out_idx,
                  float *out_val);
int launch_argmin_mode(pgv_ctx *ctx, int mode, pgv_dtype dtype, const RowGeom &g,
                       const void *rows, int64_t n, const void *centers, int k,
                       int32_t *out_idx, float *out_val);

int launch_argmin_listed(pgv_ctx *ctx, int mode, pgv_dtype dtype, const RowGeom &g, const void *rows, int64_t n,
                         const void *centers, int k, const int32_t *row_list, const int *row_count,
                         unsigned long long *packed);
int launch_hnsw_select_plan(pgv_ctx *ctx, const int32_t *cnt, int ngroups, int lcap, int m, int64_t *pair_start);
int launch_hnsw_select(pgv_ctx *ctx, const int32_t *lw_ids, const float *lw_dist, const int32_t *cnt, const int32_t *qlevels,
                       const int64_t *pair_start, const float *tri, int ngroups, int lcap, int ef, int m, int stride,
                       int32_t *out_ids, float *out_dist, uint8_t *out_closer, int32_t *out_cnt);
int launch_hnsw_link_group(pgv_ctx *ctx, int step, const HnswGraph &graph, const int32_t *elems, const uint8_t *linked, int nq,
                           int lcap, const int32_t *sel_ids, const float *sel_dist, const int32_t *sel_cnt, int *list_count,
                           int *list_rec, int *nrec, int32_t *rec_owner, int32_t *rec_lc, int32_t *rec_list,
                           const int64_t *rec_off, int *rec_fill, int32_t *link_elem, float *link_dist);
int launch_hnsw_link_size(pgv_ctx *ctx, const HnswGraph &graph, const uint8_t *nb_flag, const int32_t *rec_owner,
                          const int32_t *rec_lc, const int32_t *rec_list, const int *list_count, int64_t *rec_off, int nrec,
                          int pass, int64_t *rec_pos, int32_t *rec_nstart, int32_t *rec_from, const int32_t *rec_wait,
                          int64_t *size_ids, int64_t *size_pairs);
int launch_hnsw_link_scan(pgv_ctx *ctx, int64_t *a, int64_t *b, int64_t *c, int n, int64_t *totals);
int launch_hnsw_link_stats(pgv_ctx *ctx, const int *blocked, const int64_t *totals, int64_t *stats);
int launch_hnsw_link_pairs(pgv_ctx *ctx, const int32_t *nbr, const int64_t *rec_pos, const int32_t *rec_nstart,
                           const int32_t *rec_from, const int64_t *rec_off, int32_t *link_elem, float *link_dist,
                           const int32_t *rec_list, int *list_count, int nrec, int pass,
                           const int64_t *ids_start, int32_t *ids, const int64_t *pair_start, int32_t *a, int32_t *b);
int launch_hnsw_link_replay(pgv_ctx *ctx, const HnswGraph &graph, float *nb_dist, uint8_t *nb_flag, int nrec, int pass,
                            const int32_t *rec_lc, const int64_t *rec_off, const float *link_dist, const int64_t *rec_pos,
                            const int32_t *rec_nstart, const int32_t *rec_from, const int64_t *ids_start, const int32_t *ids,
                            const int64_t *pair_start, const float *tri, const int64_t *mm_start, const float *mm,
                            int32_t *rec_wait, int16_t *loc_save, int *blocked);
int launch_hnsw_link_new(pgv_ctx *ctx, const HnswGraph &graph, float *nb_dist, uint8_t *nb_flag, const int32_t *elems,
                         const uint8_t *linked, int nq, int lcap, const int32_t *sel_ids, const float *sel_dist,
                         const uint8_t *sel_closer, const int32_t *sel_cnt);
bool mfma_argmin_supported(int mode, int64_t n, int k);
int launch_argmin_mfma(pgv_ctx *ctx, int mode, pgv_dtype dtype, const RowGeom &g, const void *rows, int64_t n,
                       const void *centers, int k, int32_t *out_idx, float *out_val);

int mfma_scan_rows_per_task();
int mfma_scan_queries_per_task();
int launch_mfma_dense(pgv_ctx *ctx, pgv_metric metric, pgv_dtype dtype, const RowGeom &g, const void *rows, int64_t n,
                      const void *queries, int nq, const float *row_norms, float *out, int64_t out_stride);
int dense_chain_length(const RowGeom &g, pgv_dtype dtype);
int launch_row_norms(pgv_ctx *ctx, const RowsView &v, float *out, unsigned *max_bits);
int launch_mfma_scan(pgv_ctx *ctx, const RowsView &v, const void *queries, const ScanWork &w, const float *row_norms,
                     const float *query_norms, float *out, bool stream_rows, int queries_per_task = 32,
                     const float *shadow_scale = nullptr);
int launch_shadow_build(pgv_ctx *ctx, const RowGeom &g32, const RowGeom &g16, const void *rows, const void *centers,
                        const int64_t *list_off, int nlists, int64_t n, void *shadow, void *words);
int shadow_scale_of(float max_abs);
int shadow_chain_length(const RowGeom &g16);
int scan_chain_length(const RowGeom &g, pgv_dtype dtype, bool wide);
int launch_shadow_query(pgv_ctx *ctx, const RowGeom &g32, const RowGeom &g16, const void *queries, int nq,
                        const ShadowTerms &st, const RankShadowTerms &rt, const float *center_norm_max,
                        const float *row_norm_max, void *qcast, float *qscale, float *qeps, float *cscale, float *ceps);
int launch_shadow_pairs(pgv_ctx *ctx, const RowGeom &g32, const void *queries, const void *centers,
                        const int64_t *pair_start, int nlists, int64_t npairs, ScanPair *pairs);
int mfma_scan_queries_per_task_wide();

int launch_gather_words(pgv_ctx *ctx, const void *src, int words_per_row, int64_t nrows, const int64_t *idx, int n,
                        uint32_t *out);
size_t build_sort_scratch_bytes(int64_t n, int key_bits);
int launch_build_order(pgv_ctx *ctx, const int32_t *lists, int64_t n, int nlists, unsigned long long *keys_tmp,
                       unsigned long long *keys_sorted, unsigned long long *counts, int64_t *offsets, int *bad,
                       void *sort_scratch, size_t sort_scratch_bytes);
int launch_build_gather(pgv_ctx *ctx, const void *src_rows, const unsigned long long *keys_sorted, int64_t n, int nvec,
                        void *dst_rows, const uint64_t *src_tids, uint64_t *dst_tids);

struct PlanResult {
    ScanTask *tasks = nullptr;
    ScanPair *pairs = nullptr;
    int *ntasks_dev = nullptr;
    int64_t ntasks = 0;
    int64_t total_out = 0;
    int64_t ntasks_bound = 0;
    int64_t out_bound = 0;
    int64_t *seg_start = nullptr;
    int64_t *probe_off = nullptr;
    int64_t *pair_start = nullptr;
    ScanWork work() const { return {tasks, ntasks_dev, (int)ntasks_bound, pairs}; }
};
struct PlanBuffers {
    int *cnt = nullptr, *fill = nullptr;
    int64_t *probe_off = nullptr, *seg_len = nullptr;
    int64_t *seg_start = nullptr, *pair_start = nullptr, *task_start = nullptr, *totals = nullptr;
};
int plan_batch_reserve(pgv_ctx *ctx, int nlists, int nq, int probes, PlanBuffers *pb);
struct PlanEmit {
    int *cnt = nullptr;
    int64_t *probe_off = nullptr, *seg_len = nullptr;
    const int64_t *list_off = nullptr;
};
int launch_plan_batch(pgv_ctx *ctx, const pgv_index *ix, const int32_t *probe_lists, int nq,
                      int probes, int qt, int rows_per_task, bool read_totals, PlanResult *res,
                      const float *pair_t = nullptr, bool counted = false);
int launch_topk_segments(pgv_ctx *ctx, const float *vals, const int64_t *seg_start, int nseg,
                         int64_t fixed_len, int k, float *out_val, int64_t *out_pos, int32_t *zero_word = nullptr,
                         int32_t *zero_range = nullptr, int zero_n = 0, int64_t len_bound = 0);
int launch_positions_to_slots(pgv_ctx *ctx, const pgv_index *ix, const int32_t *probe_lists,
                              const int64_t *probe_off, int nq, int probes, int k,
                              const int64_t *pos, int64_t *out_slot, uint64_t *out_tid);
struct ExactRows {
    const void *vectors;
    const uint64_t *tids;
    const int64_t *list_offsets;
    pgv::RowGeom geom;
    pgv_dtype dtype;
    const unsigned *norm_max;
};
struct ExactTail {
    ExactRows rows;
    const void *queries = nullptr;
    int nq = 0;
    int kprime = 0;
    int k = 0;
    float *approx = nullptr;
    const int32_t *probe_lists = nullptr;
    const int64_t *probe_off = nullptr;
    int probes = 0;
    const int64_t *seg_start = nullptr;
    int64_t seg_bound = 0;
    int64_t fixed_len = 0;
    ScanBound bound{};
    const float *eps_add = nullptr;
    float *out_dist = nullptr;
    int64_t *out_slot = nullptr;
    uint64_t *out_tid = nullptr;
    int32_t *out_i32 = nullptr;
    float *pair_t = nullptr;
    PlanEmit emit;
    bool dense() const { return probe_lists == nullptr; }
};
int launch_exact_tail(pgv_ctx *ctx, const ExactTail &t, DBuf &scratch);
int launch_iota_slots(pgv_ctx *ctx, const pgv_index *ix, const int32_t *lists_dev, int nlists,
                      const int64_t *probe_off, int64_t *out_slot);

int query_max_batch_lists();
int query_head_cap();
size_t query_head_bytes(int head);
int launch_query_stage(pgv_ctx *ctx, const void *src_pinned, void *dst_dev, int nvec);
int launch_multi_rank(pgv_ctx *ctx, const pgv_index *ix, const void *q_dev, int nq, float *cdist, int64_t cd_stride,
                      int max_probes, int32_t *out_lists, float *out_dist);
int launch_multi_scan(pgv_ctx *ctx, const pgv_index *ix, const void *q_dev, int nq, const int32_t *probe_lists, int nprobes,
                      int64_t rows_bound, float *seg, int64_t seg_stride, int k, float *out_dist, int64_t *out_slot,
                      uint64_t *out_tid);
int launch_query_iota(pgv_ctx *ctx, int32_t *out, int n);
int launch_one_query_rows(pgv_ctx *ctx, const RowsView &v, const void *q_dev, float *out);
int launch_query_rank(pgv_ctx *ctx, const pgv_index *ix, const void *q_dev, float *cdist, int max_probes,
                      int32_t *out_lists);
int launch_query_scan(pgv_ctx *ctx, const pgv_index *ix, const void *q_dev, const int32_t *probe_lists, int nprobes,
                      int64_t rows_bound, float *seg);
int launch_query_head(pgv_ctx *ctx, const pgv_index *ix, const float *seg, const int32_t *probe_lists, int nprobes,
                      int skip, int count, void *head_rec, unsigned seq);

int launch_merge_heads(pgv_ctx *ctx, const float *dist_all, const uint64_t *tid_all, int nranks, int nq, int k,
                       float *out_dist, uint64_t *out_tid);

int launch_cast_pos_to_i32(pgv_ctx *ctx, const int64_t *pos, int64_t n, int32_t *out);

int kmpp_block_count(int n);
int launch_kmpp_update(pgv_ctx *ctx, const float *raw, float *weight, int n, int spherical,
                       double *block_sums);
int launch_kmpp_pick(pgv_ctx *ctx, const RowGeom &g, const void *samples, int n,
                     const float *weight, const double *block_sums, const double *draws,
                     int round, void *centers, int32_t *picked);
int launch_kmpp_total(pgv_ctx *ctx, const double *block_sums, int nblocks, double *out);
int launch_kmpp_pick_sharded(pgv_ctx *ctx, const RowGeom &g, const void *samples, int n, const float *weight,
                             const double *block_sums, const double *totals, const int64_t *counts, int nranks, int rank,
                             const double *draws, int round, void *send_row, int32_t *owner_out);
int launch_kmpp_take_row(pgv_ctx *ctx, const RowGeom &g, const void *gathered, const int32_t *owner, void *centers,
                         int round);
int launch_lloyd_pack(pgv_ctx *ctx, const int32_t *counts, const unsigned long long *changes, int k, float *tail);
int launch_lloyd_unpack(pgv_ctx *ctx, const float *tail, int k, int32_t *counts, unsigned long long *changes,
                        long long *host_rec, long long seq);
int launch_changes_hist(pgv_ctx *ctx, const int32_t *closest_new, int32_t *closest_io, int n,
// ... 15 lines not shown
```

Baseline: 1.402 million.

## Prune probed lists whose radius bound proves they cannot hold top-k

Computes a per-list radius at shadow build time and, during ranking or just before the scan plan, drops probed lists whose lower distance bound (center distance minus radius) exceeds an upper bound on the k-th neighbour given by nearer lists covering k rows. Dropped probes are marked -1 and skipped in planning, so fewer rows get scanned. This adds a prune step with block syncs, extra radius storage and a new stats counter. It also risks no savings when the triangle-inequality bounds are loose in 1536 dimensions.

```diff
diff --git a/include/pgv_hip.h b/include/pgv_hip.h
--- a/include/pgv_hip.h
+++ b/include/pgv_hip.h
@@ -85,6 +85,7 @@
 	double		scan_unique_rows;
 	double		scan_redo_queries;
 	double		scan_widened_queries;
+	double		scan_pruned_probes;
 	double		scan_shadow_queries;
 }			pgv_stats;
 int			pgv_ctx_set_profiling(pgv_ctx * ctx, int on);
diff --git a/pgvector_amd/_lib.py b/pgvector_amd/_lib.py
--- a/pgvector_amd/_lib.py
+++ b/pgvector_amd/_lib.py
@@ -48,6 +48,7 @@
                 ("scan_pairs", C.c_double), ("scan_rows", C.c_double),
                 ("aux_ms", C.c_double), ("aux_launches", C.c_int64), ("aux_pairs", C.c_double),
                 ("assign_redo_rows", C.c_double), ("assign_rows", C.c_double), ("assign_recheck_rows", C.c_double), ("scan_unique_rows", C.c_double), ("scan_redo_queries", C.c_double), ("scan_widened_queries", C.c_double),
+                ("scan_pruned_probes", C.c_double),
                 ("scan_shadow_queries", C.c_double)]
 
 
diff --git a/pgvector_amd/api.py b/pgvector_amd/api.py
--- a/pgvector_amd/api.py
+++ b/pgvector_amd/api.py
@@ -117,7 +117,8 @@
                 "aux_ms": s.aux_ms, "aux_launches": s.aux_launches, "aux_pairs": s.aux_pairs,
                 "assign_redo_rows": s.assign_redo_rows, "assign_rows": s.assign_rows,
                 "assign_recheck_rows": s.assign_recheck_rows, "scan_unique_rows": s.scan_unique_rows, "scan_redo_queries": s.scan_redo_queries,
-                "scan_widened_queries": s.scan_widened_queries, "scan_shadow_queries": s.scan_shadow_queries}
+                "scan_widened_queries": s.scan_widened_queries, "scan_pruned_probes": s.scan_pruned_probes,
+                "scan_shadow_queries": s.scan_shadow_queries}
 
 
 class IvfIndex:
diff --git a/pgvector_amd/csrc/kernels_query.hip b/pgvector_amd/csrc/kernels_query.hip
--- a/pgvector_amd/csrc/kernels_query.hip
+++ b/pgvector_amd/csrc/kernels_query.hip
@@ -328,6 +328,19 @@
 
 constexpr int kRecheckCap = 256;
 
+__device__ __forceinline__ int probe_prune_step(const int64_t *lens, double *near, int n, int j, bool live, float d, float r,
+                                                int need, int ld) {
+    const ProbeMargins pm = probe_margins(ld);
+    if (j >= 0) near[j] = live ? probe_near(d, r, pm) : 0.0;
+    __syncthreads();
+    const bool drop = j >= 0 && live && probe_dropped(lens, near, n, j, need, probe_far(d, r, pm), pm);
+    return 2 * __syncthreads_count(drop) + (drop ? 1 : 0);
+}
+__device__ __attribute__((noinline)) int probe_prune_step_call(const int64_t *lens, double *near, int n, int j, bool live,
+                                                               float d, float r, int need, int ld) {
+    return probe_prune_step(lens, near, n, j, live, d, r, need, ld);
+}
+
 template <typename T, bool DOT = false>
 __global__ __launch_bounds__(kQThreads) void batch_recheck_kernel(
     const char *__restrict__ vectors, const uint64_t *__restrict__ tids, int nvec, int lg,
@@ -345,7 +358,7 @@
     __shared__ __attribute__((aligned(16))) unsigned long long ent[kRecheckCap];
     const int q = blockIdx.x;
     const size_t row_bytes = (size_t)nvec * sizeof(Raw16);
-    const int64_t m = seg_start ? seg_start[q + 1] - seg_start[q] : fixed_len;
+    const int64_t m = (!DOT && seg_start) ? seg_start[q + 1] - seg_start[q] : fixed_len;
     const int ncand = (int)(m < kprime ? m : (int64_t)kprime);
     const int kk = ncand < k ? ncand : k;
     const float *av = approx_val + (size_t)q * kprime;
@@ -377,7 +390,8 @@
     if ((int)threadIdx.x < cnt) {
         const int64_t p = cand_pos[(size_t)q * kprime + threadIdx.x];
         int64_t slot = p;
-        if (cand_slot) {
+        if constexpr (DOT) {
+        } else if (cand_slot) {
             slot = cand_slot[(size_t)q * kprime + threadIdx.x];
         } else {
             const int64_t *off = probe_off + (size_t)q * probes;
@@ -423,27 +437,45 @@
     if ((int)threadIdx.x < cnt && rank < k) {
         const size_t o = (size_t)q * k + rank;
         out_dist[o] = key_to_float((unsigned)(mine >> 32));
-        if (out_slot) out_slot[o] = my_slot;
+        if constexpr (!DOT) {
+            if (out_slot) out_slot[o] = my_slot;
+            if (out_tid) out_tid[o] = tids ? tids[my_slot] : ~0ull;
+        }
         if (out_i32) out_i32[o] = (int32_t)my_slot;
-        if (out_tid) out_tid[o] = tids ? tids[my_slot] : ~0ull;
         if constexpr (DOT) pair_t[o] = -2.f * dots[threadIdx.x];
     }
     if ((int)threadIdx.x >= kk && (int)threadIdx.x < k) {
         const size_t o = (size_t)q * k + threadIdx.x;
         out_dist[o] = INFINITY;
-        if (out_slot) out_slot[o] = -1;
+        if constexpr (!DOT) {
+            if (out_slot) out_slot[o] = -1;
+            if (out_tid) out_tid[o] = ~0ull;
+        }
         if (out_i32) out_i32[o] = -1;
-        if (out_tid) out_tid[o] = ~0ull;
         if constexpr (DOT) pair_t[o] = 0.f;
     }
     if constexpr (DOT) {
         if (emit.cnt) {
             __syncthreads();
-            if ((int)threadIdx.x < cnt && rank < k) {
-                atomicAdd(&emit.cnt[my_slot], 1);
-                slots[rank] = emit.list_off[my_slot + 1] - emit.list_off[my_slot];
+            const bool emits = (int)threadIdx.x < cnt && rank < k;
+            const bool fills = (int)threadIdx.x >= kk && (int)threadIdx.x < k;
+            if (emits) slots[rank] = emit.list_off[my_slot + 1] - emit.list_off[my_slot];
+            if (fills) slots[threadIdx.x] = 0;
+            bool drop = false;
+            if (emit.radius) {
+                const int res = probe_prune_step(slots, reinterpret_cast<double *>(ent), k,
+                                                 emits ? rank : (fills ? (int)threadIdx.x : -1), emits,
+                                                 key_to_float((unsigned)(mine >> 32)), emits ? emit.radius[my_slot] : 0.f,
+                                                 emit.need, nvec * 4);
+                drop = (res & 1) != 0;
+                if (drop) {
+                    const size_t o = (size_t)q * k + rank;
+                    slots[rank] = 0;
+                    out_i32[o] = -1;
+                    pair_t[o] = 0.f;
+                }
             }
-            if ((int)threadIdx.x >= kk && (int)threadIdx.x < k) slots[threadIdx.x] = 0;
+            if (emits && !drop) atomicAdd(&emit.cnt[my_slot], 1);
             __syncthreads();
             if ((int)threadIdx.x < k) {
                 int64_t run = 0;
@@ -507,12 +539,26 @@
                     fill_pair_terms(vectors, row_bytes, qrow, nvec * 4, out_i32 ? out_i32 + (size_t)q * k : nullptr,
                                     out_slot ? out_slot + (size_t)q * k : nullptr, k, pair_t + (size_t)q * k);
                     if (emit.cnt) {
-                        if ((int)threadIdx.x < k) {
-                            const int l = __hip_atomic_load(out_i32 + (size_t)q * k + threadIdx.x, __ATOMIC_RELAXED,
-                                                            __HIP_MEMORY_SCOPE_AGENT);
-                            if (l >= 0) atomicAdd(&emit.cnt[l], 1);
+                        const bool mine_k = (int)threadIdx.x < k;
+                        const size_t o = (size_t)q * k + threadIdx.x;
+                        int l = -1;
+                        if (mine_k) {
+                            l = __hip_atomic_load(out_i32 + o, __ATOMIC_RELAXED, __HIP_MEMORY_SCOPE_AGENT);
                             slots[threadIdx.x] = l >= 0 ? emit.list_off[l + 1] - emit.list_off[l] : 0;
                         }
+                        if (emit.radius) {
+                            const int res = probe_prune_step_call(
+                                slots, reinterpret_cast<double *>(ent), k, mine_k ? (int)threadIdx.x : -1, l >= 0,
+                                mine_k ? __hip_atomic_load(out_dist + o, __ATOMIC_RELAXED, __HIP_MEMORY_SCOPE_AGENT) : 0.f,
+                                l >= 0 ? emit.radius[l] : 0.f, emit.need, nvec * 4);
+                            if (res & 1) {
+                                slots[threadIdx.x] = 0;
+                                out_i32[o] = -1;
+                                pair_t[o] = 0.f;
+                                l = -1;
+                            }
+                        }
+                        if (mine_k && l >= 0) atomicAdd(&emit.cnt[l], 1);
                         __syncthreads();
                         if ((int)threadIdx.x < k) {
                             int64_t run = 0;
@@ -618,6 +664,35 @@
     }
 }
 
+static_assert(kRecheckCap <= kQThreads, "a thread per probe");
+__global__ __launch_bounds__(kQThreads) void probe_prune_kernel(
+    const char *__restrict__ centers, const float *__restrict__ radius, const int64_t *__restrict__ list_off, int nvec,
+    int lg, const char *__restrict__ queries, const int32_t *__restrict__ probe_lists, int probes, int need,
+    int32_t *__restrict__ out_lists, float *__restrict__ pair_t) {
+    __shared__ float exact[kRecheckCap], dots[kRecheckCap];
+    __shared__ int64_t lens[kRecheckCap];
+    __shared__ double near[kRecheckCap];
+    __shared__ int32_t lists[kRecheckCap];
+    const int q = blockIdx.x;
+    const size_t row_bytes = (size_t)nvec * sizeof(Raw16);
+    const bool mine = (int)threadIdx.x < probes;
+    if (mine) lists[threadIdx.x] = probe_lists[(size_t)q * probes + threadIdx.x];
+    __syncthreads();
+    score_rows_dot([&](int64_t j) { return centers + (size_t)(lists[j] < 0 ? 0 : lists[j]) * row_bytes; }, 0, probes,
+                   queries + (size_t)q * row_bytes, nvec, lg, exact, dots);
+    __syncthreads();
+    const int l = mine ? lists[threadIdx.x] : -1;
+    if (mine) lens[threadIdx.x] = l >= 0 ? list_off[l + 1] - list_off[l] : 0;
+    const int res = probe_prune_step(lens, near, probes, mine ? (int)threadIdx.x : -1, l >= 0, mine ? exact[threadIdx.x] : 0.f,
+                                     l >= 0 ? radius[l] : 0.f, need, nvec * 4);
+    const bool drop = (res & 1) != 0;
+    if (mine) {
+        const size_t o = (size_t)q * probes + threadIdx.x;
+        out_lists[o] = drop ? -1 : l;
+        pair_t[o] = (drop || l < 0) ? 0.f : -2.f * dots[threadIdx.x];
+    }
+}
+
 constexpr size_t kQueryLds = (size_t)kHeadCap * 8 + sizeof(SelShared);
 
 void run_geometry(pgv_ctx *ctx, const RowGeom &g, int64_t nrows, int *per, int *grid) {
@@ -797,6 +872,20 @@
     return PGV_OK;
 }
 
+int probe_prune_max_probes() { return kRecheckCap; }
+
+int launch_probe_prune(pgv_ctx *ctx, const pgv_index *ix, const void *q_dev, int nq, const int32_t *probe_lists, int probes,
+                       int need, int32_t *out_lists, float *pair_t) {
+    if (nq <= 0) return PGV_OK;
+    if (probes < 1 || probes > kRecheckCap || !ix->list_radius || ix->dtype != PGV_F32)
+        PGV_FAIL(PGV_ERR_ARG, "probe pruning: fp32 rows with list radii, 1..%d probes", kRecheckCap);
+    hipLaunchKernelGGL(probe_prune_kernel, dim3(nq), dim3(kQThreads), 0, ctx->stream, static_cast<const char *>(ix->centers),
+                       ix->list_radius, ix->list_offsets, ix->geom.nvec, ix->geom.lpr_log2, static_cast<const char *>(q_dev),
+                       probe_lists, probes, need, out_lists, pair_t);
+    PGV_HIP(hipGetLastError());
+    return PGV_OK;
+}
+
 namespace {
 struct ApproxScratch {
     float *cand_val = nullptr;
@@ -823,7 +912,8 @@
         PGV_FAIL(PGV_ERR_ARG, "exact tail: a list plan or one dense run");
     if (t.kprime > kRecheckCap || t.k > t.kprime)
         PGV_FAIL(PGV_ERR_ARG, "exact tail: k' = %d outside k..%d", t.kprime, kRecheckCap);
-    if (t.pair_t && xr.dtype != PGV_F32) PGV_FAIL(PGV_ERR_ARG, "exact tail: pair terms are for fp32 rows");
+    if (t.pair_t && (xr.dtype != PGV_F32 || !dense || t.out_slot || t.out_tid || !t.out_i32))
+        PGV_FAIL(PGV_ERR_ARG, "exact tail: pair terms are for one dense run of fp32 rows whose slots leave as int32");
     static_assert(kWide >= kRecheckCap, "k <= k' <= kWide: batch_fix_kernel's emit");
     if (t.emit.cnt && !(dense && t.pair_t && t.out_i32 && t.emit.probe_off && t.emit.seg_len && t.emit.list_off))
         PGV_FAIL(PGV_ERR_ARG, "exact tail: the plan is counted where the pair terms are written");
diff --git a/pgvector_amd/csrc/kernels_select.hip b/pgvector_amd/csrc/kernels_select.hip
--- a/pgvector_amd/csrc/kernels_select.hip
+++ b/pgvector_amd/csrc/kernels_select.hip
@@ -16,6 +16,7 @@
     for (int p = 0; p < probes; p++) {
         const int l = probe_lists[(size_t)q * probes + p];
         probe_off[(size_t)q * probes + p] = run;
+        if (l < 0) continue;
         run += list_off[l + 1] - list_off[l];
         atomicAdd(&cnt[l], 1);
     }
@@ -56,7 +57,7 @@
     const int64_t *__restrict__ seg_len, int nq, int nlists, int qt, int rows_per_task,
     int64_t *__restrict__ seg_start, int64_t *__restrict__ pair_start,
     int64_t *__restrict__ task_start, int64_t *__restrict__ totals ,
-    double *__restrict__ acc) {
+    double *__restrict__ acc, int64_t given ) {
     __shared__ int64_t scratch[1024 / 64 + 1];
     __shared__ double red[2][1024 / 64];
     block_exclusive_scan(nq, [&](int i) { return seg_len[i]; }, seg_start, scratch);
@@ -97,6 +98,7 @@
             acc[0] += (double)seg_start[nq];
             acc[1] += r;
             acc[5] += u;
+            acc[8] += (double)(given - pair_start[nlists]);
         }
     }
 }
@@ -111,6 +113,7 @@
     if (i >= (int64_t)nq * probes) return;
     const int q = (int)(i / probes);
     const int l = probe_lists[i];
+    if (l < 0) return;
     const int64_t pos = pair_start[l] + atomicAdd(&fill[l], 1);
     ScanPair pr;
     pr.out_rel = seg_start[q] + probe_off[i] - list_off[l];
@@ -282,7 +285,8 @@
 __global__ __launch_bounds__(256) void plan_stats_kernel(const int *__restrict__ cnt,
                                                          const int64_t *__restrict__ list_off,
                                                          const int64_t *__restrict__ totals, int nlists,
-                                                         int qt, double *__restrict__ acc) {
+                                                         int qt, double *__restrict__ acc,
+                                                         const int64_t *__restrict__ pair_start, int64_t given) {
     __shared__ double red[256], red_u[256];
     double rows = 0.0, uniq = 0.0;
     for (int l = threadIdx.x; l < nlists; l += 256) {
@@ -304,6 +308,7 @@
         acc[0] += (double)totals[0];
         acc[1] += red[0];
         acc[5] += red_u[0];
+        acc[8] += (double)(given - pair_start[nlists]);
     }
 }
 
@@ -406,11 +411,11 @@
     if (counted) {
         double *acc = nullptr;
         if (read_totals) {
-            PGV_TRY(ctx->stats_dev.ensure(8 * sizeof(double)));
+            PGV_TRY(ctx->stats_dev.ensure(pgv::kStatsWords * sizeof(double)));
             acc = ctx->stats_dev.as<double>();
         }
         hipLaunchKernelGGL(plan_scan_kernel, dim3(1), dim3(1024), 0, ctx->stream, cnt, ix->list_offsets, seg_len, nq, nlists,
-                           qt, rows_per_task, seg_start, pair_start, task_start, totals, acc);
+                           qt, rows_per_task, seg_start, pair_start, task_start, totals, acc, (int64_t)npairs);
         hipLaunchKernelGGL(plan_pairs_tasks_kernel, dim3(pair_blocks + task_blocks), dim3(256), 0, ctx->stream, probe_lists,
                            ix->list_offsets, probe_off, seg_start, pair_start, task_start, cnt, fill, nq, probes, nlists, qt,
                            rows_per_task, pair_t, (int)pair_blocks, ctx->pairs.as<ScanPair>(), tasks);
@@ -421,7 +426,7 @@
                            probe_lists, ix->list_offsets, nq, probes, cnt, probe_off, seg_len);
         hipLaunchKernelGGL(plan_scan_kernel, dim3(1), dim3(1024), 0, ctx->stream, cnt,
                            ix->list_offsets, seg_len, nq, nlists, qt, rows_per_task, seg_start,
-                           pair_start, task_start, totals, static_cast<double *>(nullptr));
+                           pair_start, task_start, totals, static_cast<double *>(nullptr), (int64_t)npairs);
         hipLaunchKernelGGL(plan_pairs_kernel, dim3(pair_blocks), dim3(256), 0,
                            ctx->stream, probe_lists, ix->list_offsets, probe_off, seg_start,
                            pair_start, fill, nq, probes, pair_t, ctx->pairs.as<ScanPair>());
@@ -429,9 +434,10 @@
                            ctx->stream, cnt, ix->list_offsets, pair_start, task_start, nlists, qt, rows_per_task, tasks);
         PGV_HIP(hipGetLastError());
         if (read_totals) {
-            PGV_TRY(ctx->stats_dev.ensure(8 * sizeof(double)));
+            PGV_TRY(ctx->stats_dev.ensure(pgv::kStatsWords * sizeof(double)));
             hipLaunchKernelGGL(plan_stats_kernel, dim3(1), dim3(256), 0, ctx->stream, cnt,
-                               ix->list_offsets, totals, nlists, qt, ctx->stats_dev.as<double>());
+                               ix->list_offsets, totals, nlists, qt, ctx->stats_dev.as<double>(), pair_start,
+                               (int64_t)npairs);
             PGV_HIP(hipGetLastError());
         }
     }
diff --git a/pgvector_amd/csrc/kernels_shadow.hip b/pgvector_amd/csrc/kernels_shadow.hip
--- a/pgvector_amd/csrc/kernels_shadow.hip
+++ b/pgvector_amd/csrc/kernels_shadow.hip
@@ -50,23 +50,27 @@
                                                            const int64_t *__restrict__ list_off, int nlists, int64_t n,
                                                            int ld, int ld16, const unsigned *__restrict__ max_bits,
                                                            __half *__restrict__ shadow,
-                                                           unsigned long long *__restrict__ ep_bits) {
+                                                           unsigned long long *__restrict__ ep_bits,
+                                                           unsigned long long *__restrict__ radius_bits) {
     const int64_t r = (int64_t)blockIdx.x * 4 + (threadIdx.x >> 6);
     if (r >= n) return;
     const int lane = threadIdx.x & (kWave - 1);
     const int s = scale_for(__uint_as_float(*max_bits));
     const float *x = rows + (size_t)r * ld;
-    const float *c = centers ? centers + (size_t)list_of_row(list_off, nlists, r) * ld : nullptr;
+    const int list = centers ? list_of_row(list_off, nlists, r) : 0;
+    const float *c = centers ? centers + (size_t)list * ld : nullptr;
     __half *h = shadow + (size_t)r * ld16;
     const double up = ldexp(1.0, s);
-    double e2 = 0.0, p2 = 0.0;
+    double e2 = 0.0, p2 = 0.0, r2 = 0.0;
     for (int i = lane; i < ld16; i += kWave) {
         __half v = __float2half(0.f);
         if (i < ld) {
             const float ci = c ? c[i] : 0.f;
             v = __float2half(ldexpf(x[i] - ci, -s));
             const double back = (double)__half2float(v) * up;
-            const double d = ((double)x[i] - (double)ci) - back;
+            const double rho = (double)x[i] - (double)ci;
+            const double d = rho - back;
+            r2 = fma(rho, rho, r2);
             e2 = fma(d, d, e2);
             p2 = fma(back, back, p2);
         }
@@ -75,12 +79,18 @@
     for (int o = 32; o > 0; o >>= 1) {
         e2 += __shfl_xor(e2, o);
         p2 += __shfl_xor(p2, o);
+        r2 += __shfl_xor(r2, o);
     }
     if (lane == 0) {
         const unsigned long long eb = (unsigned long long)__double_as_longlong(e2 != e2 ? INFINITY : e2),
                                  pb = (unsigned long long)__double_as_longlong(p2 != p2 ? INFINITY : p2);
         if (eb > __hip_atomic_load(&ep_bits[0], __ATOMIC_RELAXED, __HIP_MEMORY_SCOPE_AGENT)) atomicMax(&ep_bits[0], eb);
         if (pb > __hip_atomic_load(&ep_bits[1], __ATOMIC_RELAXED, __HIP_MEMORY_SCOPE_AGENT)) atomicMax(&ep_bits[1], pb);
+        if (radius_bits) {
+            const unsigned long long rb = (unsigned long long)__double_as_longlong(r2 != r2 ? INFINITY : r2);
+            if (rb > __hip_atomic_load(&radius_bits[list], __ATOMIC_RELAXED, __HIP_MEMORY_SCOPE_AGENT))
+                atomicMax(&radius_bits[list], rb);
+        }
     }
 }
 
@@ -243,8 +253,9 @@
 }
 
 int launch_shadow_build(pgv_ctx *ctx, const RowGeom &g32, const RowGeom &g16, const void *rows, const void *centers,
-                        const int64_t *list_off, int nlists, int64_t n, void *shadow, void *words) {
+                        const int64_t *list_off, int nlists, int64_t n, void *shadow, void *words, void *radius_bits) {
     if (n <= 0) return PGV_OK;
+    if (radius_bits) PGV_HIP(hipMemsetAsync(radius_bits, 0, sizeof(unsigned long long) * (size_t)nlists, ctx->stream));
     PGV_HIP(hipMemsetAsync(words, 0, 24, ctx->stream));
     unsigned *max_bits = static_cast<unsigned *>(words);
     unsigned long long *ep = reinterpret_cast<unsigned long long *>(static_cast<char *>(words) + 8);
@@ -252,7 +263,8 @@
     hipLaunchKernelGGL(shadow_absmax_kernel, grid, dim3(256), 0, ctx->stream, static_cast<const float *>(rows),
                        static_cast<const float *>(centers), list_off, nlists, n, g32.ld, max_bits);
     hipLaunchKernelGGL(shadow_build_kernel, grid, dim3(256), 0, ctx->stream, static_cast<const float *>(rows),
-                       static_cast<const float *>(centers), list_off, nlists, n, g32.ld, g16.ld, max_bits, static_cast<__half *>(shadow), ep);
+                       static_cast<const float *>(centers), list_off, nlists, n, g32.ld, g16.ld, max_bits, static_cast<__half *>(shadow), ep,
+                       centers ? static_cast<unsigned long long *>(radius_bits) : nullptr);
     PGV_HIP(hipGetLastError());
     return PGV_OK;
 }
diff --git a/pgvector_amd/csrc/pgv_abi.hip b/pgvector_amd/csrc/pgv_abi.hip
--- a/pgvector_amd/csrc/pgv_abi.hip
+++ b/pgvector_amd/csrc/pgv_abi.hip
@@ -229,8 +229,8 @@
     PGV_TRY(resolve_events(ctx));
     ctx->profiling = on != 0;
     if (ctx->profiling && !ctx->stats_dev.p) {
-        PGV_TRY(ctx->stats_dev.ensure(8 * sizeof(double)));
-        PGV_HIP(hipMemsetAsync(ctx->stats_dev.p, 0, 8 * sizeof(double), ctx->stream));
+        PGV_TRY(ctx->stats_dev.ensure(pgv::kStatsWords * sizeof(double)));
+        PGV_HIP(hipMemsetAsync(ctx->stats_dev.p, 0, pgv::kStatsWords * sizeof(double), ctx->stream));
     }
     for (pgv_ctx *c : ctx->children) PGV_TRY(pgv_ctx_set_profiling(c, on));
     return PGV_OK;
@@ -260,7 +260,7 @@
     ctx->scan_launches = 0;
     ctx->scan_pairs = 0;
     ctx->scan_rows = 0;
-    if (ctx->stats_dev.p) PGV_HIP(hipMemsetAsync(ctx->stats_dev.p, 0, 8 * sizeof(double), ctx->stream));
+    if (ctx->stats_dev.p) PGV_HIP(hipMemsetAsync(ctx->stats_dev.p, 0, pgv::kStatsWords * sizeof(double), ctx->stream));
     ctx->aux_ms = 0;
     ctx->aux_launches = 0;
     ctx->aux_pairs = 0;
@@ -272,7 +272,7 @@
 int pgv_ctx_get_stats(pgv_ctx *ctx, pgv_stats *out) {
     if (!ctx || !out) PGV_FAIL(PGV_ERR_ARG, "ctx/out is NULL");
     PGV_TRY(resolve_events(ctx));
-    double dev_acc[8] = {0.0, 0.0, 0.0, 0.0, 0.0, 0.0, 0.0, 0.0};
+    double dev_acc[pgv::kStatsWords] = {};
     if (ctx->stats_dev.p) {
         PGV_HIP(hipMemcpyAsync(dev_acc, ctx->stats_dev.p, sizeof(dev_acc), hipMemcpyDeviceToHost, ctx->stream));
         PGV_HIP(hipStreamSynchronize(ctx->stream));
@@ -290,6 +290,7 @@
     out->scan_unique_rows = dev_acc[5];
     out->scan_redo_queries = dev_acc[6];
     out->scan_widened_queries = dev_acc[7];
+    out->scan_pruned_probes = dev_acc[8];
     out->scan_shadow_queries = ctx->scan_shadow_queries;
     for (pgv_ctx *c : ctx->children) {
         pgv_stats cs;
@@ -307,6 +308,7 @@
         out->scan_unique_rows += cs.scan_unique_rows;
         out->scan_redo_queries += cs.scan_redo_queries;
         out->scan_widened_queries += cs.scan_widened_queries;
+        out->scan_pruned_probes += cs.scan_pruned_probes;
         out->scan_shadow_queries += cs.scan_shadow_queries;
     }
     return PGV_OK;
diff --git a/pgvector_amd/csrc/pgv_abi_common.h b/pgvector_amd/csrc/pgv_abi_common.h
--- a/pgvector_amd/csrc/pgv_abi_common.h
+++ b/pgvector_amd/csrc/pgv_abi_common.h
@@ -359,7 +359,7 @@
 extern "C" {
 int rank_lists_dev(pgv_index *ix, const void *q_dev, int nq, int maxprobes, int32_t *out_lists_dev, float *out_dist_dev);
 int scan_batch_dev(pgv_index *ix, const void *q_dev, int nq, const int32_t *probe_lists, int probes, int k, float *out_dist,
-                   int64_t *out_slot, uint64_t *out_tid);
+                   int64_t *out_slot, uint64_t *out_tid, bool prune = false);
 int check_batch_args(pgv_index *ix, const void *queries, int nq, int probes, int k, float *out_dist, uint64_t *out_tid,
                      const char *who);
 int kmpp_begin(pgv_ctx *ctx, int n_local, int k, int64_t n_total, Rng &rng, KmppState *state, int64_t *first);
diff --git a/pgvector_amd/csrc/pgv_abi_ivf.hip b/pgvector_amd/csrc/pgv_abi_ivf.hip
--- a/pgvector_amd/csrc/pgv_abi_ivf.hip
+++ b/pgvector_amd/csrc/pgv_abi_ivf.hip
@@ -60,6 +60,11 @@
     return e ? atoi(e) : 1;
 }
 
+bool probe_prune_on(const pgv_index *ix, int probes) {
+    const char *e = getenv("PGV_PROBE_PRUNE");
+    return (e ? atoi(e) != 0 : true) && ix->list_radius && probes <= probe_prune_max_probes();
+}
+
 int shadow_create(pgv_ctx *ctx, pgv_index *ix) {
     const int env = shadow_env();
     if (env == 0 || ix->metric != PGV_L2SQ || ix->dtype != PGV_F32 || ix->nrows <= 0 || !ix->row_norms || !ix->center_norms)
@@ -68,15 +73,17 @@
     const RowGeom g16 = row_geom(ix->dim, PGV_F16);
     const size_t bytes = ((size_t)ix->nrows * g16.ld * sizeof(uint16_t) + 255) & ~(size_t)255;
     const size_t cbytes = ((size_t)ix->nlists * g16.ld * sizeof(uint16_t) + 255) & ~(size_t)255;
+    const size_t rbytes = sizeof(unsigned long long) * (size_t)ix->nlists;
     void *sh = nullptr;
-    if (hipMalloc(&sh, bytes + 256 + cbytes) != hipSuccess) {
+    if (hipMalloc(&sh, bytes + 256 + cbytes + rbytes) != hipSuccess) {
         (void)hipGetLastError();
         return PGV_OK;
     }
     void *words = static_cast<char *>(sh) + bytes;
     void *csh = static_cast<char *>(sh) + bytes + 256;
+    void *rad = static_cast<char *>(sh) + bytes + 256 + cbytes;
     int rc = launch_shadow_build(ctx, ix->geom, g16, ix->vectors, ix->centers, ix->list_offsets, ix->nlists, ix->nrows, sh,
-                                 words);
+                                 words, rad);
     if (rc == PGV_OK)
         rc = launch_shadow_build(ctx, ix->geom, g16, ix->centers, nullptr, nullptr, 0, ix->nlists, csh,
                                  static_cast<char *>(words) + 32);
@@ -105,6 +112,23 @@
     ix->shadow_s = shadow_scale_of(max_abs);
     ix->shadow_E = (E + 1e-12 * (P + E)) * (1.0 + 1e-9);
     ix->shadow_P = P * (1.0 + 1e-9);
+    {
+        std::vector<unsigned long long> rb((size_t)ix->nlists);
+        std::vector<float> rf((size_t)ix->nlists);
+        if (hipMemcpy(rb.data(), rad, rbytes, hipMemcpyDeviceToHost) == hipSuccess) {
+            for (int l = 0; l < ix->nlists; l++) {
+                double r2;
+                memcpy(&r2, &rb[l], 8);
+                const double R = std::sqrt(r2) * (1.0 + 1e-9);
+                float f = (float)R;
+                if (std::isfinite(f) && (double)f < R) f = std::nextafterf(f, INFINITY);
+                rf[l] = std::isfinite(R) ? f : INFINITY;
+            }
+            if (hipMemcpy(rad, rf.data(), sizeof(float) * rf.size(), hipMemcpyHostToDevice) == hipSuccess)
+                ix->list_radius = static_cast<float *>(rad);
+        }
+        (void)hipGetLastError();
+    }
     float cmax_abs;
     double ce2, cp2;
     memcpy(&cmax_abs, h + 32, 4);
@@ -126,6 +150,7 @@
     float *cscale = nullptr, *ceps = nullptr;
     float *pair_t = nullptr;
     bool scan_follows = false;
+    int need = 0;
     bool cast_for_scan = false;
     bool pairs_done = false;
 };
@@ -830,6 +855,10 @@
         if (tail.pair_t) {
             PGV_TRY(plan_batch_reserve(ctx, ix->nlists, nq, maxprobes, &pbuf));
             tail.emit = {pbuf.cnt, pbuf.probe_off, pbuf.seg_len, ix->list_offsets};
+            if (sb->need > 0 && probe_prune_on(ix, maxprobes)) {
+                tail.emit.radius = ix->list_radius;
+                tail.emit.need = sb->need;
+            }
         }
         tail.rows = {ix->centers, nullptr, nullptr, ix->geom, ix->dtype,
                      reinterpret_cast<const unsigned *>(ix->center_norms + ix->nlists)};
@@ -952,7 +981,7 @@
 }
 
 static int scan_batch_impl(pgv_index *ix, const void *q_dev, int nq, const int32_t *probe_lists, int probes,
-                           int k, float *out_dist, int64_t *out_slot, uint64_t *out_tid, ShadowBatch *sb) {
+                           int k, float *out_dist, int64_t *out_slot, uint64_t *out_tid, ShadowBatch *sb, bool prune) {
     pgv_ctx *ctx = ix->ctx;
     const ScanPath path = scan_path(ix, nq, probes, k);
     if (path.per_query) {
@@ -980,9 +1009,16 @@
     if (!sb) sb = &own;
     if (path.shadow && !sb->cast_for_scan) PGV_TRY(shadow_batch_cast(ix, q_dev, nq, probes, false, true, sb));
     const float *pair_t = (path.shadow && sb->pairs_done) ? sb->pair_t : nullptr;
+    const bool counted = pair_t != nullptr;
+    if (path.shadow && !pair_t && prune && probe_prune_on(ix, probes)) {
+        PGV_TRY(ctx->plan_c.ensure(sizeof(int32_t) * (size_t)nq * probes));
+        PGV_TRY(launch_probe_prune(ctx, ix, q_dev, nq, probe_lists, probes, k, ctx->plan_c.as<int32_t>(), sb->pair_t));
+        probe_lists = ctx->plan_c.as<int32_t>();
+        pair_t = sb->pair_t;
+    }
     PlanResult plan;
     PGV_TRY(launch_plan_batch(ctx, ix, probe_lists, nq, probes, path.qt, path.rows_per_task, ctx->profiling, &plan, pair_t,
-                              pair_t != nullptr));
+                              counted));
     if (path.shadow) {
         if (!pair_t)
             PGV_TRY(launch_shadow_pairs(ctx, ix->geom, q_dev, ix->centers, plan.pair_start, ix->nlists, (int64_t)nq * probes,
@@ -1036,8 +1072,8 @@
 }
 
 int scan_batch_dev(pgv_index *ix, const void *q_dev, int nq, const int32_t *probe_lists, int probes, int k, float *out_dist,
-                   int64_t *out_slot, uint64_t *out_tid) {
-    return scan_batch_impl(ix, q_dev, nq, probe_lists, probes, k, out_dist, out_slot, out_tid, nullptr);
+                   int64_t *out_slot, uint64_t *out_tid, bool prune) {
+    return scan_batch_impl(ix, q_dev, nq, probe_lists, probes, k, out_dist, out_slot, out_tid, nullptr, prune);
 }
 
 int pgv_scan_lists(pgv_index *ix, const void *query, const int32_t *lists, int nlists,
@@ -1160,8 +1196,9 @@
     int32_t *probe_lists = ctx->idx_stage.as<int32_t>();
     ShadowBatch sb;
     sb.scan_follows = scan_path(ix, nq, probes, k).shadow;
+    sb.need = k;
     PGV_TRY(rank_lists_impl(ix, q_dev, nq, probes, probe_lists, nullptr, &sb));
-    return scan_batch_impl(ix, q_dev, nq, probe_lists, probes, k, out_dist, out_slot, out_tid, &sb);
+    return scan_batch_impl(ix, q_dev, nq, probe_lists, probes, k, out_dist, out_slot, out_tid, &sb, true);
 }
 
 int pgv_scan_batch(pgv_index *ix, const void *queries, int nq, const int32_t *probe_lists, int probes, int k,
@@ -1180,7 +1217,7 @@
     PGV_TRY(stage_queries(ix, queries, nq, &q_dev));
     PGV_TRY(stage_flat(ctx, probe_lists, sizeof(int32_t) * (size_t)nq * probes, ctx->idx_stage, &pl_dev));
     return scan_batch_dev(ix, q_dev, nq, static_cast<const int32_t *>(pl_dev), probes, k, out_dist, out_slot,
-                          out_tid);
+                          out_tid, true);
 }
 
 int pgv_index_shadow_cast(pgv_index *ix, const void *queries, int nq, void *out_qcast, float *out_qscale, float *out_qeps,
diff --git a/pgvector_amd/csrc/pgv_internal.h b/pgvector_amd/csrc/pgv_internal.h
--- a/pgvector_amd/csrc/pgv_internal.h
+++ b/pgvector_amd/csrc/pgv_internal.h
@@ -112,6 +112,7 @@
     int32_t query;
     int32_t pad;
 };
+constexpr int kStatsWords = 9;
 struct ScanWork {
     const ScanTask *tasks;
     const int *ntasks_dev;
@@ -188,6 +189,7 @@
     int shadow_s = 0;
     double shadow_E = 0.0;
     double shadow_P = 0.0;
+    float *list_radius = nullptr;
     void *cshadow = nullptr;
     int cshadow_s = 0;
     double cshadow_E = 0.0;
@@ -324,6 +326,41 @@
 inline ScanBound shadow_band(int ld, float g_ref, double u = 5.9604645e-8) {
     return {0.f, 0.f, gamma_n(ld / 64.0 + 10.0, u), g_ref};
 }
+#if defined(__HIPCC__)
+#define PGV_HD __host__ __device__
+#else
+#define PGV_HD
+#endif
+struct ProbeMargins {
+    double g = 0.0, a = 0.0;
+};
+PGV_HD inline ProbeMargins probe_margins(int ld) {
+    const double n = (ld + 4.0) * 5.9604644775390625e-8;
+    return {n / (1.0 - n), (ld + 4.0) * 1.401298464324817e-45};
+}
+PGV_HD inline double probe_near(float d, float R, ProbeMargins pm) { return sqrt(((double)d + pm.a) / (1.0 - pm.g)) + (double)R; }
+PGV_HD inline double probe_far(float d, float R, ProbeMargins pm) {
+    const double e = (double)d - pm.a;
+    return sqrt((e > 0.0 ? e : 0.0) / (1.0 + pm.g)) - (double)R;
+}
+PGV_HD inline bool probe_dropped(const int64_t *lens, const double *near, int n, int j, int need, double far, ProbeMargins pm) {
+    int64_t rows = 0;
+    double tau = 0.0;
+    bool finite = true;
+    int m = 0;
+    while (m < n && rows < need) {
+        rows += lens[m];
+        const double h = near[m];
+        finite = finite && h < (double)INFINITY;
+        tau = h > tau ? h : tau;
+        m++;
+    }
+    if (rows < need || j < m || !finite) return false;
+    if (!(far > 0.0) || !(far < (double)INFINITY)) return false;
+    const double lo2 = far * far * (1.0 - pm.g) - pm.a, hi2 = tau * tau * (1.0 + pm.g) + pm.a;
+    return hi2 < 3.0e38 && lo2 > hi2 * (1.0 + 9.094947017729282e-13);
+}
+
 struct ExpansionBound {
     float gamma;
     float gamma_exact;
@@ -460,7 +497,8 @@
                      const float *query_norms, float *out, bool stream_rows, int queries_per_task = 32,
                      const float *shadow_scale = nullptr);
 int launch_shadow_build(pgv_ctx *ctx, const RowGeom &g32, const RowGeom &g16, const void *rows, const void *centers,
-                        const int64_t *list_off, int nlists, int64_t n, void *shadow, void *words);
+                        const int64_t *list_off, int nlists, int64_t n, void *shadow, void *words,
+                        void *radius_bits = nullptr);
 int shadow_scale_of(float max_abs);
 int shadow_chain_length(const RowGeom &g16);
 int scan_chain_length(const RowGeom &g, pgv_dtype dtype, bool wide);
@@ -503,7 +541,12 @@
     int *cnt = nullptr;
     int64_t *probe_off = nullptr, *seg_len = nullptr;
     const int64_t *list_off = nullptr;
-};
+    const float *radius = nullptr;
+    int need = 0;
+};
+int probe_prune_max_probes();
+int launch_probe_prune(pgv_ctx *ctx, const pgv_index *ix, const void *q_dev, int nq, const int32_t *probe_lists, int probes,
+                       int need, int32_t *out_lists, float *pair_t);
 int launch_plan_batch(pgv_ctx *ctx, const pgv_index *ix, const int32_t *probe_lists, int nq,
                       int probes, int qt, int rows_per_task, bool read_totals, PlanResult *res,
                       const float *pair_t = nullptr, bool counted = false);
```

Result: faster. 1.595 million, median of 6 (+13.8%).
